# AMReX-Combustion/PeleAnalysis

Measured on AMD Instinct MI355X. Metric: Mcells/s for grad+curvature on 512^3-base 3-level AMR; % HBM roofline, higher is better.
Workload: dtype f64; 1 GPU; fused grad->curvature, 3-level AMR, base 512^3, ref_ratio 2, 128^3 boxes (64 per level) in the file, swept on the internal tiling pa_level_retile makes of them (4, 4, 4 boxes per level, largest 512x256x256), 1 comp(s), periodic x/y + wall z, 402653184 cells in the job; cells=402653184, cells_this_rank=402653184, ncomp=1, components_per_batch=1, fused=True, parallelism=single GPU

## Files before the change

include/peleanalysis_amd.h:

```cpp
#ifndef PELEANALYSIS_AMD_H
#define PELEANALYSIS_AMD_H
#include <stdint.h>

#ifdef __cplusplus
extern "C" {
#endif

typedef struct pa_ctx pa_ctx;
typedef struct pa_level pa_level;
typedef struct pa_mf pa_mf;

typedef struct { double* p; int32_t lo[3]; int32_t hi[3]; int32_t ncomp; int64_t nstride; } pa_fab;
typedef struct { int32_t lo[3]; int32_t hi[3]; } pa_box;

enum { PA_BC_PERIODIC = 0, PA_BC_NEUMANN = 1, PA_BC_REFLECT_ODD = 2 };

int         pa_version(void);
pa_ctx*     pa_ctx_create(int device, void* hip_stream );
void        pa_ctx_destroy(pa_ctx*);
const char* pa_last_error(const pa_ctx*);
int         pa_sync(pa_ctx*);
void*       pa_ctx_stream(pa_ctx*);
void        pa_options_reload(void);

void* pa_device_malloc(pa_ctx*, int64_t bytes);
void  pa_device_free(pa_ctx*, void* devptr);
int   pa_memcpy_h2d(pa_ctx*, void* devdst, const void* hostsrc, int64_t bytes);
int   pa_memcpy_d2h(pa_ctx*, void* hostdst, const void* devsrc, int64_t bytes);
int   pa_memcpy_d2d(pa_ctx*, void* devdst, const void* devsrc, int64_t bytes);
int   pa_device_count(void);

int pa_profile_enable(pa_ctx*, int on);
const char* pa_sweep_kernel_name(const pa_ctx*);
int pa_sweep_occupancy(pa_ctx*, int which);
int pa_last_slow_cells(pa_ctx*);
int64_t pa_level_irregular_cells(pa_ctx*, const pa_level*);
int pa_profile_read(pa_ctx*, int tag, int64_t* nlaunch, double* total_ms, int reset);

pa_level* pa_level_create(pa_ctx*, int nboxes, const int32_t* boxes6, const int32_t domlo[3],
                          const int32_t domhi[3], const int32_t is_per[3], const double prob_lo[3],
                          const double prob_hi[3]);
typedef struct { int32_t peer; double* sendbuf; int64_t nsend; double* recvbuf; int64_t nrecv; } pa_xfer;
typedef struct {
  void*   user;
  int32_t rank, nranks;
  int (*exchange)(void* user, void* hip_stream, int32_t n, const pa_xfer* x);
  int (*allreduce)(void* user, double* vals, int32_t n, int32_t op);
} pa_comm;
int pa_ctx_set_comm(pa_ctx*, const pa_comm*);
int pa_ctx_set_delay_comm(pa_ctx*, int nranks, int rank, double fixed_us, double link_GBs);
int pa_delay_comm_stats(const pa_ctx*, int64_t* calls, double* total_us);
int pa_rccl_unique_id(pa_ctx*, void* id128);
int pa_ctx_init_rccl(pa_ctx*, int nranks, int rank, const void* id128);
int pa_ctx_nranks(const pa_ctx*);
int pa_comm_selftest(pa_ctx*, int64_t n);
int pa_allreduce(pa_ctx*, double* vals, int n, int op);
int pa_distribution_map(int nboxes, const int32_t* boxes6, int nranks, int32_t* owner);
pa_level* pa_level_create_sharded(pa_ctx*, int nboxes, const int32_t* boxes6, const int32_t* owner, int rank, int nranks,
                                  const int32_t domlo[3], const int32_t domhi[3], const int32_t is_per[3],
                                  const double prob_lo[3], const double prob_hi[3]);
int pa_level_global_ids(const pa_level*, int32_t* gids );
int64_t pa_plan_fill_boundary(int nboxes, const int32_t* boxes6, const int32_t* owner, int rank, const int32_t domlo[3],
                              const int32_t domhi[3], const int32_t is_per[3], int ng, int32_t* rows9, int64_t cap);
int64_t pa_plan_coarse_source(int nfine, const int32_t* fboxes6, const int32_t* fowner, const int32_t fdomlo[3],
                              const int32_t fdomhi[3], int ncrse, const int32_t* cboxes6, const int32_t* cowner,
                              const int32_t cdomlo[3], const int32_t cdomhi[3], const int32_t is_per[3], int rank,
                              int mode, int ng, int halo, int32_t* rows9, int64_t cap);
int64_t pa_plan_restriction(int nfine, const int32_t* fboxes6, const int32_t* fowner, const int32_t fdomlo[3],
                            const int32_t fdomhi[3], int ncrse, const int32_t* cboxes6, const int32_t* cowner,
                            const int32_t cdomlo[3], const int32_t cdomhi[3], const int32_t is_per[3], int rank, int ratio,
                            int which, int32_t* rows9, int64_t cap);
int pa_level_retile(int nboxes, const int32_t* boxes6, const int32_t max_size[3], int min_thick, int32_t* out_boxes6, int cap);
int pa_hierarchy_retile_limits(int nlev, const int32_t* nboxes, const int32_t* const* boxes6, int min_thick, int32_t max_size[3]);
int pa_hierarchy_retile_limits_ranks(int nlev, const int32_t* nboxes, const int32_t* const* boxes6, int min_thick, int nranks, int32_t max_size[3]);
void      pa_level_destroy(pa_level*);
int       pa_level_nboxes(const pa_level*);

int64_t pa_mf_layout(int nboxes, const int32_t* boxes6, int ncomp, int ng, int64_t* off, int64_t* cstride);
pa_mf*  pa_mf_create(pa_ctx*, const pa_level*, int ncomp, int ng, double* devptr );
void    pa_mf_destroy(pa_mf*);
double* pa_mf_data(pa_mf*);
int64_t pa_mf_size(const pa_mf*);
int     pa_mf_upload(pa_ctx*, pa_mf*, const double* host);
int     pa_mf_download(pa_ctx*, const pa_mf*, double* host);
int     pa_mf_upload_comps(pa_ctx*, pa_mf*, const double* host, int comp, int ncomp);
int     pa_mf_download_comps(pa_ctx*, const pa_mf*, double* host, int comp, int ncomp);
int     pa_mf_setval(pa_ctx*, pa_mf*, int comp, int ncomp, double v);
int     pa_mf_copy(pa_ctx*, const pa_mf* src, int scomp, pa_mf* dst, int dcomp, int ncomp, int ng);

int pa_fill_boundary(pa_ctx*, pa_mf*, int comp, int ncomp, int ng);
int pa_apply_bc(pa_ctx*, pa_mf* fine, int comp, const pa_mf* crse, int ccomp, const int32_t bc[3],
                int ratio, int only_dir);
int pa_bc_errors(pa_ctx*);

int pa_grad_level(pa_ctx*, const pa_mf* phi, int comp, pa_mf* out, int ocomp);
int pa_minmax_level(pa_ctx*, const pa_mf* s, int comp, double* mn, double* mx);
int pa_progress_level(pa_ctx*, const pa_mf* s, int comp, double pmin, double pmax, pa_mf* c, int ccomp, int ng);
int pa_normal_level(pa_ctx*, const pa_mf* c, int comp, pa_mf* G, int gcomp, pa_mf* normgrad, int ngcomp,
                    pa_mf* n, int ncomp0);
int pa_div_level(pa_ctx*, pa_mf* n, int ncomp0, double scale, const pa_mf* c, int ccomp, double thr,
                 pa_mf* K, int kcomp);
int pa_progress_shell_level(pa_ctx*, const pa_mf* s, int comp, double pmin, double pmax, pa_mf* c, int ccomp, int ng,
                            int depth);
int pa_gradcurv_level(pa_ctx*, const pa_mf* phi, int pcomp, double prog_min, double prog_max, double thr,
                      pa_mf* out, int ocomp);
int pa_gradcurv_faces_level(pa_ctx*, const pa_mf* c, int ccomp, const pa_mf* crse_n ,
                            int cncomp0, const int32_t bc[3], int ratio, double thr, pa_mf* out, int ncomp0,
                            int kcomp);

int pa_grad_fab(pa_ctx*, pa_box valid, const pa_fab* phi, int comp, const double dxinv[3], pa_fab* out, int ocomp);
int pa_progress_fab(pa_ctx*, pa_box bx, const pa_fab* s, int comp, double pmin, double pmax, pa_fab* c, int ccomp);
int pa_normal_fab(pa_ctx*, pa_box valid, const pa_fab* c, int comp, const double dxinv[3], pa_fab* G, int gcomp,
                  pa_fab* normgrad, int ngcomp, pa_fab* n, int ncomp0);
int pa_div_fab(pa_ctx*, pa_box valid, const pa_fab* n, int ncomp0, const double dxinv[3], double scale,
               pa_fab* K, int kcomp);
int pa_gradcurv_fab(pa_ctx*, pa_box valid, const pa_fab* phi, int pcomp, double prog_min, double prog_max,
                    const double dxinv[3], double thr, pa_fab* out, int ocomp);
int pa_boxfilter_fab(pa_ctx*, pa_box valid, const pa_fab* in, pa_fab* out, int scomp, int ncomp, int ng,
                     const double* w );

int pa_box_filter_weights(int fgr, double* w);
int pa_filter_weights(int type, int fgr, double* w);
int pa_boxfilter_level(pa_ctx*, const pa_mf* in, pa_mf* out, int scomp, int ncomp, int ng, const double* w);
int pa_boxfilter_hierarchy(pa_ctx*, int nlev, const pa_mf* const* in, pa_mf* const* out, int scomp, int ncomp, const int32_t* ngs,
                           const double* const* ws);
int pa_boxfilter_level2d(pa_ctx*, const pa_mf* in, pa_mf* out, int scomp, int ncomp, int ng, const double* w);
int pa_foextrap(pa_ctx*, pa_mf*, int comp, int ncomp, int ng);
int pa_fillpatch_two_levels(pa_ctx*, pa_mf* fine, const pa_mf* crse, int comp, int ncomp, int ng, int ratio,
                            int interp_type);

int pa_fill_ghosts_hierarchy(pa_ctx*, int nlev, pa_mf* const* mfs, int comp, int ncomp, const int32_t* ngs, int ratio, int interp_type, int foextrap);

int pa_mc_count_fab(pa_ctx*, pa_box loop, const pa_fab* state, const pa_fab* mask, int isocomp, double isoval,
                    int64_t* nvert, int64_t* ntri);
int pa_mc_emit_fab(pa_ctx*, pa_box loop, const pa_fab* state, const pa_fab* mask, int isocomp, double isoval,
                   double* dev_verts , int32_t* dev_vkeys ,
                   int32_t* dev_tris , int64_t nvert, int64_t ntri);
int pa_iso_mask_level(pa_ctx*, pa_mf* mask, int comp, const pa_level* fine, int ratio);
int pa_iso_coords_level(pa_ctx*, pa_mf* state, int comp0);
int pa_mc_level(pa_ctx*, const pa_mf* state, const pa_mf* mask, int mcomp, const pa_box* loops ,
                int isocomp, double isoval, int64_t* nvert , int64_t* ntri ,
                double** dev_verts , int32_t** dev_vkeys ,
                int32_t** dev_tris );
int pa_msq_level(pa_ctx*, const pa_mf* state, const pa_mf* mask, int mcomp, const pa_box* loops ,
                 int isocomp, double isoval, int64_t* nvert , int64_t* nseg ,
                 double** dev_verts , int32_t** dev_vkeys ,
                 int32_t** dev_segs );
int pa_mc_level_fine(pa_ctx*, const pa_mf* state, const pa_level* fine, int ratio, const pa_box* loops, int isocomp,
                     double isoval, int64_t* nvert, int64_t* ntri, double** dev_verts, int32_t** dev_vkeys,
                     int32_t** dev_tris);
int pa_msq_level_fine(pa_ctx*, const pa_mf* state, const pa_level* fine, int ratio, const pa_box* loops, int isocomp,
                      double isoval, int64_t* nvert, int64_t* nseg, double** dev_verts, int32_t** dev_vkeys,
                      int32_t** dev_segs);
int pa_mc_hierarchy_fine(pa_ctx*, int nlev, const pa_mf* const* states, const int32_t* fine_mask, int ratio,
                         const pa_box* const* loops, int isocomp, double isoval, int64_t* const* nvert, int64_t* const* ntri,
                         double** dev_verts, int32_t** dev_vkeys, int32_t** dev_tris, void** block);
int pa_mc_hierarchy_xyz(pa_ctx*, int nlev, const pa_mf* const* fields, const int32_t* fine_mask, int ratio, const pa_box* const* loops,
                        int isocomp, double isoval, int64_t* const* nvert, int64_t* const* ntri, double** dev_verts, int32_t** dev_vkeys,
                        int32_t** dev_tris, void** block);
typedef struct { const double* verts; int64_t nvert; const int32_t* tris; int64_t ntri; } pa_iso_frag;
int pa_iso_merge(pa_ctx*, int nfrag, const pa_iso_frag* frags , int ncomp, int64_t* nnodes,
                 double** dev_nodes, int64_t* nelts, int32_t** dev_elts);
const uint16_t* pa_mc_edge_table(void);
const int8_t*   pa_mc_tri_table(void);

typedef struct {
  int64_t ntri;  const uint32_t* tri;
  int64_t nvert; const float* x;
  float origin[3]; float dx;
  int32_t n[3];
  float* phi;
} pa_sdf_grid;
int pa_sdf_level_set3(pa_ctx*, int ngrids, const pa_sdf_grid* grids , int exact_band );
int pa_sdf_signed_fab(pa_ctx*, pa_box vbox, const float* dev_phi, const pa_fab* state, int isocomp, double isoval,
                      double dmax, pa_fab* dist, int dcomp);

int pa_stream_trace(pa_ctx*, int nlev, pa_mf* const* vfield, int vcomp, int64_t nseed, const double* seeds, int nsteps,
                    double dt, double* dev_pos, int32_t* nredist );
int pa_stream_trace_ranks(pa_ctx*, int nlev, pa_mf* const* vfield, int vcomp, int64_t nseed, const double* seeds, int nsteps,
                          double dt, double* dev_pos, int32_t* nredist , int share_flags);

int pa_vtrace_fab(pa_ctx*, const pa_fab* T, int32_t nT, const double* loc, int64_t nloc, const int32_t* ids, int32_t n_ids,
                  pa_fab* g, int32_t computeVec, pa_fab* strm, int32_t ncs, const double dx[3], const double plo[3],
                  const double phi[3], double hRK, int32_t* errFlag);
int pa_streamgrad_prepare(pa_ctx*, int nlev, pa_mf* const* state);
int pa_streamgrad_trace(pa_ctx*, int nlev, pa_mf* const* state, int vcomp, int64_t nnodes, const double* nodes,
                        const int64_t* box_start, const int32_t* ids, int nRKsteps, double hRK, double* strm,
                        int32_t* box_flag);

// ... 97 lines not shown
```

peleanalysis_amd/capi.py:

```python
from __future__ import annotations

import ctypes as C
import os
from typing import List, Optional, Sequence

import numpy as np

from .hierarchy import Hierarchy, Level, MultiFab, mf_layout

_HERE = os.path.dirname(os.path.abspath(__file__))
LIB_PATH = os.path.join(_HERE, "libpeleanalysis_amd.so")

BC_PERIODIC, BC_NEUMANN, BC_REFLECT_ODD = 0, 1, 2


class PaFab(C.Structure):
    _fields_ = [("p", C.c_void_p), ("lo", C.c_int32 * 3), ("hi", C.c_int32 * 3), ("ncomp", C.c_int32), ("nstride", C.c_int64)]


class PaBox(C.Structure):
    _fields_ = [("lo", C.c_int32 * 3), ("hi", C.c_int32 * 3)]


class PaCurvParams(C.Structure):
    _fields_ = [("prog_min", C.c_double), ("prog_max", C.c_double), ("do_threshold", C.c_int32), ("threshold", C.c_double),
                ("fused", C.c_int32), ("do_gauss_curv", C.c_int32), ("do_strain", C.c_int32), ("get_strain_tensor", C.c_int32),
                ("do_velnormal", C.c_int32), ("vel_comp", C.c_int32), ("do_smooth", C.c_int32), ("smoothing_time", C.c_double),
                ("spacedim", C.c_int32)]


class PaXfer(C.Structure):
    _fields_ = [("peer", C.c_int32), ("sendbuf", C.c_void_p), ("nsend", C.c_int64), ("recvbuf", C.c_void_p), ("nrecv", C.c_int64)]


EXCHANGE_FN = C.CFUNCTYPE(C.c_int, C.c_void_p, C.c_void_p, C.c_int32, C.POINTER(PaXfer))
ALLREDUCE_FN = C.CFUNCTYPE(C.c_int, C.c_void_p, C.POINTER(C.c_double), C.c_int32, C.c_int32)


DONE_FN = C.CFUNCTYPE(C.c_int, C.c_void_p, C.c_int)
DONE2_FN = C.CFUNCTYPE(C.c_int, C.c_void_p, C.c_int, C.c_int)


class PaComm(C.Structure):
    _fields_ = [("user", C.c_void_p), ("rank", C.c_int32), ("nranks", C.c_int32), ("exchange", EXCHANGE_FN), ("allreduce", ALLREDUCE_FN)]


class PaIsoFrag(C.Structure):
    _fields_ = [("verts", C.c_void_p), ("nvert", C.c_int64), ("tris", C.c_void_p), ("ntri", C.c_int64)]


class PaJpdfParams(C.Structure):
    _fields_ = [("nload", C.c_int32), ("do_stoichiometry", C.c_int32), ("hlist", C.c_double * 8), ("olist", C.c_double * 8), ("vmin", C.c_double * 8),
                ("vmax", C.c_double * 8), ("do_conditioning", C.c_int32), ("cvar", C.c_int32), ("norm_cval", C.c_int32), ("cnorm_min", C.c_double),
                ("cnorm_max", C.c_double), ("cmin", C.c_double), ("cmax", C.c_double), ("uncombined", C.c_int32)]


class PaSdfGrid(C.Structure):
    _fields_ = [("ntri", C.c_int64), ("tri", C.c_void_p), ("nvert", C.c_int64), ("x", C.c_void_p), ("origin", C.c_float * 3), ("dx", C.c_float),
                ("n", C.c_int32 * 3), ("phi", C.c_void_p)]


_lib = None


def load_library() -> C.CDLL:
    global _lib
    if _lib is not None:
        return _lib
    if not os.path.exists(LIB_PATH):
        raise RuntimeError(f"{LIB_PATH} not found: run `python -c 'import __graft_entry__ as g; g.build()'` "
                           "(hipcc --offload-arch=gfx950).  There is no CPU fallback.")
    L = C.CDLL(LIB_PATH)
    vp, i32, i64, dbl = C.c_void_p, C.c_int32, C.c_int64, C.c_double
    pi32, pdbl = C.POINTER(C.c_int32), C.POINTER(C.c_double)
    sig = {
        "pa_version": (C.c_int, []),
        "pa_options_reload": (None, []),
        "pa_ctx_create": (vp, [C.c_int, vp]),
        "pa_ctx_destroy": (None, [vp]),
        "pa_last_error": (C.c_char_p, [vp]),
        "pa_sync": (C.c_int, [vp]),
        "pa_ctx_stream": (vp, [vp]),
        "pa_device_malloc": (vp, [vp, i64]),
        "pa_device_free": (None, [vp, vp]),
        "pa_memcpy_h2d": (C.c_int, [vp, vp, vp, i64]),
        "pa_memcpy_d2h": (C.c_int, [vp, vp, vp, i64]),
        "pa_memcpy_d2d": (C.c_int, [vp, vp, vp, i64]),
        "pa_device_count": (C.c_int, []),
        "pa_profile_enable": (C.c_int, [vp, C.c_int]),
        "pa_sweep_kernel_name": (C.c_char_p, [vp]),
        "pa_sweep_occupancy": (C.c_int, [vp, C.c_int]),
        "pa_profile_read": (C.c_int, [vp, C.c_int, C.POINTER(i64), pdbl, C.c_int]),
        "pa_level_create": (vp, [vp, C.c_int, pi32, pi32, pi32, pi32, pdbl, pdbl]),
        "pa_level_create_sharded": (vp, [vp, C.c_int, pi32, pi32, C.c_int, C.c_int, pi32, pi32, pi32, pdbl, pdbl]),
        "pa_level_global_ids": (C.c_int, [vp, pi32]),
        "pa_ctx_set_comm": (C.c_int, [vp, C.POINTER(PaComm)]),
        "pa_ctx_set_delay_comm": (C.c_int, [vp, C.c_int, C.c_int, dbl, dbl]),
        "pa_delay_comm_stats": (C.c_int, [vp, C.POINTER(i64), pdbl]),
        "pa_rccl_unique_id": (C.c_int, [vp, vp]),
        "pa_ctx_init_rccl": (C.c_int, [vp, C.c_int, C.c_int, vp]),
        "pa_ctx_nranks": (C.c_int, [vp]),
        "pa_comm_selftest": (C.c_int, [vp, i64]),
        "pa_allreduce": (C.c_int, [vp, pdbl, C.c_int, C.c_int]),
        "pa_distribution_map": (C.c_int, [C.c_int, pi32, C.c_int, pi32]),
        "pa_plan_fill_boundary": (i64, [C.c_int, pi32, pi32, C.c_int, pi32, pi32, pi32, C.c_int, pi32, i64]),
        "pa_plan_coarse_source": (i64, [C.c_int, pi32, pi32, pi32, pi32, C.c_int, pi32, pi32, pi32, pi32, pi32, C.c_int, C.c_int, C.c_int, C.c_int, pi32,
                                        i64]),
        "pa_plan_restriction": (i64, [C.c_int, pi32, pi32, pi32, pi32, C.c_int, pi32, pi32, pi32, pi32, pi32, C.c_int, C.c_int, C.c_int, pi32, i64]),
        "pa_level_retile": (C.c_int, [C.c_int, pi32, pi32, C.c_int, pi32, C.c_int]),
        "pa_hierarchy_retile_limits": (C.c_int, [C.c_int, pi32, C.POINTER(pi32), C.c_int, pi32]),
        "pa_hierarchy_retile_limits_ranks": (C.c_int, [C.c_int, pi32, C.POINTER(pi32), C.c_int, C.c_int, pi32]),
        "pa_level_destroy": (None, [vp]),
        "pa_level_nboxes": (C.c_int, [vp]),
        "pa_mf_layout": (i64, [C.c_int, pi32, C.c_int, C.c_int, C.POINTER(i64), C.POINTER(i64)]),
        "pa_mf_create": (vp, [vp, vp, C.c_int, C.c_int, vp]),
        "pa_mf_destroy": (None, [vp]),
        "pa_mf_data": (vp, [vp]),
        "pa_mf_size": (i64, [vp]),
        "pa_mf_upload": (C.c_int, [vp, vp, vp]),
        "pa_mf_download": (C.c_int, [vp, vp, vp]),
        "pa_mf_upload_comps": (C.c_int, [vp, vp, vp, C.c_int, C.c_int]),
        "pa_mf_download_comps": (C.c_int, [vp, vp, vp, C.c_int, C.c_int]),
        "pa_mf_setval": (C.c_int, [vp, vp, C.c_int, C.c_int, dbl]),
        "pa_mf_copy": (C.c_int, [vp, vp, C.c_int, vp, C.c_int, C.c_int, C.c_int]),
        "pa_fill_boundary": (C.c_int, [vp, vp, C.c_int, C.c_int, C.c_int]),
        "pa_apply_bc": (C.c_int, [vp, vp, C.c_int, vp, C.c_int, pi32, C.c_int, C.c_int]),
        "pa_bc_errors": (C.c_int, [vp]),
        "pa_grad_level": (C.c_int, [vp, vp, C.c_int, vp, C.c_int]),
        "pa_minmax_level": (C.c_int, [vp, vp, C.c_int, pdbl, pdbl]),
        "pa_progress_level": (C.c_int, [vp, vp, C.c_int, dbl, dbl, vp, C.c_int, C.c_int]),
        "pa_normal_level": (C.c_int, [vp, vp, C.c_int, vp, C.c_int, vp, C.c_int, vp, C.c_int]),
        "pa_div_level": (C.c_int, [vp, vp, C.c_int, dbl, vp, C.c_int, dbl, vp, C.c_int]),
        "pa_progress_shell_level": (C.c_int, [vp, vp, C.c_int, dbl, dbl, vp, C.c_int, C.c_int, C.c_int]),
        "pa_gradcurv_level": (C.c_int, [vp, vp, C.c_int, dbl, dbl, dbl, vp, C.c_int]),
        "pa_gradcurv_faces_level": (C.c_int, [vp, vp, C.c_int, vp, C.c_int, pi32, C.c_int, dbl, vp, C.c_int, C.c_int]),
        "pa_grad_fab": (C.c_int, [vp, PaBox, C.POINTER(PaFab), C.c_int, pdbl, C.POINTER(PaFab), C.c_int]),
        "pa_progress_fab": (C.c_int, [vp, PaBox, C.POINTER(PaFab), C.c_int, dbl, dbl, C.POINTER(PaFab), C.c_int]),
        "pa_normal_fab": (C.c_int, [vp, PaBox, C.POINTER(PaFab), C.c_int, pdbl, C.POINTER(PaFab), C.c_int, C.POINTER(PaFab), C.c_int,
                                    C.POINTER(PaFab), C.c_int]),
        "pa_div_fab": (C.c_int, [vp, PaBox, C.POINTER(PaFab), C.c_int, pdbl, dbl, C.POINTER(PaFab), C.c_int]),
        "pa_gradcurv_fab": (C.c_int, [vp, PaBox, C.POINTER(PaFab), C.c_int, dbl, dbl, pdbl, dbl, C.POINTER(PaFab), C.c_int]),
        "pa_boxfilter_fab": (C.c_int, [vp, PaBox, C.POINTER(PaFab), C.POINTER(PaFab), C.c_int, C.c_int, C.c_int, pdbl]),
        "pa_box_filter_weights": (C.c_int, [C.c_int, pdbl]),
        "pa_filter_weights": (C.c_int, [C.c_int, C.c_int, pdbl]),
        "pa_boxfilter_level": (C.c_int, [vp, vp, vp, C.c_int, C.c_int, C.c_int, pdbl]),
        "pa_boxfilter_hierarchy": (C.c_int, [vp, C.c_int, C.POINTER(vp), C.POINTER(vp), C.c_int, C.c_int, pi32, C.POINTER(pdbl)]),
        "pa_boxfilter_level2d": (C.c_int, [vp, vp, vp, C.c_int, C.c_int, C.c_int, pdbl]),
        "pa_foextrap": (C.c_int, [vp, vp, C.c_int, C.c_int, C.c_int]),
        "pa_fillpatch_two_levels": (C.c_int, [vp, vp, vp, C.c_int, C.c_int, C.c_int, C.c_int, C.c_int]),
        "pa_fill_ghosts_hierarchy": (C.c_int, [vp, C.c_int, C.POINTER(vp), C.c_int, C.c_int, pi32, C.c_int, C.c_int, C.c_int]),
        "pa_mc_count_fab": (C.c_int, [vp, PaBox, C.POINTER(PaFab), C.POINTER(PaFab), C.c_int, dbl, C.POINTER(i64), C.POINTER(i64)]),
        "pa_mc_emit_fab": (C.c_int, [vp, PaBox, C.POINTER(PaFab), C.POINTER(PaFab), C.c_int, dbl, vp, vp, vp, i64, i64]),
        "pa_iso_mask_level": (C.c_int, [vp, vp, C.c_int, vp, C.c_int]),
        "pa_iso_coords_level": (C.c_int, [vp, vp, C.c_int]),
        "pa_mc_level_fine": (C.c_int, [vp, vp, vp, C.c_int, C.POINTER(PaBox), C.c_int, dbl, C.POINTER(i64), C.POINTER(i64), C.POINTER(vp), C.POINTER(vp),
                                       C.POINTER(vp)]),
        "pa_msq_level_fine": (C.c_int, [vp, vp, vp, C.c_int, C.POINTER(PaBox), C.c_int, dbl, C.POINTER(i64), C.POINTER(i64), C.POINTER(vp), C.POINTER(vp),
                                        C.POINTER(vp)]),
        "pa_mc_hierarchy_fine": (C.c_int, [vp, C.c_int, C.POINTER(vp), pi32, C.c_int, C.POINTER(C.POINTER(PaBox)), C.c_int, dbl, C.POINTER(C.POINTER(i64)),
                                           C.POINTER(C.POINTER(i64)), C.POINTER(vp), C.POINTER(vp), C.POINTER(vp), C.POINTER(vp)]),
        "pa_mc_hierarchy_xyz": (C.c_int, [vp, C.c_int, C.POINTER(vp), pi32, C.c_int, C.POINTER(C.POINTER(PaBox)), C.c_int, dbl, C.POINTER(C.POINTER(i64)),
                                          C.POINTER(C.POINTER(i64)), C.POINTER(vp), C.POINTER(vp), C.POINTER(vp), C.POINTER(vp)]),
        "pa_msq_level": (C.c_int, [vp, vp, vp, C.c_int, C.POINTER(PaBox), C.c_int, dbl, C.POINTER(i64), C.POINTER(i64), C.POINTER(vp), C.POINTER(vp),
                                   C.POINTER(vp)]),
        "pa_mc_level": (C.c_int, [vp, vp, vp, C.c_int, C.POINTER(PaBox), C.c_int, dbl, C.POINTER(i64), C.POINTER(i64), C.POINTER(vp), C.POINTER(vp),
                                  C.POINTER(vp)]),
        "pa_iso_merge": (C.c_int, [vp, C.c_int, C.POINTER(PaIsoFrag), C.c_int, C.POINTER(i64), C.POINTER(vp), C.POINTER(i64), C.POINTER(vp)]),
        "pa_mc_edge_table": (C.POINTER(C.c_uint16), []),
        "pa_mc_tri_table": (C.POINTER(C.c_int8), []),
        "pa_sdf_level_set3": (C.c_int, [vp, C.c_int, C.POINTER(PaSdfGrid), C.c_int]),
        "pa_sdf_signed_fab": (C.c_int, [vp, PaBox, vp, C.POINTER(PaFab), C.c_int, dbl, dbl, C.POINTER(PaFab), C.c_int]),
        "pa_smooth_solve": (C.c_int, [vp, C.c_int, C.POINTER(vp), C.c_int, C.POINTER(vp), C.c_int, dbl, pi32, dbl, C.c_int, C.POINTER(C.c_int), pdbl]),
        "pa_stream_trace": (C.c_int, [vp, C.c_int, C.POINTER(vp), C.c_int, i64, pdbl, C.c_int, dbl, vp, pi32]),
        "pa_last_slow_cells": (C.c_int, [vp]),
        "pa_level_irregular_cells": (i64, [vp, vp]),
        "pa_stream_trace_ranks": (C.c_int, [vp, C.c_int, C.POINTER(vp), C.c_int, i64, pdbl, C.c_int, dbl, vp, pi32, C.c_int]),
        "pa_vtrace_fab": (C.c_int, [vp, C.POINTER(PaFab), i32, vp, i64, vp, i32, C.POINTER(PaFab), i32, C.POINTER(PaFab), i32, pdbl, pdbl, pdbl, dbl,
                                    pi32]),
        "pa_streamgrad_prepare": (C.c_int, [vp, C.c_int, C.POINTER(vp)]),
        "pa_streamgrad_trace": (C.c_int, [vp, C.c_int, C.POINTER(vp), C.c_int, i64, vp, C.POINTER(i64), vp, C.c_int, dbl, vp, pi32]),
        "pa_interpstream_fab": (C.c_int, [vp, C.POINTER(PaFab), i32, C.POINTER(PaFab), i32, C.POINTER(PaFab), pdbl, pdbl, pi32]),
        "pa_set_distance_fab": (C.c_int, [vp, C.POINTER(PaFab), C.POINTER(PaFab)]),
        "pa_streamsample_run": (C.c_int, [vp, C.c_int, C.POINTER(vp), i32, pdbl, pdbl, pi32, pi32, pi32, pi32, pi32, vp, vp, i32, i32, i32, pi32]),
        "pa_device_mem_info": (C.c_int, [vp, C.POINTER(i64), C.POINTER(i64)]),
        "pa_minmax_comps_level": (C.c_int, [vp, vp, C.c_int, pi32, pdbl, pdbl]),
        "pa_jpdf_create": (vp, [vp, C.c_int, C.c_int]),
        "pa_jpdf_begin": (C.c_int, [vp, vp, dbl, pdbl]),
        "pa_jpdf_add_level": (C.c_int, [vp, vp, vp, vp, C.c_int, dbl, C.POINTER(PaJpdfParams), C.POINTER(i64), C.POINTER(i64)]),
        "pa_jpdf_read": (C.c_int, [vp, vp, pdbl, pdbl, pdbl]),
        "pa_condmean_create": (vp, [vp, C.c_int, C.c_int, C.c_int]),
        "pa_condmean_begin": (C.c_int, [vp, vp, i64, pdbl]),
        "pa_condmean_add_level": (C.c_int, [vp, vp, vp, vp, C.c_int, C.POINTER(PaBox), i64, dbl, dbl, C.c_int]),
        "pa_condmean_read": (C.c_int, [vp, vp, C.POINTER(i64), pdbl, pdbl, pdbl, pdbl]),
        "pa_hist_destroy": (None, [vp]),
        "pa_integral_create": (vp, [vp, C.c_int, C.c_int, C.c_int, C.POINTER(PaBox), C.c_int]),
        "pa_integral_begin": (C.c_int, [vp, vp, dbl, pdbl]),
        "pa_integral_add_level": (C.c_int, [vp, vp, vp, vp, C.c_int, C.c_int, dbl, C.c_int, dbl, dbl, C.c_int]),
        "pa_integral_slots": (i64, [vp]),
        "pa_integral_read": (C.c_int, [vp, vp, pdbl]),
        "pa_integral_destroy": (None, [vp]),
        "pa_tube_create": (vp, [vp, i32, C.POINTER(i64), i64, pi32, i64, pi32]),
        "pa_tube_destroy": (None, [vp]),
        "pa_tube_wedges": (C.c_int, [vp, vp, vp, vp, i32, i32, i32, i32, vp, vp, vp, vp, vp]),
        "pa_tube_lines": (C.c_int, [vp, vp, vp, vp, i32, i32, i32, vp]),
        "pa_tube_peaks": (C.c_int, [vp, vp, vp, i32, i32, i32, pi32, vp, vp]),
        "pa_tube_node_means": (C.c_int, [vp, vp, i32, vp, vp]),
        "pa_tube_node_all": (C.c_int, [vp, vp, vp, vp]),
        "pa_tube_node_avg": (C.c_int, [vp, vp, vp, i32, i32, vp]),
        "pa_tube_smooth": (C.c_int, [vp, vp, vp, vp, i32, vp]),
        "pa_tube_neighbors": (C.c_int, [vp, vp, C.POINTER(i64), C.POINTER(i64), pi32]),
        "pa_smooth_last": (C.c_int, [vp, C.POINTER(C.c_int), pdbl]),
        "pa_curvature_last_path": (C.c_int, [vp]),
        "pa_level_free_scratch": (i64, [vp]),
        "pa_grad_run": (C.c_int, [vp, C.c_int, C.POINTER(vp), C.c_int, pi32, C.POINTER(vp), C.c_int]),
        "pa_curvature_run": (C.c_int, [vp, C.c_int, C.POINTER(vp), C.c_int, pi32, C.POINTER(PaCurvParams), C.POINTER(vp), C.c_int]),
        "pa_gradcurv_run": (C.c_int, [vp, C.c_int, C.POINTER(vp), C.c_int, pi32, C.POINTER(PaCurvParams), C.POINTER(vp), C.POINTER(vp),
                                      C.c_int]),
        "pa_gradcurv_run_comps": (C.c_int, [vp, C.c_int, C.POINTER(vp), C.c_int, C.c_int, pi32, C.POINTER(PaCurvParams), C.POINTER(vp), C.POINTER(vp),
                                            C.c_int, DONE_FN, vp]),
        "pa_gradcurv_run_comps2": (C.c_int, [vp, C.c_int, C.POINTER(vp), C.c_int, C.c_int, pi32, C.POINTER(PaCurvParams), C.POINTER(vp), C.POINTER(vp),
                                             C.c_int, C.c_int, DONE2_FN, vp]),
    }
    missing = []
    for name, (res, args) in sig.items():
        try:
            fn = getattr(L, name)
        except AttributeError:
            missing.append(name)
            continue
        fn.restype = res
        fn.argtypes = args
    L._pa_signatures = sig
    L._pa_missing = missing
    _lib = L
    return L


def declared_symbols(header: Optional[str] = None) -> List[str]:
    import re
    header = header or os.path.join(os.path.dirname(_HERE), "include", "peleanalysis_amd.h")
    txt = re.sub(r"/\*.*?\*/", "", open(header).read(), flags=re.S)
    return sorted(set(re.findall(r"\b(pa_[a-z0-9_]+)\s*\(", txt)))


def reload_options() -> None:
    load_library().pa_options_reload()


class PaError(RuntimeError):
    pass


def _i3(v):
    return (C.c_int32 * 3)(*[int(x) for x in v])


def _d3(v):
    return (C.c_double * 3)(*[float(x) for x in v])


class Context:
    def __init__(self, device: int = 0, stream: Optional[int] = None):
        self.lib = load_library()
        self.h = self.lib.pa_ctx_create(int(device), C.c_void_p(stream) if stream else None)
        if not self.h:
            raise PaError("pa_ctx_create failed: no MI355X/HIP device visible (no CPU fallback)")

    def check(self, rc: int):
        if rc != 0:
            raise PaError(self.lib.pa_last_error(self.h).decode())

    def sync(self):
        self.check(self.lib.pa_sync(self.h))

    def profile_enable(self, on=True):
        self.check(self.lib.pa_profile_enable(self.h, int(on)))

    def profile_read(self, tag: int, reset: bool = False):
        n, ms = C.c_int64(0), C.c_double(0.0)
        self.check(self.lib.pa_profile_read(self.h, tag, C.byref(n), C.byref(ms), int(reset)))
        return n.value, ms.value

    def bc_errors(self) -> int:
        return int(self.lib.pa_bc_errors(self.h))

    def set_comm(self, comm: "PaComm"):
        self._comm = comm
        self.check(self.lib.pa_ctx_set_comm(self.h, C.byref(comm) if comm is not None else None))

    def rccl_unique_id(self) -> bytes:
        buf = C.create_string_buffer(128)
        self.check(self.lib.pa_rccl_unique_id(self.h, buf))
        return buf.raw

    def init_rccl(self, nranks: int, rank: int, unique_id: bytes):
        assert len(unique_id) == 128
        self.check(self.lib.pa_ctx_init_rccl(self.h, int(nranks), int(rank), C.create_string_buffer(unique_id, 128)))

    def comm_selftest(self, n: int = 4096):
        self.check(self.lib.pa_comm_selftest(self.h, int(n)))

    def allreduce(self, vals, op: int):
        a = np.ascontiguousarray(vals, dtype=np.float64).copy()
        self.check(self.lib.pa_allreduce(self.h, a.ctypes.data_as(C.POINTER(C.c_double)), a.size, int(op)))
        return a

    def close(self):
        if self.h:
            self.lib.pa_ctx_destroy(self.h)
            self.h = None

    def __enter__(self):
        return self

    def __exit__(self, *exc):
        self.close()


class DevBuf:

    def __init__(self, ctx: Context, nbytes: int):
        self.ctx, self.nbytes = ctx, int(nbytes)
        self.ptr = ctx.lib.pa_device_malloc(ctx.h, self.nbytes)
        if not self.ptr:
            raise PaError(ctx.lib.pa_last_error(ctx.h).decode())

    @classmethod
    def from_numpy(cls, ctx: Context, a: np.ndarray) -> "DevBuf":
# ... 689 lines not shown
```

peleanalysis_amd/csrc/pa_core.hip:

```cpp
#include "pa_internal.h"
#include "pa_dist.h"
#include <algorithm>
#include <atomic>
#include <cstring>
#include <numeric>

int pa_fail(pa_ctx* ctx, const std::string& msg) {
  if (ctx) ctx->err = msg;
  return 1;
}

extern "C" int pa_version(void) { return 100; }

static int host_owner(const pa_level* L, int i, int j, int k);
const WgTab* pa_sweep_wgtab(const pa_level* L, int cls, int tw, int mty, int kseg, bool force, int part) {
  if (part) force = true;
  const long long key = ((long long)cls << 56) | ((long long)part << 54) | ((long long)(force ? 1 : 0) << 52) | ((long long)tw << 40) | ((long long)mty << 24) | (long long)kseg;
  auto it = L->wgtabs.find(key);
  if (it != L->wgtabs.end()) return (it->second->d || part) ? it->second.get() : nullptr;
  std::unique_ptr<WgTab> T(new WgTab());
  struct Chunk { int n, box, t0; };
  std::vector<std::pair<int, int>> bt;
  std::vector<std::vector<int>> sel;
  long long real = 0;
// ... 536 lines not shown
        cpoff[e] = L->cp_total;
        L->cp_total += ((long long)pw * ph + 7) / 8 * 8;
      }
    }
    sfindex[f] = (int)e;
    sfoff[e] = ncode;
    ncode += (long long)(B.hi[t0] - B.lo[t0] + 1) * (B.hi[t1] - B.lo[t1] + 1);
    L->cgoff[e] = L->cg_total;
    L->cg_total += ((long long)(B.hi[t0] - B.lo[t0] + 3) * (B.hi[t1] - B.lo[t1] + 5) + 7) / 8 * 8;
  }
  {
    std::vector<int> wide, narrow;
    for (int b = 0; b < nboxes; ++b) {
      const DBox& B = L->boxes[b];
      const bool nar = B.hi[0] - B.lo[0] + 1 <= 32;
      (nar ? narrow : wide).push_back(b);
      for (int d = 0; d < 3; ++d) {
        int& m = nar ? L->nmax[d] : L->wmax[d];
        m = std::max(m, B.hi[d] - B.lo[d] + 1);
      }
    }
    L->nwide = (int)wide.size();
    L->nnarrow = (int)narrow.size();
    if (L->nwide && L->nnarrow) {
      wide.insert(wide.end(), narrow.begin(), narrow.end());
      if (hipMalloc(&L->d_blist, sizeof(int) * wide.size()) != hipSuccess ||
          hipMemcpy(L->d_blist, wide.data(), sizeof(int) * wide.size(), hipMemcpyHostToDevice) != hipSuccess) {
        pa_fail(ctx, "pa_level_create: device allocation failed");
        delete L;
        return nullptr;
      }
    }
  }
  {
    std::vector<int> wg, pwg;
    for (size_t e = 0; e < L->sfaces.size(); ++e) {
      const int f = L->sfaces[e];
      const DBox& B = L->boxes[f / 6];
      const int d = (f % 6) >> 1, t0 = (d == 0) ? 1 : 0, t1 = (d == 2) ? 1 : 2;
      const long long nc = (long long)(B.hi[t0] - B.lo[t0] + 1) * (B.hi[t1] - B.lo[t1] + 1);
      for (int c = 0; c < (int)((nc + 255) / 256); ++c) { wg.push_back((int)e); wg.push_back(c); }
      const long long n0 = B.hi[t0] - B.lo[t0] + 1, n1 = B.hi[t1] - B.lo[t1] + 1, P = n1 >= 2 ? 2 * n0 + 2 * (n1 - 2) : n0;
      for (int c = 0; c < (int)((P + 255) / 256); ++c) { pwg.push_back((int)e); pwg.push_back(c); }
    }
    L->npfwg = (int)(pwg.size() / 2);
    if (L->npfwg > 0 && (hipMalloc(&L->d_pfwg, sizeof(int) * pwg.size()) != hipSuccess ||
                         hipMemcpy(L->d_pfwg, pwg.data(), sizeof(int) * pwg.size(), hipMemcpyHostToDevice) != hipSuccess)) {
      pa_fail(ctx, "pa_level_create: device allocation failed");
      delete L;
      return nullptr;
    }
    std::vector<int> sfb;
    for (int f : L->sfaces)
      if (sfb.empty() || sfb.back() != f / 6) sfb.push_back(f / 6);
    L->nsfboxes = (int)sfb.size();
    if (L->nsfboxes > 0 && (hipMalloc(&L->d_sfboxes, sizeof(int) * sfb.size()) != hipSuccess ||
                            hipMemcpy(L->d_sfboxes, sfb.data(), sizeof(int) * sfb.size(), hipMemcpyHostToDevice) != hipSuccess)) {
      pa_fail(ctx, "pa_level_create: device allocation failed");
      delete L;
      return nullptr;
    }
    {
      std::vector<SfChunk> ck;
      for (size_t e = 0; e < L->sfaces.size(); ++e) {
        const int f = L->sfaces[e];
        const DBox& B = L->boxes[f / 6];
        const int d = (f % 6) >> 1, t0 = (d == 0) ? 1 : 0, t1 = (d == 2) ? 1 : 2;
        const int n0 = B.hi[t0] - B.lo[t0] + 1, n1 = B.hi[t1] - B.lo[t1] + 1;
        int cw = 32;
        while (cw < 512 && cw < n0) cw *= 2;
        const int ch = 1024 / cw;
        for (int v0 = -(B.lo[t1] & 1); v0 < n1; v0 += ch)
          for (int u0 = -(B.lo[t0] & 1); u0 < n0; u0 += cw) {
            SfChunk D;
            D.face = (int)e; D.box = f / 6; D.dir_side = f % 6; D.flags = 0;
            for (int q = 0; q < 3; ++q) { D.lo[q] = B.lo[q]; D.hi[q] = B.hi[q]; }
            D.u0 = u0; D.v0 = v0; D.cw = cw; D.ch = ch;
            D.sfoff = sfoff[e]; D.cgoff = L->cgoff[e]; D.cpoff = cpoff[e];
            ck.push_back(D);
          }
      }
      L->nsfchunk = (int)ck.size();
      if (L->nsfchunk > 0 && (hipMalloc(&L->d_sfchunk, sizeof(SfChunk) * ck.size()) != hipSuccess ||
                              hipMemcpy(L->d_sfchunk, ck.data(), sizeof(SfChunk) * ck.size(), hipMemcpyHostToDevice) != hipSuccess)) {
        pa_fail(ctx, "pa_level_create: device allocation failed");
        delete L;
        return nullptr;
      }
    }
    L->nsfwg = (int)(wg.size() / 2);
    if (L->nsfwg > 0 && (hipMalloc(&L->d_sfwg, sizeof(int) * wg.size()) != hipSuccess ||
                         hipMemcpy(L->d_sfwg, wg.data(), sizeof(int) * wg.size(), hipMemcpyHostToDevice) != hipSuccess)) {
      pa_fail(ctx, "pa_level_create: device allocation failed");
      delete L;
      return nullptr;
    }
  }
  if (hipMalloc(&L->d_boxes, sizeof(DBox) * std::max(nboxes, 1)) != hipSuccess ||
      hipMalloc(&L->d_sfaces, sizeof(int) * nsf_alloc) != hipSuccess ||
      (!L->sfaces.empty() && hipMemcpy(L->d_sfaces, L->sfaces.data(), sizeof(int) * L->sfaces.size(), hipMemcpyHostToDevice) != hipSuccess) ||
      hipMalloc(&L->d_sfindex, sizeof(int) * std::max<size_t>(sfindex.size(), 1)) != hipSuccess ||
      (!sfindex.empty() && hipMemcpy(L->d_sfindex, sfindex.data(), sizeof(int) * sfindex.size(), hipMemcpyHostToDevice) != hipSuccess) ||
      hipMalloc(&L->d_cpoff, sizeof(long long) * nsf_alloc) != hipSuccess ||
      hipMemcpy(L->d_cpoff, cpoff.data(), sizeof(long long) * nsf_alloc, hipMemcpyHostToDevice) != hipSuccess ||
      hipMalloc(&L->d_cgoff, sizeof(long long) * nsf_alloc) != hipSuccess ||
      hipMemcpy(L->d_cgoff, L->cgoff.data(), sizeof(long long) * nsf_alloc, hipMemcpyHostToDevice) != hipSuccess ||
      hipMalloc(&L->d_sfoff, sizeof(long long) * nsf_alloc) != hipSuccess ||
      hipMemcpy(L->d_sfoff, sfoff.data(), sizeof(long long) * nsf_alloc, hipMemcpyHostToDevice) != hipSuccess ||
      hipMalloc(&L->d_sfcode, sizeof(unsigned short) * std::max<long long>(ncode, 1)) != hipSuccess ||
      hipMalloc(&L->d_owner, sizeof(int) * msz) != hipSuccess ||
      (nboxes > 0 && hipMemcpy(L->d_boxes, L->boxes.data(), sizeof(DBox) * nboxes, hipMemcpyHostToDevice) != hipSuccess) ||
      hipMemcpy(L->d_owner, L->owner.data(), sizeof(int) * msz, hipMemcpyHostToDevice) != hipSuccess) {
    pa_fail(ctx, "pa_level_create: device allocation failed");
    if (L->d_boxes) (void)hipFree(L->d_boxes);
    if (L->d_owner) (void)hipFree(L->d_owner);
    if (L->d_sfaces) (void)hipFree(L->d_sfaces);
    if (L->d_sfindex) (void)hipFree(L->d_sfindex);
    if (L->d_sfoff) (void)hipFree(L->d_sfoff);
    if (L->d_cgoff) (void)hipFree(L->d_cgoff);
    if (L->d_cpoff) (void)hipFree(L->d_cpoff);
    if (L->d_sfcode) (void)hipFree(L->d_sfcode);
    delete L;
    return nullptr;
  }
  DLevelView& V = L->view;
  V.cgoff = L->d_cgoff;
  V.cg = nullptr;
  V.cpoff = L->d_cpoff;
  V.cp = nullptr;
  V.sfindex = L->d_sfindex;
  V.sfoff = L->d_sfoff;
  V.sfcode = L->d_sfcode;
  V.gshift = (g & (g - 1)) == 0 ? __builtin_ctz((unsigned)g) : -1;
  V.nsf = (int)L->sfaces.size();
  V.sfaces = L->d_sfaces;
  V.nboxes = nboxes;
  V.boxes = L->d_boxes;
  V.owner = L->d_owner;
  V.g = g;
  for (int d = 0; d < 3; ++d) {
    V.domlo[d] = L->domlo[d]; V.domhi[d] = L->domhi[d]; V.is_per[d] = L->is_per[d];
    V.mlo[d] = L->mlo[d]; V.mn[d] = L->mn[d]; V.dxinv[d] = L->dxinv[d];
  }
  if (!L->sfaces.empty()) {
    const long long n0 = L->maxn[0], n1 = L->maxn[1], n2 = L->maxn[2];
    const long long nt = std::max(n1 * n2, std::max(n0 * n2, n0 * n1));
    hipLaunchKernelGGL(k_build_sfcode, dim3((unsigned)((nt + 255) / 256), (unsigned)L->sfaces.size()), dim3(256), 0, ctx->stream, V, L->d_sfcode);
    if (L->nsfchunk > 0) hipLaunchKernelGGL(k_sfchunk_flags, dim3((unsigned)L->nsfchunk), dim3(256), 0, ctx->stream, V, L->d_sfchunk);
    if (hipGetLastError() != hipSuccess || hipStreamSynchronize(ctx->stream) != hipSuccess) {
      pa_fail(ctx, "pa_level_create: building the boundary masks failed");
      pa_level_destroy(L);
      return nullptr;
    }
  }
  return L;
}

extern "C" void pa_level_destroy(pa_level* L) {
  if (!L) return;
  if (L->d_sfaces) (void)hipFree(L->d_sfaces);
  if (L->d_sfindex) (void)hipFree(L->d_sfindex);
  if (L->d_sfoff) (void)hipFree(L->d_sfoff);
  if (L->d_cgoff) (void)hipFree(L->d_cgoff);
  if (L->d_cg) (void)hipFree(L->d_cg);
  if (L->d_ncg) (void)hipFree(L->d_ncg);
  if (L->d_cpoff) (void)hipFree(L->d_cpoff);
  if (L->d_cp) (void)hipFree(L->d_cp);
  if (L->d_sfcode) (void)hipFree(L->d_sfcode);
  if (L->d_boxes) (void)hipFree(L->d_boxes);
  if (L->d_owner) (void)hipFree(L->d_owner);
  if (L->d_irr) (void)hipFree(L->d_irr);
  if (L->d_sfwg) (void)hipFree(L->d_sfwg);
  if (L->d_pfwg) (void)hipFree(L->d_pfwg);
  if (L->d_sfchunk) (void)hipFree(L->d_sfchunk);
  if (L->d_ring) (void)hipFree(L->d_ring);
  if (L->d_blist) (void)hipFree(L->d_blist);
  if (L->d_sfboxes) (void)hipFree(L->d_sfboxes);
  delete L;
}
extern "C" int pa_level_nboxes(const pa_level* L) { return L ? (int)L->boxes.size() : 0; }

extern "C" int64_t pa_mf_layout(int nboxes, const int32_t* b6, int ncomp, int ng, int64_t* off, int64_t* cstride) {
  int64_t t = 0;
  for (int b = 0; b < nboxes; ++b) {
    if (off) off[b] = t;
    int64_t n = 1;
    for (int d = 0; d < 3; ++d) n *= (int64_t)(b6[6 * b + 3 + d] - b6[6 * b + d] + 1 + 2 * ng);
    const int64_t cs = pa_cstride(n, ncomp);
    if (cstride) cstride[b] = cs;
    t += cs * ncomp;
  }
  return t;
}

extern "C" pa_mf* pa_mf_create(pa_ctx* ctx, const pa_level* L, int ncomp, int ng, double* devptr) {
  PaBind bind_(ctx);
  if (!ctx || !L) return nullptr;
  if (ncomp <= 0 || ng < 0) { pa_fail(ctx, "pa_mf_create: bad ncomp/ng"); return nullptr; }
  pa_mf* M = new pa_mf();
  M->lev = L; M->ncomp = ncomp; M->ng = ng;
  const int nb = (int)L->boxes.size();
  std::vector<int32_t> b6(6 * (size_t)nb);
  for (int b = 0; b < nb; ++b)
    for (int d = 0; d < 3; ++d) { b6[6 * b + d] = L->boxes[b].lo[d]; b6[6 * b + 3 + d] = L->boxes[b].hi[d]; }
  std::vector<int64_t> off(nb);
  M->total = pa_mf_layout(nb, b6.data(), ncomp, ng, off.data(), nullptr);
  M->off.assign(off.begin(), off.end());
  if (hipMalloc(&M->d_off, sizeof(long long) * std::max(nb, 1)) != hipSuccess ||
      (nb > 0 && hipMemcpy(M->d_off, M->off.data(), sizeof(long long) * nb, hipMemcpyHostToDevice) != hipSuccess)) {
    pa_fail(ctx, "pa_mf_create: device allocation failed");
    delete M;
    return nullptr;
  }
  if (devptr) {
    M->data = devptr;
  } else {
    if (hipMalloc(&M->data, sizeof(double) * (size_t)std::max<long long>(M->total, 1)) != hipSuccess ||
        hipMemsetAsync(M->data, 0, sizeof(double) * (size_t)M->total, ctx->stream) != hipSuccess) {
      pa_fail(ctx, "pa_mf_create: out of device memory (" + std::to_string(M->total * 8) + " bytes)");
      (void)hipFree(M->d_off);
      delete M;
      return nullptr;
    }
    M->owned = true;
  }
  M->view.data = M->data; M->view.off = M->d_off; M->view.ncomp = ncomp; M->view.ng = ng; M->view.xform = 0; M->view.xa = 0; M->view.xb = 1;
  return M;
}

extern "C" void pa_mf_destroy(pa_mf* M) {
  if (!M) return;
  if (M->owned && M->data) (void)hipFree(M->data);
  if (M->d_off) (void)hipFree(M->d_off);
  delete M;
}
extern "C" double* pa_mf_data(pa_mf* M) { return M ? M->data : nullptr; }
extern "C" int64_t pa_mf_size(const pa_mf* M) { return M ? M->total : 0; }

extern "C" int pa_mf_upload(pa_ctx* ctx, pa_mf* M, const double* host) {
  PaBind bind_(ctx);
  if (ctx && M && M->total == 0) return 0;
  if (!ctx || !M || !host) return pa_fail(ctx, "pa_mf_upload: null argument");
  PA_HIP(hipMemcpyAsync(M->data, host, sizeof(double) * (size_t)M->total, hipMemcpyHostToDevice, ctx->stream));
  PA_HIP(hipStreamSynchronize(ctx->stream));
  return 0;
}
extern "C" int pa_mf_download(pa_ctx* ctx, const pa_mf* M, double* host) {
  PaBind bind_(ctx);
  if (ctx && M && M->total == 0) return 0;
  if (!ctx || !M || !host) return pa_fail(ctx, "pa_mf_download: null argument");
  PA_HIP(hipMemcpyAsync(host, M->data, sizeof(double) * (size_t)M->total, hipMemcpyDeviceToHost, ctx->stream));
  PA_HIP(hipStreamSynchronize(ctx->stream));
  return 0;
}

static int mf_copy_comps(pa_ctx* ctx, const pa_mf* M, double* host, int comp, int ncomp, bool up, const char* who) {
  if (ctx && M && M->total == 0) return 0;
  if (!ctx || !M || !host) return pa_fail(ctx, std::string(who) + ": null argument");
  if (comp < 0 || ncomp < 1 || comp + ncomp > M->ncomp) return pa_fail(ctx, std::string(who) + ": component range");
  const pa_level* L = M->lev;
  for (size_t b = 0; b < L->boxes.size(); ++b) {
    const DBox& B = L->boxes[b];
    const long long cs = pa_cstride((long long)(B.hi[0] - B.lo[0] + 1 + 2 * M->ng) * (B.hi[1] - B.lo[1] + 1 + 2 * M->ng) * (B.hi[2] - B.lo[2] + 1 + 2 * M->ng), M->ncomp);
    const long long o = M->off[b] + (long long)comp * cs;
    if (up) PA_HIP(hipMemcpyAsync(M->data + o, host + o, sizeof(double) * (size_t)(cs * ncomp), hipMemcpyHostToDevice, ctx->stream));
    else PA_HIP(hipMemcpyAsync(host + o, M->data + o, sizeof(double) * (size_t)(cs * ncomp), hipMemcpyDeviceToHost, ctx->stream));
  }
  PA_HIP(hipStreamSynchronize(ctx->stream));
  return 0;
}
extern "C" int pa_mf_upload_comps(pa_ctx* ctx, pa_mf* M, const double* host, int comp, int ncomp) {
  PaBind bind_(ctx);
  return mf_copy_comps(ctx, M, const_cast<double*>(host), comp, ncomp, true, "pa_mf_upload_comps");
}
extern "C" int pa_mf_download_comps(pa_ctx* ctx, const pa_mf* M, double* host, int comp, int ncomp) {
  PaBind bind_(ctx);
  return mf_copy_comps(ctx, M, host, comp, ncomp, false, "pa_mf_download_comps");
}

__global__ void k_setval(double* p, long long n, double v) {
  for (long long i = blockIdx.x * (long long)blockDim.x + threadIdx.x; i < n; i += (long long)gridDim.x * blockDim.x) p[i] = v;
}

__global__ void k_setval_comp(DLevelView L, DMFView M, int comp, int ncomp, double v) {
  const int b = blockIdx.y;
  const DBox B = L.boxes[b];
  const long long per = pa_cstride((long long)(B.hi[0] - B.lo[0] + 1 + 2 * M.ng) * (B.hi[1] - B.lo[1] + 1 + 2 * M.ng) *
                                       (B.hi[2] - B.lo[2] + 1 + 2 * M.ng), M.ncomp);
  double* p = M.data + M.off[b] + per * comp;
  const long long n = per * ncomp;
  for (long long i = blockIdx.x * (long long)blockDim.x + threadIdx.x; i < n; i += (long long)gridDim.x * blockDim.x) p[i] = v;
}

extern "C" int pa_mf_setval(pa_ctx* ctx, pa_mf* M, int comp, int ncomp, double v) {
  PaBind bind_(ctx);
  if (!ctx || !M) return pa_fail(ctx, "pa_mf_setval: null argument");
  if (comp < 0 || comp + ncomp > M->ncomp) return pa_fail(ctx, "pa_mf_setval: component range");
  if (M->lev->boxes.empty()) return 0;
  dim3 grid(64, (unsigned)M->lev->boxes.size());
  hipLaunchKernelGGL(k_setval_comp, grid, dim3(256), 0, ctx->stream, M->lev->view, M->view, comp, ncomp, v);
  PA_HIP(hipGetLastError());
  return 0;
}

__global__ void k_copy(DLevelView L, DMFView S, int scomp, DMFView D, int dcomp, int ncomp, int ng) {
  const int b = blockIdx.y;
  const DBox B = L.boxes[b];
  const int nx = B.hi[0] - B.lo[0] + 1 + 2 * ng, ny = B.hi[1] - B.lo[1] + 1 + 2 * ng, nz = B.hi[2] - B.lo[2] + 1 + 2 * ng;
  const long long n = (long long)nx * ny * nz * ncomp;
  for (long long t = blockIdx.x * (long long)blockDim.x + threadIdx.x; t < n; t += (long long)gridDim.x * blockDim.x) {
    const int i = (int)(t % nx);
    const int j = (int)((t / nx) % ny);
    const int k = (int)((t / ((long long)nx * ny)) % nz);
    const int c = (int)(t / ((long long)nx * ny * nz));
    const int I = B.lo[0] - ng + i, J = B.lo[1] - ng + j, K = B.lo[2] - ng + k;
    D.data[D.off[b] + fab_index(B, D.ng, D.ncomp, dcomp + c, I, J, K)] = S.data[S.off[b] + fab_index(B, S.ng, S.ncomp, scomp + c, I, J, K)];
  }
}

extern "C" int pa_mf_copy(pa_ctx* ctx, const pa_mf* S, int scomp, pa_mf* D, int dcomp, int ncomp, int ng) {
  PaBind bind_(ctx);
  if (!ctx || !S || !D) return pa_fail(ctx, "pa_mf_copy: null argument");
  if (S->lev != D->lev) return pa_fail(ctx, "pa_mf_copy: different levels");
  if (ng > S->ng || ng > D->ng || scomp + ncomp > S->ncomp || dcomp + ncomp > D->ncomp)
    return pa_fail(ctx, "pa_mf_copy: ng/component range");
  if (S->lev->boxes.empty()) return 0;
  dim3 grid(128, (unsigned)S->lev->boxes.size());
  hipLaunchKernelGGL(k_copy, grid, dim3(256), 0, ctx->stream, S->lev->view, S->view, scomp, D->view, dcomp, ncomp, ng);
  PA_HIP(hipGetLastError());
  return 0;
}

__device__ __forceinline__ bool shell_cell(const DBox& B, int ng, long long tt, int& i, int& j, int& k) {
// ... 469 lines not shown
```

peleanalysis_amd/csrc/pa_fused.hip:

```cpp
#include "pa_internal.h"
#include "pa_dist.h"
#include "pa_fabview.h"
#include "pa_fused_march.h"
#include "pa_fused_march3.h"
#include "pa_fused_march3n.h"
#include <algorithm>
#include <cstdlib>

#ifndef PA_FC_WAVES
#define PA_FC_WAVES 3
#endif
struct Vec3 { double x, y, z; };

struct ShellAcc {
  FabView C;
  int cc;
  __device__ __forceinline__ double operator()(int i, int j, int k) const { return C(i, j, k, cc); }
};
struct CgAcc {
  const DLevelView* L;
  FabView P;
  DBox B;
  int b, pcomp;
  double pmin, invd;
  const double* cg;
  __device__ __forceinline__ double operator()(int i, int j, int k) const {
    const int p[3] = {i, j, k};
    int nout = 0, fd[2] = {0, 0}, fs[2] = {0, 0};
    bool near = true;
#pragma unroll
    for (int d = 0; d < 3; ++d) {
      const int o = p[d] < B.lo[d] ? B.lo[d] - p[d] : (p[d] > B.hi[d] ? p[d] - B.hi[d] : 0);
      if (o) {
        if (nout < 2) { fd[nout] = d; fs[nout] = p[d] > B.hi[d]; }
        ++nout;
        near = near && o == 1;
      }
    }
    int e = -1, d = 0;
    if (near && nout == 1) { d = fd[0]; e = L->sfindex[b * 6 + d * 2 + fs[0]]; }
    if (near && nout == 2) {
      const int ea = L->sfindex[b * 6 + fd[0] * 2 + fs[0]], ec = L->sfindex[b * 6 + fd[1] * 2 + fs[1]];
      if (ea >= 0 && ec >= 0) return 0.0;
      if (ea >= 0) { e = ea; d = fd[0]; }
      if (ec >= 0) { e = ec; d = fd[1]; }
    }
    if (e < 0) return (P(i, j, k, pcomp) - pmin) * invd;
    const int t0 = (d == 0) ? 1 : 0, t1 = (d == 2) ? 1 : 2;
    return cg[L->cgoff[e] + (long long)(p[t1] - B.lo[t1] + 1) * (B.hi[t0] - B.lo[t0] + 3) + (p[t0] - B.lo[t0] + 1)];
  }
};

template <typename Acc>
__device__ __forceinline__ Vec3 normal_at(const Acc& C, int i, int j, int k, const double dxinv[3]) {
  Vec3 n;
  normal_from(C(i - 1, j, k), C(i + 1, j, k), C(i, j - 1, k), C(i, j + 1, k), C(i, j, k - 1), C(i, j, k), C(i, j, k + 1), dxinv, n.x, n.y, n.z);
  return n;
}

struct FaceArgs {
  int bc[3];
  int ratio;
  int has_crse;
  int layers;
  double thr;
  int perim_only;
  double pmin, invd;
};

struct FixArgs {
  DLevelView L;
  DMFView MC_;
  int ccomp;
  DLevelView LCr;
  DMFView MN;
  int cncomp0;
  DMFView MO;
  int ncomp0, kcomp;
  FaceArgs A;
  int use_cp = 0;
  long long cg_stride = 0, cp_stride = 0;
  const int2* wg = nullptr; int nwg = 0;
  const int2* pwg = nullptr; int npwg = 0;
  const double* ncg = nullptr; long long ncgs = 0; int ncg_minw = 0;
};
typedef double pa_fix_d2 __attribute__((ext_vector_type(2)));
__device__ __forceinline__ bool ncg_face_ok(const DBox& B, int side, int minw) {
  const int nx = B.hi[0] - B.lo[0] + 1;
  return nx >= minw && (side ? ((nx - 1) & 63) + 1 : min(nx, 64)) >= 3;
}
template <typename BT>
__device__ __forceinline__ bool wg_decode(const BT& Bt, int& blev, unsigned& fy, long long& t, unsigned w = blockIdx.x) {
  blev = 0;
  while (blev + 1 < Bt.n && w >= (unsigned)Bt.a[blev].nwg) { w -= (unsigned)Bt.a[blev].nwg; ++blev; }
  if (w >= (unsigned)Bt.a[blev].nwg) return false;
  const int2 c = Bt.a[blev].wg[w];
  fy = (unsigned)c.x;
  t = (long long)c.y * 256 + threadIdx.x;
  return true;
}
struct SlotK { const double* prog = nullptr; int cn_z = 8; };

__device__ __forceinline__ double comp_of(const Vec3& v, int d) { return d == 0 ? v.x : (d == 1 ? v.y : v.z); }

__device__ __forceinline__ bool in_box(const DBox& B, const int q[3]) {
  return q[0] >= B.lo[0] && q[0] <= B.hi[0] && q[1] >= B.lo[1] && q[1] <= B.hi[1] && q[2] >= B.lo[2] && q[2] <= B.hi[2];
}

__global__ __launch_bounds__(256) void k_faces_normal(DLevelView L, DMFView MC_, int ccomp, DMFView MO, int ncomp0, FaceArgs A) {
  int b, dir, side, layer, q[3];
  DBox B;
  const long long t = blockIdx.x * (long long)blockDim.x + threadIdx.x;
  if (!sface_decode(L, blockIdx.y, t, 1, b, B, dir, side, q, layer)) return;
  if ((L.sfcode[L.sfoff[blockIdx.y] + t] & 3u) == 0) return;
  int X[3] = {q[0], q[1], q[2]};
  X[dir] += side ? -1 : 1;
  const ShellAcc C = {mf_view(MC_, B, b), ccomp};
  const double dxinv[3] = {L.dxinv[0], L.dxinv[1], L.dxinv[2]};
  Vec3 no = normal_at(C, X[0], X[1], X[2], dxinv);
  if (A.thr >= 0.0) {
    const double c0 = C(X[0], X[1], X[2]);
    if (c0 < A.thr || c0 > 1.0 - A.thr) { no.x = 0.0; no.y = 0.0; no.z = 0.0; }
  }
  double* o = MO.data + MO.off[b];
  o[fab_index(B, MO.ng, MO.ncomp, ncomp0, X[0], X[1], X[2])] = no.x;
  o[fab_index(B, MO.ng, MO.ncomp, ncomp0 + 1, X[0], X[1], X[2])] = no.y;
  o[fab_index(B, MO.ng, MO.ncomp, ncomp0 + 2, X[0], X[1], X[2])] = no.z;
}

struct SlowList {
  int* count; int2* items; int cap;
  int* gcount = nullptr; int4* gitems = nullptr; int gcap = 0; unsigned glev = 0;
};
template <bool CG, bool PATCH, bool CGCLIP = false>
__device__ __forceinline__ void faces_curv_cell(const LevBatch<FixArgs>& Bt, unsigned y, long long t, int perim_only, int* nbad, const SlotK& sk, int z) {
  unsigned fy;
  const FixArgs& Fx = Bt.a[Bt.find(y, fy)];
  const DLevelView& L = Fx.L;
  const DMFView& MC_ = Fx.MC_;
  const DLevelView& LCr = Fx.LCr;
  const DMFView& MN = Fx.MN;
  const DMFView& MO = Fx.MO;
  FaceArgs A = Fx.A;
  if (sk.prog) { A.pmin = sk.prog[2 * z]; A.invd = sk.prog[2 * z + 1]; }
  const int ccomp = Fx.ccomp + z, cncomp0 = Fx.cncomp0 + sk.cn_z * z, ncomp0 = Fx.ncomp0 + 8 * z, kcomp = Fx.kcomp + 8 * z;
  const double* cgz = L.cg + z * Fx.cg_stride;
  const double* cpz = L.cp ? L.cp + z * Fx.cp_stride : nullptr;
  int b, fdir, side, layer, q0[3];
  DBox B;
  if (perim_only) {
    const int e = L.sfaces[fy];
    b = e / 6; fdir = (e % 6) >> 1; side = e & 1;
    B = L.boxes[b];
    const int t0 = (fdir == 0) ? 1 : 0, t1 = (fdir == 2) ? 1 : 2;
    const unsigned n0 = B.hi[t0] - B.lo[t0] + 1, n1 = B.hi[t1] - B.lo[t1] + 1;
    const unsigned P = (n1 >= 2) ? 2 * n0 + 2 * (n1 - 2) : n0;
    if (t >= (long long)P * A.layers) return;
    unsigned r = (unsigned)t;
    layer = 0;
    while (r >= P) { r -= P; ++layer; }
    unsigned a0, a1;
    if (r < n0) { a0 = r; a1 = 0; }
    else if (r < 2 * n0) { a0 = r - n0; a1 = n1 - 1; }
    else { r -= 2 * n0; a0 = (r & 1u) ? n0 - 1 : 0; a1 = 1 + (r >> 1); }
    if (n0 == 1 && (r & 1u) && t >= 2 * (long long)n0) return;
    q0[fdir] = side ? B.hi[fdir] + 1 : B.lo[fdir] - 1;
    q0[t0] = B.lo[t0] + (int)a0;
    q0[t1] = B.lo[t1] + (int)a1;
    if (layer >= B.hi[fdir] - B.lo[fdir] + 1) return;
    if ((L.sfcode[L.sfoff[fy] + a0 + (long long)n0 * a1] & 3u) == 0) return;
  } else {
    if (!sface_decode(L, fy, t, A.layers, b, B, fdir, side, q0, layer)) return;
    const int t0 = (fdir == 0) ? 1 : 0, t1 = (fdir == 2) ? 1 : 2;
    if (layer >= B.hi[fdir] - B.lo[fdir] + 1) return;
    if ((L.sfcode[L.sfoff[fy] + (t - (long long)layer * (B.hi[t0] - B.lo[t0] + 1) * (B.hi[t1] - B.lo[t1] + 1))] & 3u) == 0) return;
  }
  const int n[3] = {B.hi[0] - B.lo[0] + 1, B.hi[1] - B.lo[1] + 1, B.hi[2] - B.lo[2] + 1};
  int X[3] = {q0[0], q0[1], q0[2]};
  X[fdir] += side ? -(1 + layer) : (1 + layer);
  const ShellAcc Cs = {mf_view(MC_, B, b), ccomp};
  const CgAcc Cg = {&L, mf_view(MC_, B, b), B, b, ccomp, A.pmin, A.invd, cgz};
  const double dxinv[3] = {L.dxinv[0], L.dxinv[1], L.dxinv[2]};
  const double* o = MO.data + MO.off[b];
  auto C = [&](int i, int j, int k) -> double { return CG ? Cg(i, j, k) : Cs(i, j, k); };
  auto nrm = [&](const int p[3], int d) -> double {
    if ((!CG || CGCLIP) && A.thr >= 0.0) {
      const double cp = C(p[0], p[1], p[2]);
      if (cp < A.thr || cp > 1.0 - A.thr) return comp_of(normal_at(C, p[0], p[1], p[2], dxinv), d);
    }
    return o[fab_index(B, MO.ng, MO.ncomp, ncomp0 + d, p[0], p[1], p[2])];
  };
  double curv = 0.0;
  bool ok = true;
  for (int d = 0; d < 3; ++d) {
    const double n0d = nrm(X, d);
    double nb[2];
    for (int s2 = 0; s2 < 2; ++s2) {
      const int sg = s2 ? 1 : -1;
      int q[3] = {X[0], X[1], X[2]};
      q[d] += sg;
      if (in_box(B, q)) { nb[s2] = nrm(q, d); continue; }
      unsigned code = 0;
      const int e2 = L.sfindex[b * 6 + d * 2 + s2];
      {
        const int u0 = (d == 0) ? 1 : 0, u1 = (d == 2) ? 1 : 2;
        if (e2 >= 0) code = L.sfcode[L.sfoff[e2] + (q[u0] - B.lo[u0]) + (long long)n[u0] * (q[u1] - B.lo[u1])];
      }
      const int cls = (int)(code & 3u);
      if (cls == 0) {
        nb[s2] = comp_of(normal_at(C, q[0], q[1], q[2], dxinv), d);
      } else if (cls == 2) {
        nb[s2] = (A.bc[d] == PA_BC_REFLECT_ODD) ? -n0d : n0d;
      } else {
        if (!A.has_crse) { ok = false; nb[s2] = 0.0; continue; }
        double coef[4];
        const int NX = cf_normal_coef(n[d], A.ratio, coef);
        const int xf[1] = {0};
        double bv1[1];
        const long long cpo = (Fx.use_cp && L.cp) ? L.cpoff[e2] : -1;
        if (PATCH || cpo >= 0) cf_interp_patch<1>(code, cpz + cpo, B, s2, MN, q, d, xf, ok, bv1);
        else cf_interp<1>(code, LCr, MN, cncomp0 + d, q, d, A.ratio, xf, ok, bv1);
        const double bv = bv1[0];
        double tmp = 0.0;
        for (int m = 1; m < NX; ++m) {
          int pc[3] = {q[0], q[1], q[2]};
          pc[d] -= sg * m;
          const double v = (m == 1) ? n0d : nrm(pc, d);
          tmp += v * coef[m];
        }
        double g = tmp;
        g += bv * coef[0];
        nb[s2] = g;
      }
    }
    curv += cdiff(dxinv[d], nb[0], n0d, nb[1]);
  }
  curv = curv * 0.5;
  if ((!CG || CGCLIP) && A.thr >= 0.0) {
    const double c0 = C(X[0], X[1], X[2]);
    if (c0 < A.thr || c0 > 1.0 - A.thr) curv = 0.0;
  }
  if (!ok) atomicAdd(nbad, 1);
  MO.data[MO.off[b] + fab_index(B, MO.ng, MO.ncomp, kcomp, X[0], X[1], X[2])] = curv;
}
template <bool CG, bool PATCH = false, bool CGCLIP = false>
__global__ __launch_bounds__(256, PA_FC_WAVES) void k_faces_curv(LevBatch<FixArgs> Bt, int* nbad, SlotK sk = SlotK()) {
  unsigned fy;
  const int perim = Bt.a[Bt.find(blockIdx.y, fy)].A.perim_only;
  faces_curv_cell<CG, PATCH, CGCLIP>(Bt, blockIdx.y, blockIdx.x * (long long)blockDim.x + threadIdx.x, perim, nbad, sk, (int)blockIdx.z);
}
template <bool CG, bool PATCH, bool CGCLIP>
__device__ __forceinline__ void faces_tab_wg(const LevBatch<FixArgs>& Bt, int* nbad, const SlotK& sk, unsigned w) {
  int blev = 0;
  while (blev + 1 < Bt.n && w >= (unsigned)Bt.a[blev].npwg) { w -= (unsigned)Bt.a[blev].npwg; ++blev; }
  if (w >= (unsigned)Bt.a[blev].npwg) return;
  const int2 it = Bt.a[blev].pwg[w];
  faces_curv_cell<CG, PATCH, CGCLIP>(Bt, (unsigned)Bt.ycum[blev] + (unsigned)it.x, (long long)it.y * 256 + threadIdx.x, 1, nbad, sk, (int)blockIdx.z);
}
template <bool CG, bool PATCH = false, bool CGCLIP = false>
__global__ __launch_bounds__(256, PA_FC_WAVES) void k_faces_curv_tab(LevBatch<FixArgs> Bt, int* nbad, SlotK sk = SlotK()) {
  faces_tab_wg<CG, PATCH, CGCLIP>(Bt, nbad, sk, blockIdx.x);
}
template <bool PATCH>
__global__ __launch_bounds__(256, PA_FC_WAVES) void k_faces_curv_list(LevBatch<FixArgs> Bt, int* nbad, SlowList sl, SlotK sk = SlotK()) {
  const int n = min(*sl.count, sl.cap);
  for (int i = blockIdx.x * 256 + threadIdx.x; i < n; i += gridDim.x * 256) {
    const int2 it = sl.items[i];
    faces_curv_cell<true, PATCH, true>(Bt, (unsigned)it.x & 0xffffffu, it.y, 0, nbad, sk, (int)((unsigned)it.x >> 24));
  }
}

template <int FD, int NL, bool PATCH, bool CLIP = false>
__device__ __forceinline__ void faces_curv_fast_body(const DLevelView& L, const DLevelView& LCr, const DMFView& MN, int cncomp0, const DMFView& MO,
                                                     int ncomp0, int kcomp, const FaceArgs& A, int* nbad, int b, const DBox& B, int side,
                                                     const int q0[3], unsigned code, const double* patch, const DMFView& MP = DMFView(), int pcomp = 0, SlowList sl = SlowList(),
                                                     unsigned row = 0, long long tcell = 0, const double* ncgp = nullptr, long long ncgs = 0) {
  constexpr int T0 = (FD == 0) ? 1 : 0, T1 = (FD == 2) ? 1 : 2;
  const int cls = (int)(code & 3u);
  int sbn = -1, qw[3] = {0, 0, 0};
  if (cls == 0) {
    if (NL > 1) return;
    if (classify(L, q0[0], q0[1], q0[2], sbn, qw) != 0 || sbn < 0) return;
  }
  const int n[3] = {B.hi[0] - B.lo[0] + 1, B.hi[1] - B.lo[1] + 1, B.hi[2] - B.lo[2] + 1};
  const int sg = side ? 1 : -1;
  int X1[3] = {q0[0], q0[1], q0[2]};
  X1[FD] -= sg;
  const long long nxo = n[0] + 2 * MO.ng, nyo = n[1] + 2 * MO.ng, nzo = n[2] + 2 * MO.ng;
  const long long cso = pa_cstride(nxo * nyo * nzo, MO.ncomp);
  const long long st[3] = {1, nxo, nxo * nyo};
  const long long idx1 = ((long long)(X1[2] - B.lo[2] + MO.ng) * nyo + (X1[1] - B.lo[1] + MO.ng)) * nxo + (X1[0] - B.lo[0] + MO.ng);
  const long long in = -sg * st[FD];
  double* o = MO.data + MO.off[b];
  const double* nf = o + (long long)(ncomp0 + FD) * cso + idx1;
  const double* n0p = o + (long long)(ncomp0 + T0) * cso + idx1;
  const double* n1p = o + (long long)(ncomp0 + T1) * cso + idx1;
  const bool pre = FD == 0 && NL == 1 && !CLIP && ncgp != nullptr;
  double nfd1, nfd2, nfd3, a0m = 0, a0c = 0, a0p = 0, a1m = 0, a1c = 0, a1p = 0, t01n = 0, t11n = 0;
  if (pre) {
    const pa_fix_d2* np = (const pa_fix_d2*)ncgp;
    const pa_fix_d2 v0 = np[0], v1 = np[ncgs], v2 = np[2 * ncgs];
    nfd1 = v0.x; nfd2 = v0.y; nfd3 = v1.x; t01n = v1.y; t11n = v2.x;
  } else {
    nfd1 = nf[0]; nfd2 = nf[in]; nfd3 = nf[2 * in];
    a0m = n0p[-st[T0]]; a0c = n0p[0]; a0p = n0p[st[T0]];
    a1m = n1p[-st[T1]]; a1c = n1p[0]; a1p = n1p[st[T1]];
  }
  if (CLIP) {
    static_assert(!CLIP || NL == 1, "the clip-aware fast path fixes one layer");
    const FabView P = mf_view(MP, B, b);
    auto clipped = [&](int i, int j, int k) {
      const double c = (P(i, j, k, pcomp) - A.pmin) * A.invd;
      return c < A.thr || c > 1.0 - A.thr;
    };
    if (clipped(X1[0], X1[1], X1[2])) return;
    const int iv = -sg;
    bool slow = false;
    if (cls == 0) {
      const double gn = MO.data[MO.off[sbn] + fab_index(L.boxes[sbn], MO.ng, MO.ncomp, ncomp0 + FD, qw[0], qw[1], qw[2])];
      slow = gn == 0.0 && clipped(q0[0], q0[1], q0[2]);
    }
// ... 201 lines not shown
  DBox B;
#pragma unroll
  for (int d = 0; d < 3; ++d) { B.lo[d] = D.lo[d]; B.hi[d] = D.hi[d]; }
  const bool wall = (D.flags & PA_SFC_WALL) != 0;
  const bool pre = FD == 0 && Fx.ncg && z == 0 && ncg_face_ok(B, side, Fx.ncg_minw);
  double nfd[2][2][3], A0[2][4], A1[2][4], t01n[2][2], t11n[2][2];
  long long k0[4], k1o[4];
#pragma unroll
  for (int k = 0; k < 4; ++k) {
    k0[k] = (long long)(min(max(u + k - 1, 0), n0 - 1) - u) * s0;
    k1o[k] = (long long)(min(max(v + k - 1, 0), n1 - 1) - v) * s1;
  }
  if (pre) {
    const pa_fix_d2* np = (const pa_fix_d2*)(Fx.ncg + 2 * (D.cgoff + (long long)(v + 1) * (n0 + 2) + (u + 1)));
#pragma unroll
    for (int dv = 0; dv < 2; ++dv)
#pragma unroll
      for (int du = 0; du < 2; ++du) {
        const pa_fix_d2 v0 = np[dv * (n0 + 2) + du], v1 = np[Fx.ncgs + dv * (n0 + 2) + du], v2 = np[2 * Fx.ncgs + dv * (n0 + 2) + du];
        nfd[dv][du][0] = v0.x; nfd[dv][du][1] = v0.y; nfd[dv][du][2] = v1.x; t01n[dv][du] = v1.y; t11n[dv][du] = v2.x;
      }
  } else {
#pragma unroll
    for (int dv = 0; dv < 2; ++dv)
#pragma unroll
      for (int du = 0; du < 2; ++du)
#pragma unroll
        for (int m = 0; m < 3; ++m) nfd[dv][du][m] = nf[dv * s1 + du * s0 + m * in];
#pragma unroll
    for (int dv = 0; dv < 2; ++dv)
#pragma unroll
      for (int k = 0; k < 4; ++k) A0[dv][k] = n0p[dv * s1 + k0[k]];
#pragma unroll
    for (int du = 0; du < 2; ++du)
#pragma unroll
      for (int k = 0; k < 4; ++k) A1[du][k] = n1p[du * s0 + k1o[k]];
  }
  double r[3][3];
  if (!wall) {
    int plane, pu0, pv0, pw, ph;
    cpatch_geom(B, FD, side, plane, pu0, pv0, pw, ph);
    const double* const cb = L.cp + z * Fx.cp_stride + D.cpoff + (long long)((X1[T1] >> 1) - pv0) * pw + ((X1[T0] >> 1) - pu0);
    bool ok = true;
#pragma unroll
    for (int a1 = 0; a1 < 3; ++a1)
#pragma unroll
      for (int a0 = 0; a0 < 3; ++a0) r[a1][a0] = cb[(a1 - 1) * pw + (a0 - 1)];
#pragma unroll
    for (int a1 = 0; a1 < 3; ++a1)
#pragma unroll
      for (int a0 = 0; a0 < 3; ++a0)
        if (__double_as_longlong(r[a1][a0]) == PA_CP_MISSING) { ok = false; r[a1][a0] = 0.0; }
    if (!ok) atomicAdd(nbad, ((int)(u > 0) + (int)(u + 1 < n0 - 1)) * ((int)(v > 0) + (int)(v + 1 < n1 - 1)));
  }
  const bool odd = Fx.A.bc[FD] == PA_BC_REFLECT_ODD;
  constexpr double nc0 = k_cf_coef.nrm[4][0], nc1 = k_cf_coef.nrm[4][1], nc2 = k_cf_coef.nrm[4][2], nc3 = k_cf_coef.nrm[4][3];
#pragma unroll
  for (int dv = 0; dv < 2; ++dv)
#pragma unroll
    for (int du = 0; du < 2; ++du) {
      const double nfd1 = nfd[dv][du][0], nfd2 = nfd[dv][du][1], nfd3 = nfd[dv][du][2];
      double g;
      if (wall) {
        g = odd ? -nfd1 : nfd1;
      } else {
        const double c00 = du ? k_cf_coef.tan[1][1][1][0] : k_cf_coef.tan[0][1][1][0], c01 = du ? k_cf_coef.tan[1][1][1][1] : k_cf_coef.tan[0][1][1][1],
                     c02 = du ? k_cf_coef.tan[1][1][1][2] : k_cf_coef.tan[0][1][1][2];
        const double c10 = dv ? k_cf_coef.tan[1][1][1][0] : k_cf_coef.tan[0][1][1][0], c11 = dv ? k_cf_coef.tan[1][1][1][1] : k_cf_coef.tan[0][1][1][1],
                     c12 = dv ? k_cf_coef.tan[1][1][1][2] : k_cf_coef.tan[0][1][1][2];
        const double xi0 = du ? 0.25 : -0.25, xi1 = dv ? 0.25 : -0.25;
        double b0 = 0.0;
        b0 += c00 * r[1][0];
        b0 += c01 * r[1][1];
        b0 += c02 * r[1][2];
        b0 += c10 * r[0][1];
        b0 += c11 * r[1][1];
        b0 += c12 * r[2][1];
        b0 -= r[1][1];
        b0 += ((xi0 * xi1) * 0.25) * (((r[2][2] - r[2][0]) + r[0][0]) - r[0][2]);
        double tmp = 0.0;
        tmp += nfd1 * nc1;
        tmp += nfd2 * nc2;
        tmp += nfd3 * nc3;
        g = tmp;
        g += b0 * nc0;
      }
      const double f1 = side ? cdiff(L.dxinv[FD], nfd2, nfd1, g) : cdiff(L.dxinv[FD], g, nfd1, nfd2);
      const double t01 = pre ? t01n[dv][du] : cdiff(L.dxinv[T0], A0[dv][du], A0[dv][du + 1], A0[dv][du + 2]);
      const double t11 = pre ? t11n[dv][du] : cdiff(L.dxinv[T1], A1[du][dv], A1[du][dv + 1], A1[du][dv + 2]);
      double k1 = 0.0;
      k1 += (FD == 0) ? f1 : t01;
      k1 += (FD == 1) ? f1 : (FD == 0 ? t01 : t11);
      k1 += (FD == 2) ? f1 : t11;
      k1 = k1 * 0.5;
      const int uu = u + du, vv = v + dv;
      if (uu > 0 && uu < n0 - 1 && vv > 0 && vv < n1 - 1) ko[dv * s1 + du * s0] = k1;
    }
}


template <int FD>
__device__ __forceinline__ void fix_chunk_mixed(const FixArgs& Fx, const SfChunk& D, int z, int* nbad, const double* tabs) {
  constexpr int T0 = (FD == 0) ? 1 : 0, T1 = (FD == 2) ? 1 : 2;
  const int side = D.dir_side & 1;
  const DMFView& MO = Fx.MO;
  const DLevelView& L = Fx.L;
  const int n[3] = {D.hi[0] - D.lo[0] + 1, D.hi[1] - D.lo[1] + 1, D.hi[2] - D.lo[2] + 1};
  const int n0 = n[T0], n1 = n[T1];
  const int hw = D.cw >> 1, sh = 31 - __builtin_clz((unsigned)hw);
  const int u = D.u0 + 2 * ((int)threadIdx.x & (hw - 1)), v = D.v0 + 2 * ((int)threadIdx.x >> sh);
  if (u >= n0 || v >= n1) return;
  const int ng = MO.ng, ncomp0 = Fx.ncomp0 + 8 * z, kcomp = Fx.kcomp + 8 * z;
  const long long nxo = n[0] + 2 * ng, nyo = n[1] + 2 * ng, nzo = n[2] + 2 * ng;
  const long long cso = pa_cstride(nxo * nyo * nzo, MO.ncomp);
  const long long st[3] = {1, nxo, nxo * nyo};
  int X1[3];
  X1[FD] = side ? D.hi[FD] : D.lo[FD];
  X1[T0] = D.lo[T0] + u;
  X1[T1] = D.lo[T1] + v;
  const long long idx1 = ((long long)(X1[2] - D.lo[2] + ng) * nyo + (X1[1] - D.lo[1] + ng)) * nxo + (X1[0] - D.lo[0] + ng);
  const long long in = side ? -st[FD] : st[FD], s0 = st[T0], s1 = st[T1];
  double* const o = MO.data + MO.off[D.box];
  const double* const nf = o + (long long)(ncomp0 + FD) * cso + idx1;
  const double* const n0p = o + (long long)(ncomp0 + T0) * cso + idx1;
  const double* const n1p = o + (long long)(ncomp0 + T1) * cso + idx1;
  double* const ko = o + (long long)kcomp * cso + idx1;
  DBox B;
#pragma unroll
  for (int d = 0; d < 3; ++d) { B.lo[d] = D.lo[d]; B.hi[d] = D.hi[d]; }
  const bool pre = FD == 0 && Fx.ncg && z == 0 && ncg_face_ok(B, side, Fx.ncg_minw);
  bool live[2][2];
  long long off[2][2], cgo[2][2];
  unsigned code[2][2];
  const int ulo = min(1, n0 - 1), uhi = max(n0 - 2, 0), vlo = min(1, n1 - 1), vhi = max(n1 - 2, 0);
#pragma unroll
  for (int dv = 0; dv < 2; ++dv)
#pragma unroll
    for (int du = 0; du < 2; ++du) {
      const int uu = u + du, vv = v + dv;
      live[dv][du] = uu > 0 && uu < n0 - 1 && vv > 0 && vv < n1 - 1;
      const int uc = min(max(uu, ulo), uhi), vc = min(max(vv, vlo), vhi);
      off[dv][du] = (long long)(vc - v) * s1 + (long long)(uc - u) * s0;
      cgo[dv][du] = (long long)(vc + 1) * (n0 + 2) + (uc + 1);
      code[dv][du] = L.sfcode[D.sfoff + (long long)vc * n0 + uc];
    }
  if (n0 < 3 || n1 < 3) return;
  const bool cf_here = (D.flags & PA_SFC_HAS_CF) != 0;
  CfBlock K;
  if (cf_here) {
    int plane, pu0, pv0, pw, ph;
    cpatch_geom(B, FD, side, plane, pu0, pv0, pw, ph);
    cf_block_load(L.cp + z * Fx.cp_stride + D.cpoff + (long long)((X1[T1] >> 1) - pv0) * pw + ((X1[T0] >> 1) - pu0), pw, K);
  }
  double nfd[2][2][3], a0[2][2][3], a1[2][2][3], t01n[2][2], t11n[2][2];
  if (pre) {
    const pa_fix_d2* np = (const pa_fix_d2*)(Fx.ncg + 2 * D.cgoff);
#pragma unroll
    for (int dv = 0; dv < 2; ++dv)
#pragma unroll
      for (int du = 0; du < 2; ++du) {
        const pa_fix_d2 v0 = np[cgo[dv][du]], v1 = np[Fx.ncgs + cgo[dv][du]], v2 = np[2 * Fx.ncgs + cgo[dv][du]];
        nfd[dv][du][0] = v0.x; nfd[dv][du][1] = v0.y; nfd[dv][du][2] = v1.x; t01n[dv][du] = v1.y; t11n[dv][du] = v2.x;
      }
  } else {
#pragma unroll
    for (int dv = 0; dv < 2; ++dv)
#pragma unroll
      for (int du = 0; du < 2; ++du) {
#pragma unroll
        for (int m = 0; m < 3; ++m) nfd[dv][du][m] = nf[off[dv][du] + m * in];
#pragma unroll
        for (int k = 0; k < 3; ++k) {
          a0[dv][du][k] = n0p[off[dv][du] + (k - 1) * s0];
          a1[dv][du][k] = n1p[off[dv][du] + (k - 1) * s1];
        }
      }
  }
  if (cf_here) cf_block_finish(K);
  const bool odd = Fx.A.bc[FD] == PA_BC_REFLECT_ODD;
  constexpr double nc0 = k_cf_coef.nrm[4][0], nc1 = k_cf_coef.nrm[4][1], nc2 = k_cf_coef.nrm[4][2], nc3 = k_cf_coef.nrm[4][3];
  int nbad_here = 0;
#pragma unroll
  for (int dv = 0; dv < 2; ++dv)
#pragma unroll
    for (int du = 0; du < 2; ++du) {
      const unsigned cd = live[dv][du] ? code[dv][du] : 2u;
      const int cls = (int)(cd & 3u);
      const double nfd1 = nfd[dv][du][0], nfd2 = nfd[dv][du][1], nfd3 = nfd[dv][du][2];
      double g = odd ? -nfd1 : nfd1;
      bool write = live[dv][du];
      if (cf_here) {
        double b[1];
        const bool bad = cf_block_interp<1>(K, cd, du, dv, tabs, 0.0, 1.0, b);
        double tmp = 0.0;
        tmp += nfd1 * nc1;
        tmp += nfd2 * nc2;
        tmp += nfd3 * nc3;
        double h = tmp;
        h += b[0] * nc0;
        g = cls == 1 ? h : g;
        nbad_here += (cls == 1 && bad) ? 1 : 0;
      }
      if (cls == 0) {
        int q0[3] = {X1[0], X1[1], X1[2]};
        q0[FD] += side ? 1 : -1;
        q0[T0] += du;
        q0[T1] += dv;
        int sbn = -1, qw[3];
        if (classify(L, q0[0], q0[1], q0[2], sbn, qw) == 0 && sbn >= 0) g = MO.data[MO.off[sbn] + fab_index(L.boxes[sbn], MO.ng, MO.ncomp, ncomp0 + FD, qw[0], qw[1], qw[2])];
        else write = false;
      }
      const double f1 = side ? cdiff(L.dxinv[FD], nfd2, nfd1, g) : cdiff(L.dxinv[FD], g, nfd1, nfd2);
      const double t01 = pre ? t01n[dv][du] : cdiff(L.dxinv[T0], a0[dv][du][0], a0[dv][du][1], a0[dv][du][2]);
      const double t11 = pre ? t11n[dv][du] : cdiff(L.dxinv[T1], a1[dv][du][0], a1[dv][du][1], a1[dv][du][2]);
      double k1 = 0.0;
      k1 += (FD == 0) ? f1 : t01;
      k1 += (FD == 1) ? f1 : (FD == 0 ? t01 : t11);
      k1 += (FD == 2) ? f1 : t11;
      k1 = k1 * 0.5;
      if (write) ko[off[dv][du]] = k1;
    }
  if (nbad_here) atomicAdd(nbad, nbad_here);
}

struct LevChunks { const SfChunk* ck[PA_MAXB]; unsigned w0[PA_MAXB + 1]; };
template <bool PATCH>
__global__ __launch_bounds__(256) void k_faces_fix_chunks(LevBatch<FixArgs> Bt, LevChunks Ck, int* nbad, SlotK sk, unsigned nperim) {
  if (blockIdx.x < nperim) { faces_tab_wg<true, PATCH, false>(Bt, nbad, sk, blockIdx.x); return; }
  const unsigned wx = blockIdx.x - nperim;
  int blev = 0;
  while (blev + 1 < Bt.n && wx >= Ck.w0[blev + 1]) ++blev;
  const FixArgs& Fx = Bt.a[blev];
  const SfChunk D = Ck.ck[blev][wx - Ck.w0[blev]];
  const int dir = D.dir_side >> 1;
  const int e0 = D.hi[0] - D.lo[0] + 1, e1 = D.hi[1] - D.lo[1] + 1, e2 = D.hi[2] - D.lo[2] + 1;
  const int blen = dir == 0 ? e0 : (dir == 1 ? e1 : e2), n0 = dir == 0 ? e1 : e0, n1 = dir == 2 ? e1 : e2;
  const bool cfok = Fx.A.has_crse && Fx.A.ratio == 2 && Fx.use_cp && Fx.L.cp && D.cpoff >= 0;
  const bool straight = blen >= 3 && ((D.flags & PA_SFC_WALL) != 0 || ((D.flags & PA_SFC_FULL) != 0 && cfok));
  const bool mixed = !straight && blen >= 3 && (cfok || !(D.flags & PA_SFC_HAS_CF));
  if (straight) {
    switch (dir) {
      case 0: fix_chunk_uniform<0>(Fx, D, (int)blockIdx.z, nbad); break;
      case 1: fix_chunk_uniform<1>(Fx, D, (int)blockIdx.z, nbad); break;
      default: fix_chunk_uniform<2>(Fx, D, (int)blockIdx.z, nbad); break;
    }
    return;
  }
  if (mixed) {
    __shared__ double tabs[54];
    cf_tab_to_lds(tabs);
    switch (dir) {
      case 0: fix_chunk_mixed<0>(Fx, D, (int)blockIdx.z, nbad, tabs); break;
      case 1: fix_chunk_mixed<1>(Fx, D, (int)blockIdx.z, nbad, tabs); break;
      default: fix_chunk_mixed<2>(Fx, D, (int)blockIdx.z, nbad, tabs); break;
    }
    return;
  }
  const int hw = D.cw >> 1, sh = 31 - __builtin_clz((unsigned)hw);
  const int u = D.u0 + 2 * ((int)threadIdx.x & (hw - 1)), v = D.v0 + 2 * ((int)threadIdx.x >> sh);
  for (int dv = 0; dv < 2; ++dv)
    for (int du = 0; du < 2; ++du)
      if (u + du >= 0 && v + dv >= 0 && u + du < n0 && v + dv < n1) faces_fast_cell<1, PATCH, false>(Bt, nbad, SlowList(), sk, blev, (unsigned)D.face, (long long)(v + dv) * n0 + (u + du));
}

template <int NL, bool PATCH = false, bool CLIP = false>
__global__ __launch_bounds__(256) void k_faces_curv_fast(LevBatch<FixArgs> Bt, int* nbad, SlowList sl = SlowList(), SlotK sk = SlotK()) {
  faces_fast_wg<NL, PATCH, CLIP>(Bt, nbad, sl, sk, blockIdx.x);
}
static int fused_kseg() { return 64; }
static dim3 march_grid(int nx, int ny, int nz, int kseg, int mty, unsigned nboxes) {
  const unsigned tx = (nx + 63) / 64, ty = (ny + mty - 1) / mty, tz = (nz + kseg - 1) / kseg;
  return dim3(tx * ty * tz, nboxes);
}
static int fused_order() { return 2; }
template <typename BP>
static void march_launch(hipStream_t st, const BP& bp, int nx, int ny, int nz, unsigned nboxes, const MarchArgs& A0, bool  = false, std::string* kname = nullptr) {
  MarchArgs A = A0;
  {
    const long long per_seg = (long long)((nx + 63) / 64) * ((ny + 12) / 13) * nboxes;
    if (per_seg * ((nz + A.kseg - 1) / A.kseg) < 2048) {
      long long best = -1;
      int best_k = A.kseg;
      for (int tz = 1; tz <= std::max(1, nz / 8); ++tz) {
        const int k = (nz + tz - 1) / tz;
        const long long rounds = (per_seg * ((nz + k - 1) / k) + 255) / 256, cost = rounds * (k + 4);
        if (best < 0 || cost < best) { best = cost; best_k = k; }
      }
      A.kseg = std::max(best_k, 4);
    }
  }
  A.order = fused_order();
  A.nboxes = (int)nboxes;
  const bool clip = A.thr >= 0.0;
  if (nx <= 32) {
    constexpr int NRW = 8;
    const unsigned tiles = (unsigned)(((nx + 31) / 32) * ((ny + 2 * NRW - 1) / (2 * NRW)) * ((nz + A.kseg - 1) / A.kseg));
    A.tiles_max = (int)tiles;
    const dim3 g(tiles * 8u * ((nboxes + 7u) / 8u), 1);
    if (A.cg && clip) hipLaunchKernelGGL((k_gradcurv_march3n<BP, NRW, true, true>), g, dim3(64 * (NRW + 2)), 0, st, bp, A);
    else if (A.cg) hipLaunchKernelGGL((k_gradcurv_march3n<BP, NRW, false, true>), g, dim3(64 * (NRW + 2)), 0, st, bp, A);
    else if (clip) hipLaunchKernelGGL((k_gradcurv_march3n<BP, NRW, true>), g, dim3(64 * (NRW + 2)), 0, st, bp, A);
    else hipLaunchKernelGGL((k_gradcurv_march3n<BP, NRW, false>), g, dim3(64 * (NRW + 2)), 0, st, bp, A);
    if (kname) *kname = std::string("k_gradcurv_march3n<NRW=8,CLIP=") + (clip ? "1" : "0") + ",CG=" + (A.cg ? "1>" : "0>");
    return;
  }
  auto go = [&](auto mc) {
    constexpr int M = decltype(mc)::value;
    dim3 g = march_grid(nx, ny, nz, A.kseg, M, nboxes);
    A.txy_max = ((nx + 63) / 64) * ((ny + M - 1) / M);
    A.tiles_max = (int)g.x;
    g = dim3(g.x * 8u * ((nboxes + 7u) / 8u), 1);
    if (kname) *kname = "k_gradcurv_march3<MTY=" + std::to_string(M) + ",CLIP=" + std::to_string((int)clip) + ",PAIR=0,CG=" + std::to_string((int)(A.cg != 0)) + ">";
    if (A.cg && !clip) hipLaunchKernelGGL((k_gradcurv_march3<BP, M, false, false, 0, true>), g, dim3(64 * (M + 3)), 0, st, bp, A);
    else if (A.cg) hipLaunchKernelGGL((k_gradcurv_march3<BP, M, true, false, 0, true>), g, dim3(64 * (M + 3)), 0, st, bp, A);
    else if (clip) hipLaunchKernelGGL((k_gradcurv_march3<BP, M, true>), g, dim3(64 * (M + 3)), 0, st, bp, A);
    else hipLaunchKernelGGL((k_gradcurv_march3<BP, M, false>), g, dim3(64 * (M + 3)), 0, st, bp, A);
  };
  if (ny >= 52) go(std::integral_constant<int, 13>{});
  else if (ny >= 16) go(std::integral_constant<int, 8>{});
  else go(std::integral_constant<int, 4>{});
}

extern "C" int pa_sweep_occupancy(pa_ctx* ctx, int which) {
  PaBind bind_(ctx);
  if (!ctx) return -1;
  int nb = -1;
  hipError_t e = which == 0 ? hipOccupancyMaxActiveBlocksPerMultiprocessor(&nb, k_gradcurv_march3_levels<13, false>, 64 * 16, 0)
                            : hipOccupancyMaxActiveBlocksPerMultiprocessor(&nb, k_gradcurv_march3n_levels<8, false>, 64 * 10, 0);
  if (e != hipSuccess) { (void)hipGetLastError(); return -1; }
  return nb;
}

extern "C" int pa_gradcurv_level(pa_ctx* ctx, const pa_mf* phi, int pcomp, double pmin, double pmax, double thr, pa_mf* out, int ocomp) {
  PaBind bind_(ctx);
  if (!ctx || !phi || !out) return pa_fail(ctx, "pa_gradcurv_level: null argument");
  if (phi->lev != out->lev) return pa_fail(ctx, "pa_gradcurv_level: different levels");
  if (phi->ng < 2) return pa_fail(ctx, "pa_gradcurv_level: phi needs >= 2 ghost layers");
  if (pcomp < 0 || pcomp >= phi->ncomp || ocomp < 0 || ocomp + 8 > out->ncomp) return pa_fail(ctx, "pa_gradcurv_level: component range");
  if (!(pmax > pmin)) return pa_fail(ctx, "pa_gradcurv_level: progress variable has no range");
  const pa_level* L = phi->lev;
  if (phi->lev->boxes.empty()) return 0;
  LevelBP2 bp{L->view, phi->view, out->view};
  MarchArgs A{pcomp, ocomp, fused_kseg(), pmin, 1.0 / (pmax - pmin), thr, 0, 1, 1, 1};
  ProfScope prof(ctx, PA_TAG_GRADCURV);
  march_launch(ctx->stream, bp, L->maxn[0], L->maxn[1], L->maxn[2], (unsigned)L->boxes.size(), A, false, &ctx->sweep_kernel);
  PA_HIP(hipGetLastError());
  return 0;
}

int pa_gradcurv_faces_phase(pa_ctx* ctx, const pa_mf* c, int ccomp, const pa_mf* crse_n, int cncomp0, const int32_t bc[3], int ratio, double thr,
                            pa_mf* out, int ncomp0, int kcomp, int phase);
extern "C" int pa_gradcurv_faces_level(pa_ctx* ctx, const pa_mf* c, int ccomp, const pa_mf* crse_n, int cncomp0, const int32_t bc[3],
                                       int ratio, double thr, pa_mf* out, int ncomp0, int kcomp) {
  PaBind bind_(ctx);
  return pa_gradcurv_faces_phase(ctx, c, ccomp, crse_n, cncomp0, bc, ratio, thr, out, ncomp0, kcomp, 3);
}
int pa_gradcurv_faces_phase(pa_ctx* ctx, const pa_mf* c, int ccomp, const pa_mf* crse_n, int cncomp0, const int32_t bc[3], int ratio, double thr,
                            pa_mf* out, int ncomp0, int kcomp, int phase) {
  if (!ctx || !c || !out) return pa_fail(ctx, "pa_gradcurv_faces_level: null argument");
  if (c->lev != out->lev) return pa_fail(ctx, "pa_gradcurv_faces_level: different levels");
  if (c->ng < 2) return pa_fail(ctx, "pa_gradcurv_faces_level: c needs >= 2 ghost layers");
  if (ccomp >= c->ncomp || kcomp >= out->ncomp || ncomp0 + 3 > out->ncomp || (crse_n && cncomp0 + 3 > crse_n->ncomp))
    return pa_fail(ctx, "pa_gradcurv_faces_level: component range");
  if (crse_n && ratio != 2) return pa_fail(ctx, "pa_gradcurv_faces_level: only refinement ratio 2 is supported");
  const pa_level* L = c->lev;
  for (const DBox& B : L->boxes)
    for (int d = 0; d < 3; ++d)
      if (crse_n && B.hi[d] - B.lo[d] + 1 < 3) return pa_fail(ctx, "pa_gradcurv_faces_level: boxes thinner than 3 cells need the pass-by-pass path");
  if (crse_n && (phase & 2) && pa_coarse_source(ctx, L, crse_n, cncomp0, 3, 0, 0, 0, &crse_n, &cncomp0)) return 1;
  FaceArgs A;
  for (int d = 0; d < 3; ++d) A.bc[d] = bc[d];
  A.ratio = ratio; A.has_crse = crse_n ? 1 : 0; A.thr = thr; A.layers = 2; A.perim_only = 0; A.pmin = 0.0; A.invd = 1.0;
  bool fast = !(thr >= 0.0);
  for (const DBox& B : c->lev->boxes)
    for (int d = 0; d < 3; ++d) fast = fast && (B.hi[d] - B.lo[d] + 1 >= 3);
  constexpr int fast_env = 1;
  fast = fast && fast_env;
  if (L->sfaces.empty()) return 0;
  const long long n0 = L->maxn[0], n1 = L->maxn[1], n2 = L->maxn[2];
  const long long nf = std::max(n1 * n2, std::max(n0 * n2, n0 * n1));
  const unsigned nsf = (unsigned)L->sfaces.size();
  ProfScope prof(ctx, PA_TAG_GRADCURV_FACES);
  if (phase & 1) hipLaunchKernelGGL(k_faces_normal, dim3((unsigned)((nf + 255) / 256), nsf), dim3(256), 0, ctx->stream, L->view, c->view, ccomp, out->view, ncomp0, A);
  if (!(phase & 2)) {
    PA_HIP(hipGetLastError());
    return 0;
  }
  LevBatch<FixArgs> Bt;
  Bt.n = 1;
  Bt.ycum[1] = (int)nsf;
  Bt.a[0] = FixArgs{L->view, c->view, ccomp, crse_n ? crse_n->lev->view : L->view, crse_n ? crse_n->view : c->view, cncomp0, out->view, ncomp0, kcomp, A};
  Bt.a[0].wg = (const int2*)L->d_sfwg;
  Bt.a[0].nwg = L->nsfwg;
  if (fast) {
    hipLaunchKernelGGL(k_faces_curv_fast<2>, dim3((unsigned)L->nsfwg), dim3(256), 0, ctx->stream, Bt, ctx->d_flags);
    Bt.a[0].A.perim_only = 1;
  }
  const long long ncell = fast ? 2 * (std::max(n0, std::max(n1, n2)) + std::max(n0, std::max(n1, n2))) : nf;
  hipLaunchKernelGGL(k_faces_curv<false>, dim3((unsigned)((ncell * A.layers + 255) / 256), nsf), dim3(256), 0, ctx->stream, Bt, ctx->d_flags);
  PA_HIP(hipGetLastError());
  return 0;
}

extern "C" int pa_gradcurv_fab(pa_ctx* ctx, pa_box valid, const pa_fab* phi, int pcomp, double pmin, double pmax, const double dxinv[3],
                               double thr, pa_fab* out, int ocomp) {
  PaBind bind_(ctx);
  if (!ctx || !phi || !out || !dxinv) return pa_fail(ctx, "pa_gradcurv_fab: null argument");
  std::string why;
  if (!fab_covers(*phi, valid, 2, pcomp, 1, why) || !fab_covers(*out, valid, 0, ocomp, 8, why)) return pa_fail(ctx, "pa_gradcurv_fab: " + why);
  if (!(pmax > pmin)) return pa_fail(ctx, "pa_gradcurv_fab: progress variable has no range");
  FabBP2 bp{fab_view(*phi), fab_view(*out), to_dbox(valid), {dxinv[0], dxinv[1], dxinv[2]}};
  MarchArgs A{pcomp, ocomp, fused_kseg(), pmin, 1.0 / (pmax - pmin), thr, 0, 1, 1, 1};
  march_launch(ctx->stream, bp, valid.hi[0] - valid.lo[0] + 1, valid.hi[1] - valid.lo[1] + 1, valid.hi[2] - valid.lo[2] + 1, 1, A);
  PA_HIP(hipGetLastError());
  return 0;
// ... 244 lines not shown
        double b[2];
        const bool bad = cf_block_interp<2>(K, cd, du, dv, tabs, xa, xb, b);
        double tp = 0.0, tc = 0.0;
        tp += f[dv][du][0] * nc1;  tc += ((f[dv][du][0] - A.pmin) * A.invd) * nc1;
        tp += f[dv][du][1] * nc2;  tc += ((f[dv][du][1] - A.pmin) * A.invd) * nc2;
        tp += f[dv][du][2] * nc3;  tc += ((f[dv][du][2] - A.pmin) * A.invd) * nc3;
        double hp = tp, hc = tc;
        hp += b[0] * nc0;
        hc += b[1] * nc0;
        gp = cls == 1 ? hp : gp;
        gc = cls == 1 ? hc : gc;
        nbad_here += (cls == 1 && bad) ? 1 : 0;
      }
      if (in[dv][du] && cls != 0) {
        p[iq + off[dv][du]] = gp;
        if (!PHIONLY) cgp[dv * (n0 + 2) + du] = gc;
      }
    }
  if (nbad_here) atomicAdd(nbad, nbad_here);
  if (!PHIONLY && any_valid) {
#pragma unroll
    for (int dv = 0; dv < 2; ++dv)
#pragma unroll
      for (int du = 0; du < 2; ++du) {
        if (!(in[dv][du] && (code[dv][du] & 3u) == 0u)) continue;
        int qq[3] = {q[0], q[1], q[2]};
        qq[t0] += du;
        qq[t1] += dv;
        int sb, xw[3];
        double x;
        if (classify(L, qq[0], qq[1], qq[2], sb, xw) == 0 && sb >= 0) x = M.data[M.off[sb] + fab_index(L.boxes[sb], M.ng, M.ncomp, comp, xw[0], xw[1], xw[2])];
        else x = p[iq + off[dv][du]];
        cgp[dv * (n0 + 2) + du] = (x - A.pmin) * A.invd;
      }
  }
}

struct RingItem { int b, q[3], w , ef, code, pad; };
__global__ __launch_bounds__(256) void k_find_ring(DLevelView L, const int* sfboxes, int nsfboxes, RingItem* items, int* count, int cap) {
  const int b = sfboxes[blockIdx.y];
  const DBox B = L.boxes[b];
  const int n[3] = {B.hi[0] - B.lo[0] + 1, B.hi[1] - B.lo[1] + 1, B.hi[2] - B.lo[2] + 1};
  long long t = blockIdx.x * (long long)blockDim.x + threadIdx.x;
  int e = -1, which = 0, pos = 0;
  for (int d = 0; d < 3; ++d) {
    if (t < 4LL * n[d]) { e = d; which = (int)((unsigned)t / (unsigned)n[d]); pos = (int)((unsigned)t % (unsigned)n[d]); break; }
    t -= 4LL * n[d];
  }
  if (e < 0) return;
  const int a = (e == 0) ? 1 : 0, c = (e == 2) ? 1 : 2;
  const int sa = which & 1, sc = which >> 1;
  int q[3];
  q[e] = B.lo[e] + pos;
  q[a] = sa ? B.hi[a] + 1 : B.lo[a] - 1;
  q[c] = sc ? B.hi[c] + 1 : B.lo[c] - 1;
  const int cls = classify(L, q[0], q[1], q[2]);
  if (cls == 0) return;
  int qa[3] = {q[0], q[1], q[2]}, qc[3] = {q[0], q[1], q[2]};
  qa[a] += sa ? -1 : 1;
  qc[c] += sc ? -1 : 1;
  const bool va = classify(L, qa[0], qa[1], qa[2]) == 0;
  const bool vc = classify(L, qc[0], qc[1], qc[2]) == 0;
  if (va == vc) return;
  const int dir = va ? a : c, sd = va ? sa : sc;
  if (cls == 2 && !((q[dir] < L.domlo[dir] || q[dir] > L.domhi[dir]) && !L.is_per[dir])) return;
  const int ef = L.sfindex[b * 6 + dir * 2 + sd];
  if (ef < 0) return;
  const int i = atomicAdd(count, 1);
  if (items && i < cap) {
    RingItem R;
    R.b = b; R.q[0] = q[0]; R.q[1] = q[1]; R.q[2] = q[2]; R.w = dir | (sd << 2) | (cls << 3); R.ef = ef;
    R.code = cls == 1 ? (int)(cf_masks(L, q, dir, 2) | 1u) : 0;
    R.pad = 0;
    items[i] = R;
  }
}

template <bool PATCH, bool DIRECT>
__device__ __forceinline__ void prep_ring_item(const PrepLev& Pl, const RingItem& R, int* nbad, const SlotK& sk) {
  const DLevelView& L = Pl.L;
  const DMFView& M = Pl.M;
  const DLevelView& LC = Pl.LC;
  const int z = (int)blockIdx.z;
  DMFView MC = Pl.MC;
  PrepArgs A = Pl.A;
  if (sk.prog) { A.pmin = MC.xa = sk.prog[2 * z]; A.invd = MC.xb = sk.prog[2 * z + 1]; }
  const int comp = Pl.comp + z, ccomp = Pl.ccomp + z;
  double* const cgz = L.cg + z * Pl.cg_stride;
  const double* const cpz = L.cp ? L.cp + z * Pl.cp_stride : nullptr;
  const int b = R.b, dir = R.w & 3, sd = (R.w >> 2) & 1, cls = R.w >> 3, ef = R.ef;
  const int q[3] = {R.q[0], R.q[1], R.q[2]};
  const DBox B = L.boxes[b];
  const int n[3] = {B.hi[0] - B.lo[0] + 1, B.hi[1] - B.lo[1] + 1, B.hi[2] - B.lo[2] + 1};
  const int s = sd ? -1 : 1;
  if (cls == 1 && !A.has_crse) { atomicAdd(nbad, 1); return; }
  const double* p = M.data + M.off[b];
  auto phi_at = [&](const int x[3]) -> double {
    if (DIRECT) {
      int sb, xw[3];
      if (classify(L, x[0], x[1], x[2], sb, xw) == 0 && sb >= 0) return M.data[M.off[sb] + fab_index(L.boxes[sb], M.ng, M.ncomp, comp, xw[0], xw[1], xw[2])];
    }
    return p[fab_index(B, M.ng, M.ncomp, comp, x[0], x[1], x[2])];
  };
  double g;
  if (cls == 2) {
    int in[3] = {q[0], q[1], q[2]};
    in[dir] += s;
    const double v = (phi_at(in) - A.pmin) * A.invd;
    g = (A.bc[dir] == PA_BC_REFLECT_ODD) ? -v : v;
  } else {
    bool ok = true;
    double coef[4];
    const int NX = cf_normal_coef(n[dir], A.ratio, coef);
    double bv;
    const long long cpo = (Pl.use_cp && L.cp) ? L.cpoff[ef] : -1;
    if (PATCH || cpo >= 0) {
      const int xf[1] = {MC.xform};
      double b1[1];
      cf_interp_patch<1>((unsigned)R.code, cpz + cpo, B, sd, MC, q, dir, xf, ok, b1);
      bv = b1[0];
    } else {
      const int xf[1] = {MC.xform};
      double b1[1];
      cf_interp<1>((unsigned)R.code, LC, MC, ccomp, q, dir, A.ratio, xf, ok, b1);
      bv = b1[0];
    }
    if (!ok) atomicAdd(nbad, 1);
    double tmp = 0.0;
    for (int m = 1; m < NX; ++m) {
      int pc[3] = {q[0], q[1], q[2]};
      pc[dir] += s * m;
      tmp += ((phi_at(pc) - A.pmin) * A.invd) * coef[m];
    }
    g = tmp;
    g += bv * coef[0];
  }
  const int t0 = (dir == 0) ? 1 : 0, t1 = (dir == 2) ? 1 : 2;
  cgz[L.cgoff[ef] + (long long)(q[t1] - B.lo[t1] + 1) * (B.hi[t0] - B.lo[t0] + 3) + (q[t0] - B.lo[t0] + 1)] = g;
}
struct LevRings { const RingItem* it[PA_MAXB]; unsigned n[PA_MAXB]; unsigned w0[PA_MAXB + 1]; };
template <bool PATCH, bool DIRECT>
__device__ __forceinline__ void prep_ring_wg(const LevBatch<PrepLev>& Bt, const LevRings& Rg, int* nbad, const SlotK& sk, unsigned w) {
  int blev = 0;
  while (blev + 1 < Bt.n && w >= Rg.w0[blev + 1]) ++blev;
  const unsigned i = (w - Rg.w0[blev]) * 256u + threadIdx.x;
  if (i >= Rg.n[blev]) return;
  prep_ring_item<PATCH, DIRECT>(Bt.a[blev], Rg.it[blev][i], nbad, sk);
}
template <bool PATCH, bool DIRECT = false>
__global__ __launch_bounds__(256) void k_prep_ring(LevBatch<PrepLev> Bt, LevRings Rg, int* nbad, SlotK sk = SlotK()) {
  prep_ring_wg<PATCH, DIRECT>(Bt, Rg, nbad, sk, blockIdx.x);
}

template <bool PATCH, bool PHIONLY = false>
__global__ __launch_bounds__(256) void k_prep_faces_chunks(LevBatch<PrepLev> Bt, LevChunks Ck, LevRings Rg, int* nbad, SlotK sk = SlotK()) {
  const unsigned nrw = Rg.w0[Bt.n];
  if (blockIdx.x < nrw) { if (!PHIONLY) prep_ring_wg<PATCH, true>(Bt, Rg, nbad, sk, blockIdx.x); return; }
  const unsigned wx = blockIdx.x - nrw;
  int blev = 0;
  while (blev + 1 < Bt.n && wx >= Ck.w0[blev + 1]) ++blev;
  const PrepLev& Pl = Bt.a[blev];
  const SfChunk D = Ck.ck[blev][wx - Ck.w0[blev]];
  const int dir = D.dir_side >> 1;
  const int e0 = D.hi[0] - D.lo[0] + 1, e1 = D.hi[1] - D.lo[1] + 1, e2 = D.hi[2] - D.lo[2] + 1;
  const int blen = dir == 0 ? e0 : (dir == 1 ? e1 : e2), n0 = dir == 0 ? e1 : e0, n1 = dir == 2 ? e1 : e2;
  const bool cfok = Pl.A.has_crse && Pl.A.ratio == 2 && Pl.use_cp && Pl.L.cp && D.cpoff >= 0 && blen >= 3;
  const bool straight = (D.flags & PA_SFC_WALL) != 0 || ((D.flags & PA_SFC_FULL) != 0 && cfok);
  const bool mixed = !straight && blen >= 3 && (cfok || !(D.flags & PA_SFC_HAS_CF));
  if (straight || mixed) {
    __shared__ double tabs[54];
    if (mixed) cf_tab_to_lds(tabs);
    const int z = (int)blockIdx.z;
    PrepArgs A = Pl.A;
    double xa = Pl.MC.xa, xb = Pl.MC.xb;
    if (sk.prog) { A.pmin = xa = sk.prog[2 * z]; A.invd = xb = sk.prog[2 * z + 1]; }
    double* const cgz = PHIONLY ? nullptr : Pl.L.cg + z * Pl.cg_stride;
    const double* const cpz = Pl.L.cp ? Pl.L.cp + z * Pl.cp_stride : nullptr;
    if (straight) {
      switch (dir) {
        case 0: prep_chunk_uniform<0, PHIONLY>(Pl, D, A, xa, xb, Pl.comp + z, cgz, cpz, nbad); break;
        case 1: prep_chunk_uniform<1, PHIONLY>(Pl, D, A, xa, xb, Pl.comp + z, cgz, cpz, nbad); break;
        default: prep_chunk_uniform<2, PHIONLY>(Pl, D, A, xa, xb, Pl.comp + z, cgz, cpz, nbad); break;
      }
    } else {
      switch (dir) {
        case 0: prep_chunk_mixed<0, PHIONLY>(Pl, D, A, xa, xb, Pl.comp + z, cgz, cpz, nbad, tabs); break;
        case 1: prep_chunk_mixed<1, PHIONLY>(Pl, D, A, xa, xb, Pl.comp + z, cgz, cpz, nbad, tabs); break;
        default: prep_chunk_mixed<2, PHIONLY>(Pl, D, A, xa, xb, Pl.comp + z, cgz, cpz, nbad, tabs); break;
      }
    }
    return;
  }
  const int hw = D.cw >> 1, sh = 31 - __builtin_clz((unsigned)hw);
  const int u = D.u0 + 2 * ((int)threadIdx.x & (hw - 1)), v = D.v0 + 2 * ((int)threadIdx.x >> sh);
  for (int dv = 0; dv < 2; ++dv)
    for (int du = 0; du < 2; ++du)
      if (u + du >= 0 && v + dv >= 0 && u + du < n0 && v + dv < n1) prep_faces_cell<PATCH, PHIONLY>(Pl, nbad, sk, (unsigned)D.face, (long long)(v + dv) * n0 + (u + du));
}

static int level_cg(pa_ctx* ctx, const pa_level* Lc, int nsets = 1) {
  pa_level* L = const_cast<pa_level*>(Lc);
  if (L->d_cg && L->cg_sets >= nsets) return 0;
  if (L->d_cg) {
    PA_HIP(hipStreamSynchronize(ctx->stream));
    if (ctx->stream2) PA_HIP(hipStreamSynchronize(ctx->stream2));
    (void)hipFree(L->d_cg);
    L->d_cg = nullptr;
  }
  const size_t n = (size_t)std::max<long long>(L->cg_total, 8) * (size_t)nsets;
  PA_HIP(hipMalloc(&L->d_cg, sizeof(double) * n));
  PA_HIP(hipMemsetAsync(L->d_cg, 0, sizeof(double) * n, ctx->stream));
  L->cg_sets = nsets;
  L->view.cg = L->d_cg;
  return 0;
}
static long long cg_stride(const pa_level* L) { return std::max<long long>(L->cg_total, 8); }
static int level_ncg(pa_ctx* ctx, const pa_level* Lc) {
  pa_level* L = const_cast<pa_level*>(Lc);
  if (L->d_ncg) return 0;
  const size_t n = 6 * (size_t)std::max<long long>(L->cg_total, 8);
  if (hipMalloc(&L->d_ncg, sizeof(double) * n) != hipSuccess) { L->d_ncg = nullptr; return pa_fail(ctx, "compact first-layer arrays: device allocation failed"); }
  PA_HIP(hipMemsetAsync(L->d_ncg, 0, sizeof(double) * n, ctx->stream));
  return 0;
}
static long long cp_stride(const pa_level* L) { return std::max<long long>(L->cp_total, 8); }
static int level_ring(pa_ctx* ctx, const pa_level* Lc) {
  pa_level* L = const_cast<pa_level*>(Lc);
  if (L->nring >= 0) return 0;
  if (L->nsfboxes == 0 || L->sfaces.empty()) { L->nring = 0; return 0; }
  int* d_count = nullptr;
  auto fail = [&](const char* what) {
    if (d_count) (void)hipFree(d_count);
    if (L->d_ring) { (void)hipFree(L->d_ring); L->d_ring = nullptr; }
    (void)hipGetLastError();
    return pa_fail(ctx, std::string("ring list: ") + what);
  };
  if (hipMalloc(&d_count, sizeof(int)) != hipSuccess) return fail("device allocation failed");
  const long long nt = 4LL * (L->maxn[0] + L->maxn[1] + L->maxn[2]);
  int n = 0;
  for (int pass = 0; pass < 2; ++pass) {
    if (pass == 1) {
      if (n == 0) break;
      if (hipMalloc(&L->d_ring, sizeof(RingItem) * (size_t)n) != hipSuccess) { L->d_ring = nullptr; return fail("device allocation failed"); }
    }
    if (hipMemsetAsync(d_count, 0, sizeof(int), ctx->stream) != hipSuccess) return fail("memset failed");
    for (int y0 = 0; y0 < L->nsfboxes; y0 += 65535)
      hipLaunchKernelGGL(k_find_ring, dim3((unsigned)((nt + 255) / 256), (unsigned)std::min(65535, L->nsfboxes - y0)), dim3(256), 0, ctx->stream, L->view, L->d_sfboxes + y0,
                         L->nsfboxes - y0, pass ? (RingItem*)L->d_ring : nullptr, d_count, n);
    int m = 0;
    if (hipMemcpyAsync(&m, d_count, sizeof(int), hipMemcpyDeviceToHost, ctx->stream) != hipSuccess || hipStreamSynchronize(ctx->stream) != hipSuccess) return fail("reading the count failed");
    if (pass == 1 && m != n) return fail("the two passes disagree");
    n = m;
  }
  (void)hipFree(d_count);
  d_count = nullptr;
  if (n > 1) {
    std::vector<RingItem> h((size_t)n);
    if (hipMemcpy(h.data(), L->d_ring, sizeof(RingItem) * (size_t)n, hipMemcpyDeviceToHost) != hipSuccess) return fail("download failed");
    std::sort(h.begin(), h.end(), [](const RingItem& a, const RingItem& b) {
      if (a.ef != b.ef) return a.ef < b.ef;
      if (a.q[2] != b.q[2]) return a.q[2] < b.q[2];
      if (a.q[1] != b.q[1]) return a.q[1] < b.q[1];
      return a.q[0] < b.q[0];
    });
    if (hipMemcpy(L->d_ring, h.data(), sizeof(RingItem) * (size_t)n, hipMemcpyHostToDevice) != hipSuccess) return fail("upload failed");
  }
  L->nring = n;
  return 0;
}


struct CpLev { DLevelView L; DLevelView LC; DMFView MC; int ccomp, by_dir; long long cp_stride = 0; int zstride = 1; };
__global__ __launch_bounds__(256) void k_cpatch(LevBatch<CpLev> Bt) {
  unsigned fy;
  const CpLev& P = Bt.a[Bt.find(blockIdx.y, fy)];
  const DLevelView& L = P.L;
  const long long off = L.cpoff[fy];
  if (off < 0) return;
  const int e = L.sfaces[fy], dir = (e % 6) >> 1, side = e & 1;
  const DBox B = L.boxes[e / 6];
  int plane, u0, v0, pw, ph;
  cpatch_geom(B, dir, side, plane, u0, v0, pw, ph);
  const unsigned t = blockIdx.x * 256u + threadIdx.x;
  if (t >= (unsigned)(pw * ph)) return;
  const int t0 = dir == 0 ? 1 : 0, t1 = dir == 2 ? 1 : 2;
  const unsigned r = t / (unsigned)pw;
  int p[3];
  p[dir] = plane; p[t0] = u0 + (int)(t - r * (unsigned)pw); p[t1] = v0 + (int)r;
  double v = __longlong_as_double(PA_CP_MISSING);
  const int z = (int)blockIdx.z;
  if (wrap_cell(P.LC, p)) {
    const int cb = owner_of(P.LC, p);
    if (cb >= 0) v = P.MC.data[P.MC.off[cb] + fab_index(P.LC.boxes[cb], P.MC.ng, P.MC.ncomp, P.ccomp + P.zstride * z + (P.by_dir ? dir : 0), p[0], p[1], p[2])];
  }
  L.cp[z * P.cp_stride + off + t] = v;
}
struct CprLev { DLevelView L; DLevelView LC; DMFView MC; const int* regs; const int* wgs; int nwg, ccomp, by_dir; long long cp_stride = 0; int zstride = 1; };
__global__ __launch_bounds__(256) void k_cpatch_regions(LevBatch<CprLev> Bt) {
  const CprLev& P = Bt.a[blockIdx.y];
  if ((int)blockIdx.x >= P.nwg) return;
  const int* R = P.regs + 12 * P.wgs[2 * blockIdx.x];
  const unsigned t = (unsigned)P.wgs[2 * blockIdx.x + 1] * 256u + threadIdx.x, nu = (unsigned)R[7];
  if (t >= nu * (unsigned)R[8]) return;
  const unsigned b = nu == 1 ? t : __umulhi(t, (unsigned)R[10]), a = t - b * nu;
  const int dir = R[9], t0 = dir == 0 ? 1 : 0, t1 = dir == 2 ? 1 : 2;
  const DLevelView& L = P.L;
  const int e = L.sfaces[R[0]], side = e & 1;
  int plane, u0, v0, pw, ph;
  cpatch_geom(L.boxes[e / 6], dir, side, plane, u0, v0, pw, ph);
  int p[3] = {R[4], R[5], R[6]};
  p[t0] += (int)a; p[t1] += (int)b;
  const int z = (int)blockIdx.z;
  L.cp[z * P.cp_stride + L.cpoff[R[0]] + (long long)(R[3] + (int)b) * pw + (R[2] + (int)a)] =
      P.MC.data[P.MC.off[R[1]] + fab_index(P.LC.boxes[R[1]], P.MC.ng, P.MC.ncomp, P.ccomp + P.zstride * z + (P.by_dir ? dir : 0), p[0], p[1], p[2])];
}
__global__ __launch_bounds__(256) void k_cpatch_clear(double* cp, long long n) {
  const long long t = blockIdx.x * 256LL + threadIdx.x;
  if (t < n) cp[t] = __longlong_as_double(PA_CP_MISSING);
}
static int level_cp(pa_ctx* ctx, const pa_level* Lc, int nsets = 1) {
  pa_level* L = const_cast<pa_level*>(Lc);
  if (L->d_cp && L->cp_sets >= nsets) return 0;
  if (L->d_cp) {
    PA_HIP(hipStreamSynchronize(ctx->stream));
    if (ctx->stream2) PA_HIP(hipStreamSynchronize(ctx->stream2));
    (void)hipFree(L->d_cp);
    L->d_cp = nullptr;
  }
  const long long n = cp_stride(L) * nsets;
  PA_HIP(hipMalloc(&L->d_cp, sizeof(double) * (size_t)n));
  hipLaunchKernelGGL(k_cpatch_clear, dim3((unsigned)((n + 255) / 256)), dim3(256), 0, ctx->stream, L->d_cp, n);
  L->cp_sets = nsets;
  L->view.cp = L->d_cp;
  return 0;
}
static bool cpatch_on() { return true; }
static int cpatch_launch(pa_ctx* ctx, int l0, int l1, pa_mf* const* fine, const pa_mf* const* crse, int ccomp, int by_dir, int nslots = 1, int zstride = 1) {
  {
    LevBatch<CprLev> Br;
    bool regions = true;
    int mw = 0;
    for (int l = l0; l < l1 && regions; ++l) {
      const pa_level* L = fine[l]->lev;
      if (!crse[l] || L->boxes.empty() || L->sfaces.empty() || L->cp_total == 0) continue;
      if (level_cp(ctx, L, nslots)) return 1;
      const CpPlan* P = pa_cp_plan(ctx, L, crse[l]->lev);
      regions = P && P->ok;
      if (!regions || P->nwg == 0) continue;
      Br.a[Br.n] = CprLev{L->view, crse[l]->lev->view, crse[l]->view, P->d_regs, P->d_wgs, P->nwg, ccomp, by_dir, cp_stride(L), zstride};
      ++Br.n;
// ... 296 lines not shown
          double gv = tmp;
          gv += bv * coef[0];
          nb[s2] = gv;
        }
      }
      curv += cdiff(dxinv[d], nb[0], n0d, nb[1]);
    }
    curv = curv * 0.5;
    if (!ok) atomicAdd(nbad, 1);
    *kout = curv;
  }
}
template <bool CLIP, bool GEN = true, bool PATCH = false>
__global__ __launch_bounds__(256) void k_curv_general(GenLev G, int* nbad, SlotK sk) {
  curv_general_body<CLIP, GEN, PATCH>(G, nbad, sk, blockIdx.x * 256LL + threadIdx.x, gridDim.x * 256LL);
}
struct GenBatch { int n; unsigned wg0[PA_MAXB + 1]; GenLev a[PA_MAXB]; };
static_assert(sizeof(GenBatch) + sizeof(SlotK) + 16 <= 4000, "kernel arguments of k_curv_general_levels");
template <bool CLIP, bool GEN, bool PATCH>
__global__ __launch_bounds__(256) void k_curv_general_levels(GenBatch Bt, int* nbad, SlotK sk) {
  int l = 0;
  while (l + 1 < Bt.n && blockIdx.x >= Bt.wg0[l + 1]) ++l;
  const GenLev G = Bt.a[l];
  curv_general_body<CLIP, GEN, PATCH>(G, nbad, sk, (long long)(blockIdx.x - Bt.wg0[l]) * 256 + threadIdx.x, 1LL << 40);
}

bool pa_fused2_level_ok(const pa_level* L) {
  const std::vector<DBox>& all = L->gboxes.empty() ? L->boxes : L->gboxes;
  for (const DBox& B : all)
    for (int d = 0; d < 3; ++d)
      if (B.hi[d] - B.lo[d] + 1 < 3) return false;
  return true;
}

struct GaussFixLev { DLevelView L; DMFView G, O; int pc, kgc; double thr; const SfChunk* ck; unsigned nck; const int4* irr; unsigned nirr; unsigned w0; };
__device__ __forceinline__ void gauss_cell(const GaussFixLev& A, int b, int i, int j, int k) {
  const DBox V = A.L.boxes[b];
  const FabView G = mf_view(A.G, V, b), O = mf_view(A.O, V, b);
  double H[3][3], g[3];
#pragma unroll
  for (int d = 0; d < 3; ++d) {
    const double c0 = G(i, j, k, d);
    g[d] = c0;
    H[d][0] = cdiff(A.L.dxinv[0], G(i - 1, j, k, d), c0, G(i + 1, j, k, d));
    H[d][1] = cdiff(A.L.dxinv[1], G(i, j - 1, k, d), c0, G(i, j + 1, k, d));
    H[d][2] = cdiff(A.L.dxinv[2], G(i, j, k - 1, d), c0, G(i, j, k + 1, d));
  }
  const double ax0 = H[1][1] * H[2][2] - H[2][1] * H[1][2];
  const double ay0 = H[1][2] * H[2][0] - H[2][2] * H[1][0];
  const double az0 = H[1][0] * H[2][1] - H[2][0] * H[1][1];
  const double ax1 = H[0][2] * H[2][1] - H[2][2] * H[0][1];
  const double ay1 = H[0][0] * H[2][2] - H[2][0] * H[0][2];
  const double az1 = H[0][1] * H[2][0] - H[2][1] * H[0][0];
  const double ax2 = H[0][1] * H[1][2] - H[1][1] * H[0][2];
  const double ay2 = H[0][2] * H[1][0] - H[1][2] * H[0][0];
  const double az2 = H[0][0] * H[1][1] - H[1][0] * H[0][1];
  const double cx = g[0], cy = g[1], cz = g[2];
  const double sn = sqrt(cx * cx + cy * cy + cz * cz);
  const double gn = (1e-14 < sn) ? sn : 1e-14;
  double kg = (cx * (ax0 * cx + ax1 * cy + ax2 * cz) + cy * (ay0 * cx + ay1 * cy + ay2 * cz) + cz * (az0 * cx + az1 * cy + az2 * cz)) / ((gn * gn) * (gn * gn));
  if (A.thr >= 0.0) {
    const double p = O(i, j, k, A.pc);
    if (p < A.thr || p > 1.0 - A.thr) kg = 0.0;
  }
  O(i, j, k, A.kgc) = kg;
}
__global__ __launch_bounds__(256) void k_gauss_cells(LevBatch<GaussFixLev> Bt) {
  int l = 0;
  while (l + 1 < Bt.n && blockIdx.x >= Bt.a[l + 1].w0) ++l;
  const GaussFixLev& A = Bt.a[l];
  const unsigned w = blockIdx.x - A.w0;
  if (w < A.nck) {
    const SfChunk D = A.ck[w];
    const int dir = D.dir_side >> 1, side = D.dir_side & 1;
    const int e0 = D.hi[0] - D.lo[0] + 1, e1 = D.hi[1] - D.lo[1] + 1, e2 = D.hi[2] - D.lo[2] + 1;
    const int n0 = dir == 0 ? e1 : e0, n1 = dir == 2 ? e1 : e2;
    const int sh = 31 - __builtin_clz((unsigned)D.cw);
#pragma unroll 2
    for (int r = 0; r < 4; ++r) {
      const int c = (int)threadIdx.x + 256 * r;
      const int uu = D.u0 + (c & (D.cw - 1)), vv = D.v0 + (c >> sh);
      if (uu < 0 || vv < 0 || uu >= n0 || vv >= n1) continue;
      int i, j, k;
      if (dir == 0) { i = side ? D.hi[0] : D.lo[0]; j = D.lo[1] + uu; k = D.lo[2] + vv; }
      else if (dir == 1) { i = D.lo[0] + uu; j = side ? D.hi[1] : D.lo[1]; k = D.lo[2] + vv; }
      else { i = D.lo[0] + uu; j = D.lo[1] + vv; k = side ? D.hi[2] : D.lo[2]; }
      gauss_cell(A, D.box, i, j, k);
    }
    return;
  }
  const unsigned q = (w - A.nck) * 256u + threadIdx.x;
  if (q < A.nirr) {
    const int4 it = A.irr[q];
    gauss_cell(A, it.x, it.y, it.z, it.w);
  }
}
int pa_gauss_cells_levels(pa_ctx* ctx, int nlev, pa_mf* const* G, pa_mf* const* out, int pc, int kgc, double thr) {
  for (int l0 = 0; l0 < nlev; l0 += PA_MAXB) {
    LevBatch<GaussFixLev> Bt;
    unsigned w = 0;
    for (int l = l0; l < nlev && l < l0 + PA_MAXB; ++l) {
      const pa_level* L = out[l]->lev;
      if (L->boxes.empty()) continue;
      if (G[l]->lev != L || G[l]->ng < 1 || G[l]->ncomp < 3) return pa_fail(ctx, "pa_gauss_cells_levels: G needs 3 components and a ghost layer on the level of out");
      if (L->nirr < 0 && level_irregular(ctx, L)) return 1;
      GaussFixLev A{L->view, G[l]->view, out[l]->view, pc, kgc, thr, L->d_sfchunk, (unsigned)L->nsfchunk, (const int4*)L->d_irr, (unsigned)std::max(L->nirr, 0), w};
      w += A.nck + (A.nirr + 255u) / 256u;
      Bt.a[Bt.n++] = A;
    }
    if (!Bt.n || w == 0) continue;
    hipLaunchKernelGGL(k_gauss_cells, dim3(w), dim3(256), 0, ctx->stream, Bt);
  }
  PA_HIP(hipGetLastError());
  return 0;
}

int pa_gradcurv_prep_levels(pa_ctx* ctx, int nlev, pa_mf* const* phi, int comp, const pa_mf* const* crse, int ccomp, const int32_t bc[3], double pmin, double pmax, int phase,
                            int nslots, const double* prog) {
  bool direct = (phase & 4) != 0;
  for (int l = 0; l < nlev; ++l) direct = direct && phi[l]->lev->nranks == 1;
  SlotK sk;
  sk.prog = prog;
  const bool use_cp = cpatch_on();
  for (int l0 = 0; l0 < nlev; l0 += PA_MAXB) {
    if (use_cp && (phase & 1) && cpatch_launch(ctx, l0, std::min(nlev, l0 + PA_MAXB), phi, crse, ccomp, 0, nslots, 1)) return 1;
    LevBatch<PrepLev> Bf;
    const pa_level* batch_lev[PA_MAXB] = {};
    long long ntf = 0;
    for (int l = l0; l < nlev && l < l0 + PA_MAXB; ++l) {
      const pa_level* L = phi[l]->lev;
      if (L->boxes.empty()) continue;
      if (!(phase & 8) && level_cg(ctx, L, nslots)) return 1;
      if (L->sfaces.empty()) continue;
      PrepLev P;
      P.cg_stride = cg_stride(L); P.cp_stride = cp_stride(L);
      for (int d = 0; d < 3; ++d) P.A.bc[d] = bc[d];
      P.A.ratio = 2; P.A.has_crse = crse[l] ? 1 : 0; P.A.pmin = pmin; P.A.invd = 1.0 / (pmax - pmin);
      P.L = L->view; P.M = phi[l]->view; P.comp = comp;
      P.LC = crse[l] ? crse[l]->lev->view : L->view;
      P.MC = crse[l] ? crse[l]->view : phi[l]->view;
      P.MC.xform = 1; P.MC.xa = pmin; P.MC.xb = P.A.invd;
      P.ccomp = ccomp;
      P.use_cp = (use_cp && crse[l] && L->cp_total > 0) ? 1 : 0;
      P.wg = (const int2*)L->d_sfwg; P.nwg = L->nsfwg; P.sfboxes = L->d_sfboxes;
      const long long n0 = L->maxn[0], n1 = L->maxn[1], n2 = L->maxn[2];
      ntf = std::max(ntf, std::max(n1 * n2, std::max(n0 * n2, n0 * n1)));
      batch_lev[Bf.n] = L;
      Bf.a[Bf.n] = P; Bf.ycum[Bf.n + 1] = Bf.ycum[Bf.n] + (int)L->sfaces.size(); ++Bf.n;
    }
    if (!Bf.n) continue;
    ProfScope prof(ctx, PA_TAG_BC);
    bool all_patch = true;
    for (int q = 0; q < Bf.n; ++q) all_patch = all_patch && (Bf.a[q].use_cp || !Bf.a[q].A.has_crse);
    LevChunks Ck;
    Ck.w0[0] = 0;
    for (int q = 0; q < Bf.n; ++q) {
      const pa_level* Lq = batch_lev[q];
      if (!Lq->d_sfchunk || Lq->nsfchunk <= 0) return pa_fail(ctx, "pa_gradcurv_prep_levels: a level without chunk records");
      Ck.ck[q] = Lq->d_sfchunk;
      Ck.w0[q + 1] = Ck.w0[q] + (unsigned)Lq->nsfchunk;
    }
    LevRings Rg, Rnone;
    Rg.w0[0] = 0;
    for (int q = 0; q <= PA_MAXB; ++q) Rnone.w0[q] = 0;
    for (int q = 0; q < PA_MAXB; ++q) { Rnone.it[q] = nullptr; Rnone.n[q] = 0; }
    if (phase & 2)
      for (int q = 0; q < Bf.n; ++q) {
        const pa_level* Lq = batch_lev[q];
        if (level_ring(ctx, Lq)) return 1;
        Rg.it[q] = (const RingItem*)Lq->d_ring;
        Rg.n[q] = (unsigned)Lq->nring;
        Rg.w0[q + 1] = Rg.w0[q] + (unsigned)((Lq->nring + 255) / 256);
      }
    const bool ring_with_faces = (phase & 1) && (phase & 2) && !(phase & 8) && direct && Rg.w0[Bf.n] * 8u <= Ck.w0[Bf.n];
    if (phase & 1) {
      const LevRings& Rk = ring_with_faces ? Rg : Rnone;
      const dim3 gc(Rk.w0[Bf.n] + Ck.w0[Bf.n], 1, (unsigned)nslots);
      if (phase & 8) {
        if (all_patch) hipLaunchKernelGGL((k_prep_faces_chunks<true, true>), gc, dim3(256), 0, ctx->stream, Bf, Ck, Rk, ctx->d_flags, sk);
        else hipLaunchKernelGGL((k_prep_faces_chunks<false, true>), gc, dim3(256), 0, ctx->stream, Bf, Ck, Rk, ctx->d_flags, sk);
      } else {
        if (all_patch) hipLaunchKernelGGL((k_prep_faces_chunks<true, false>), gc, dim3(256), 0, ctx->stream, Bf, Ck, Rk, ctx->d_flags, sk);
        else hipLaunchKernelGGL((k_prep_faces_chunks<false, false>), gc, dim3(256), 0, ctx->stream, Bf, Ck, Rk, ctx->d_flags, sk);
      }
    }
    if ((phase & 2) && !ring_with_faces && Rg.w0[Bf.n] > 0) {
      const dim3 gr(Rg.w0[Bf.n], 1, (unsigned)nslots);
      if (all_patch && direct) hipLaunchKernelGGL((k_prep_ring<true, true>), gr, dim3(256), 0, ctx->stream, Bf, Rg, ctx->d_flags, sk);
      else if (direct) hipLaunchKernelGGL((k_prep_ring<false, true>), gr, dim3(256), 0, ctx->stream, Bf, Rg, ctx->d_flags, sk);
      else if (all_patch) hipLaunchKernelGGL(k_prep_ring<true>, gr, dim3(256), 0, ctx->stream, Bf, Rg, ctx->d_flags, sk);
      else hipLaunchKernelGGL(k_prep_ring<false>, gr, dim3(256), 0, ctx->stream, Bf, Rg, ctx->d_flags, sk);
    }
  }
  PA_HIP(hipGetLastError());
  return 0;
}

struct SweepGroup { int lev; const int* list; int n; int dims[3]; };
static void sweep_groups(int l, const pa_level* L, std::vector<SweepGroup>& out) {
  if (L->boxes.empty()) return;
  if (!L->d_blist) { out.push_back({l, nullptr, (int)L->boxes.size(), {L->maxn[0], L->maxn[1], L->maxn[2]}}); return; }
  out.push_back({l, L->d_blist, L->nwide, {L->wmax[0], L->wmax[1], L->wmax[2]}});
  out.push_back({l, L->d_blist + L->nwide, L->nnarrow, {L->nmax[0], L->nmax[1], L->nmax[2]}});
}

static const WgTab* sweep_wgtab(const pa_level* L, const SweepGroup& g, int tw, int mty, int kseg, int part = 0, bool force = false) {
  if (!part && g.n <= 0) return nullptr;
  return pa_sweep_wgtab(L, !g.list ? 2 : (g.list == L->d_blist ? 0 : 1), tw, mty, kseg, force, part);
}

static int sweep_group_cg(pa_ctx* ctx, const SweepGroup& g, const pa_mf* phi, int pcomp, double pmin, double pmax, pa_mf* out, int ocomp, double thr, int slot) {
  const pa_level* L = phi->lev;
  if (level_cg(ctx, L, slot + 1)) return 1;
  LevelBP2 bp{L->view, phi->view, out->view};
  bp.L.cg += slot * cg_stride(L);
  MarchArgs A{pcomp, ocomp, fused_kseg(), pmin, 1.0 / (pmax - pmin), thr >= 0.0 ? thr : -1.0, 0, 1, 1, 1};
  A.cg = 1;
  A.boxlist = g.list;
  ProfScope prof(ctx, PA_TAG_GRADCURV);
  march_launch(ctx->stream, bp, g.dims[0], g.dims[1], g.dims[2], (unsigned)g.n, A, false, &ctx->sweep_kernel);
  PA_HIP(hipGetLastError());
  return 0;
}
int pa_gradcurv_level_cg(pa_ctx* ctx, const pa_mf* phi, int pcomp, double pmin, double pmax, pa_mf* out, int ocomp, double thr, int slot) {
  std::vector<SweepGroup> gs;
  sweep_groups(0, phi->lev, gs);
  for (const SweepGroup& g : gs)
    if (sweep_group_cg(ctx, g, phi, pcomp, pmin, pmax, out, ocomp, thr, slot)) return 1;
  return 0;
}

bool pa_gradcurv_gout_ok(int nlev, pa_mf* const* phi);
bool pa_gradcurv_parts_ok(int nlev, pa_mf* const* phi) { return pa_gradcurv_gout_ok(nlev, phi); }
bool pa_gradcurv_kg_ok(int nlev, pa_mf* const* phi) {
  if (!pa_gradcurv_gout_ok(nlev, phi)) return false;
  for (int l = 0; l < nlev; ++l) {
    const pa_level* L = phi[l]->lev;
    if (L->boxes.empty()) continue;
    if (L->nnarrow > 0 || L->maxn[1] < 16) return false;
    for (const DBox& B : L->boxes)
      if (B.hi[0] - B.lo[0] + 1 <= 32) return false;
  }
  return true;
}
bool pa_gradcurv_gout_ok(int nlev, pa_mf* const* phi) {
  if (pa_opt().force_fallbacks) return false;
  std::vector<SweepGroup> all;
  for (int l = 0; l < nlev; ++l) sweep_groups(l, phi[l]->lev, all);
  return all.size() <= 8 * PA_MAXB;
}

int pa_gradcurv_levels_cg(pa_ctx* ctx, int nlev, pa_mf* const* phi, int pcomp, double pmin, double pmax, pa_mf* const* out, int ocomp, double thr, int slot,
                          int nslots, const double* prog, const double* pmins, const double* pmaxs, pa_mf* const* gout, int part, int kg) {
  const bool clip = thr >= 0.0;
  if (kg && (!gout || !pa_gradcurv_kg_ok(nlev, phi))) return pa_fail(ctx, "pa_gradcurv_levels_cg: the Gaussian curvature inside the sweep needs the G-output sweeps of wide boxes");
  if (part && !pa_gradcurv_parts_ok(nlev, phi)) return pa_fail(ctx, "pa_gradcurv_levels_cg: this hierarchy's sweeps cannot be split into early and late tiles");
  if (nslots > 1 && (slot != 0 || !prog || !pmins || !pmaxs)) return pa_fail(ctx, "pa_gradcurv_levels_cg: component slots need slot 0 and the progress ranges");
  if (gout && (nslots != 1 || slot != 0 || !pa_gradcurv_gout_ok(nlev, phi))) return pa_fail(ctx, "pa_gradcurv_levels_cg: the G-output sweeps take one component of a hierarchy pa_gradcurv_gout_ok accepts");
  std::vector<SweepGroup> all, lv, rest;
  for (int l = 0; l < nlev; ++l) sweep_groups(l, phi[l]->lev, all);
  for (int l = 0; l < nlev; ++l) const_cast<pa_level*>(phi[l]->lev)->ncg_live = false;
  bool any_ncg = false;
  int mty = 0;
  bool same = true;
  for (const SweepGroup& g : all) {
    if (g.dims[0] <= 32) { rest.push_back(g); continue; }
    const int m = g.dims[1] >= 52 ? 13 : (g.dims[1] >= 16 ? 8 : 4);
    same = same && (mty == 0 || m == mty);
    mty = m;
    lv.push_back(g);
  }
  (void)same;
  const bool ok = !lv.empty() && lv.size() <= 8u * PA_MAXB && !pa_opt().force_fallbacks;
  if (!ok) {
    rest.insert(rest.begin(), lv.begin(), lv.end());
    lv.clear();
  }
  const std::vector<SweepGroup> lv_all = lv;
  bool nar_side = false;
  for (const SweepGroup& g : rest) nar_side = nar_side || g.dims[0] <= 32;
  nar_side = nar_side && !lv_all.empty() && part == 0 && !pa_opt().force_fallbacks && phi[0]->lev->nranks == 1;
  if (nar_side) {
    if (!ctx->stream2) PA_HIP(hipStreamCreateWithFlags(&ctx->stream2, hipStreamNonBlocking));
    while (ctx->sync_evs.size() < 5) {
      hipEvent_t e;
      PA_HIP(hipEventCreateWithFlags(&e, hipEventDisableTiming));
      ctx->sync_evs.push_back(e);
    }
    PA_HIP(hipEventRecord(ctx->sync_evs[3], ctx->stream));
    PA_HIP(hipStreamWaitEvent(ctx->stream2, ctx->sync_evs[3], 0));
  }
  for (int pass_i = 0; pass_i < 3 * 8; ++pass_i) {
    const int mty_pass = pass_i / 8 == 0 ? 13 : (pass_i / 8 == 1 ? 8 : 4), chunk = pass_i % 8;
    std::vector<SweepGroup> lvm, lv;
    for (const SweepGroup& g : lv_all)
      if ((g.dims[1] >= 52 ? 13 : (g.dims[1] >= 16 ? 8 : 4)) == mty_pass) lvm.push_back(g);
    for (size_t q = (size_t)chunk * PA_MAXB; q < lvm.size() && q < (size_t)(chunk + 1) * PA_MAXB; ++q) lv.push_back(lvm[q]);
    if (lv.empty()) continue;
    const int mty = mty_pass;
    SweepBatch S;
    S.n = (int)lv.size();
    S.wg0[0] = 0;
    std::vector<long long> per_seg(lv.size());
    long long wgs = 0;
    const int kdef = fused_kseg();
    for (size_t q = 0; q < lv.size(); ++q) {
      per_seg[q] = (long long)((lv[q].dims[0] + 63) / 64) * ((lv[q].dims[1] + mty - 1) / mty) * (long long)lv[q].n;
      wgs += per_seg[q] * ((lv[q].dims[2] + kdef - 1) / kdef);
    }
    int tz_best = 0;
    if (wgs < 2048) {
      long long best = -1;
      int nzmax = 0;
      for (const SweepGroup& g : lv) nzmax = std::max(nzmax, g.dims[2]);
      for (int tz = 1; tz <= std::max(1, nzmax / 8); ++tz) {
        long long w = 0;
        int kmax = 0;
        for (size_t q = 0; q < lv.size(); ++q) {
          const int nz = lv[q].dims[2], k = std::max(4, (nz + tz - 1) / tz);
          w += per_seg[q] * ((nz + k - 1) / k);
          kmax = std::max(kmax, k);
        }
        const long long cost = ((w + 255) / 256) * (kmax + 4);
        if (best < 0 || cost < best) { best = cost; tz_best = tz; }
      }
    }
    for (size_t q = 0; q < lv.size(); ++q) {
      const int l = lv[q].lev;
      const pa_level* L = phi[l]->lev;
      if (level_cg(ctx, L, slot + nslots)) return 1;
      S.bp[q] = LevelBP2{L->view, phi[l]->view, out[l]->view};
      S.bp[q].L.cg += slot * cg_stride(L);
      S.cgs[q] = cg_stride(L);
      MarchArgs A{pcomp, ocomp, kdef, pmin, 1.0 / (pmax - pmin), clip ? thr : -1.0, 2, 1, 1, 1};
      A.cg = 1;
      {
        if (pa_opt().ncg && !clip && nslots == 1 && slot == 0 && !L->sfaces.empty()) {
// ... 29 lines not shown
    S.prog = nslots > 1 ? prog : nullptr;
    const dim3 grid(S.wg0[S.n], (unsigned)nslots);
    if (gout && kg) {
      if (clip) {
        if (mty == 13) hipLaunchKernelGGL((k_gradcurv_march3_levels<13, true, 2>), grid, dim3(64 * 16), 0, ctx->stream, S);
        else hipLaunchKernelGGL((k_gradcurv_march3_levels<8, true, 2>), grid, dim3(64 * 11), 0, ctx->stream, S);
      } else {
        if (mty == 13) hipLaunchKernelGGL((k_gradcurv_march3_levels<13, false, 2>), grid, dim3(64 * 16), 0, ctx->stream, S);
        else hipLaunchKernelGGL((k_gradcurv_march3_levels<8, false, 2>), grid, dim3(64 * 11), 0, ctx->stream, S);
      }
    } else if (gout) {
      if (clip) {
        if (mty == 13) hipLaunchKernelGGL((k_gradcurv_march3_levels<13, true, true>), grid, dim3(64 * 16), 0, ctx->stream, S);
        else if (mty == 8) hipLaunchKernelGGL((k_gradcurv_march3_levels<8, true, true>), grid, dim3(64 * 11), 0, ctx->stream, S);
        else hipLaunchKernelGGL((k_gradcurv_march3_levels<4, true, true>), grid, dim3(64 * 7), 0, ctx->stream, S);
      } else {
        if (mty == 13) hipLaunchKernelGGL((k_gradcurv_march3_levels<13, false, true>), grid, dim3(64 * 16), 0, ctx->stream, S);
        else if (mty == 8) hipLaunchKernelGGL((k_gradcurv_march3_levels<8, false, true>), grid, dim3(64 * 11), 0, ctx->stream, S);
        else hipLaunchKernelGGL((k_gradcurv_march3_levels<4, false, true>), grid, dim3(64 * 7), 0, ctx->stream, S);
      }
    } else if (clip) {
      if (mty == 13) hipLaunchKernelGGL((k_gradcurv_march3_levels<13, true>), grid, dim3(64 * 16), 0, ctx->stream, S);
      else if (mty == 8) hipLaunchKernelGGL((k_gradcurv_march3_levels<8, true>), grid, dim3(64 * 11), 0, ctx->stream, S);
      else hipLaunchKernelGGL((k_gradcurv_march3_levels<4, true>), grid, dim3(64 * 7), 0, ctx->stream, S);
    } else {
      if (mty == 13) hipLaunchKernelGGL(k_gradcurv_march3_levels<13>, grid, dim3(64 * 16), 0, ctx->stream, S);
      else if (mty == 8) hipLaunchKernelGGL(k_gradcurv_march3_levels<8>, grid, dim3(64 * 11), 0, ctx->stream, S);
      else hipLaunchKernelGGL(k_gradcurv_march3_levels<4>, grid, dim3(64 * 7), 0, ctx->stream, S);
    }
    PA_HIP(hipGetLastError());
  }
  if (part == 1) return 0;
  std::vector<SweepGroup> nar;
  {
    std::vector<SweepGroup> keep;
    for (const SweepGroup& g : rest) (g.dims[0] <= 32 ? nar : keep).push_back(g);
    if (!nar.empty() && !pa_opt().force_fallbacks) rest.swap(keep);
    else nar.clear();
  }
  const std::vector<SweepGroup> nar_all = nar;
  for (size_t n0 = 0; n0 < nar_all.size(); n0 += PA_MAXB) {
    const std::vector<SweepGroup> nar(nar_all.begin() + (long)n0, nar_all.begin() + (long)std::min(nar_all.size(), n0 + PA_MAXB));
    constexpr int NRW = 8;
    SweepBatch S;
    S.n = (int)nar.size();
    S.wg0[0] = 0;
    for (size_t q = 0; q < nar.size(); ++q) {
      const int l = nar[q].lev;
      const pa_level* L = phi[l]->lev;
      if (level_cg(ctx, L, slot + nslots)) return 1;
      S.bp[q] = LevelBP2{L->view, phi[l]->view, out[l]->view};
      S.bp[q].L.cg += slot * cg_stride(L);
      S.cgs[q] = cg_stride(L);
      MarchArgs A{pcomp, ocomp, fused_kseg(), pmin, 1.0 / (pmax - pmin), clip ? thr : -1.0, 2, 1, 1, 1};
      A.cg = 1;
      A.boxlist = nar[q].list;
      A.nboxes = nar[q].n;
      const int nx = nar[q].dims[0], ny = nar[q].dims[1], nz = nar[q].dims[2];
      {
        const long long per_seg = (long long)((nx + 63) / 64) * ((ny + 12) / 13) * nar[q].n;
        if (per_seg * ((nz + A.kseg - 1) / A.kseg) < 2048) {
          long long best = -1;
          int best_k = A.kseg;
          for (int tz = 1; tz <= std::max(1, nz / 8); ++tz) {
            const int k = (nz + tz - 1) / tz;
            const long long rounds = (per_seg * ((nz + k - 1) / k) + 255) / 256, cost = rounds * (k + 4);
            if (best < 0 || cost < best) { best = cost; best_k = k; }
          }
          A.kseg = std::max(best_k, 4);
        }
      }
      const unsigned tiles = (unsigned)(((nx + 31) / 32) * ((ny + 2 * NRW - 1) / (2 * NRW)) * ((nz + A.kseg - 1) / A.kseg));
      A.tiles_max = (int)tiles;
      const WgTab* wt = sweep_wgtab(L, nar[q], 32, 2 * NRW, A.kseg);
      if (wt) A.wgtab = wt->d;
      if (gout) { A.gdata = gout[l]->data; A.goff = gout[l]->d_off; A.gng = gout[l]->ng; }
      S.A[q] = A;
      S.wg0[q + 1] = S.wg0[q] + (wt ? wt->n : tiles * 8u * (((unsigned)nar[q].n + 7u) / 8u));
    }
    ProfScope prof(ctx, PA_TAG_GRADCURV);
    S.prog = nslots > 1 ? prog : nullptr;
    hipStream_t ns = nar_side ? ctx->stream2 : ctx->stream;
    if (gout && clip) hipLaunchKernelGGL((k_gradcurv_march3n_levels<NRW, true, true>), dim3(S.wg0[S.n], 1u), dim3(64 * (NRW + 2)), 0, ns, S);
    else if (gout) hipLaunchKernelGGL((k_gradcurv_march3n_levels<NRW, false, true>), dim3(S.wg0[S.n], 1u), dim3(64 * (NRW + 2)), 0, ns, S);
    else if (clip) hipLaunchKernelGGL((k_gradcurv_march3n_levels<NRW, true>), dim3(S.wg0[S.n], (unsigned)nslots), dim3(64 * (NRW + 2)), 0, ns, S);
    else hipLaunchKernelGGL((k_gradcurv_march3n_levels<NRW, false>), dim3(S.wg0[S.n], (unsigned)nslots), dim3(64 * (NRW + 2)), 0, ns, S);
    PA_HIP(hipGetLastError());
    if (lv.empty()) ctx->sweep_kernel = "k_gradcurv_march3n_levels<NRW=8" + std::string(clip ? ",CLIP" : "") + ">[" + std::to_string(S.n) + " levels per launch]";
  }
  if (nar_side) {
    PA_HIP(hipEventRecord(ctx->sync_evs[4], ctx->stream2));
    PA_HIP(hipStreamWaitEvent(ctx->stream, ctx->sync_evs[4], 0));
  }
  if (gout && !rest.empty()) return pa_fail(ctx, "pa_gradcurv_levels_cg: a sweep group outside the all-levels launches (G-output variant)");
  for (const SweepGroup& g : rest)
    for (int z = 0; z < nslots; ++z)
      if (sweep_group_cg(ctx, g, phi[g.lev], pcomp + z, nslots > 1 ? pmins[z] : pmin, nslots > 1 ? pmaxs[z] : pmax, out[g.lev], ocomp + 8 * z, thr, slot + z)) return 1;
  if (!lv.empty())
    ctx->sweep_kernel = "k_gradcurv_march3_levels<MTY=" + std::to_string(mty) + (clip ? ",CLIP" : "") + ">[" + std::to_string(lv.size()) + " levels per launch" + (any_ncg ? "; x faces mirrored" : "") + "]" +
                        ((rest.empty() && nar.empty()) ? "" : " + narrow-box launch(es)");
  return 0;
}

int pa_gradcurv_fix_levels(pa_ctx* ctx, int nlev, pa_mf* const* phi, int pcomp, const pa_mf* const* crse_n, int cncomp0, const int32_t bc[3], double pmin, double pmax,
                           pa_mf* const* out, int ncomp0, int kcomp, double thr, int nslots, const double* prog, int cn_z, const pa_mf* const* crse_phi, int cpcomp) {
  SlotK sk;
  sk.prog = prog;
  sk.cn_z = cn_z;
  const bool use_cp = cpatch_on();
  const bool clip = thr >= 0.0;
  auto gen_lev = [&](int l) {
    const pa_level* L = phi[l]->lev;
    GenLev G;
    G.L = L->view; G.MP = phi[l]->view; G.pcomp = pcomp;
    const pa_mf* cp = crse_phi ? crse_phi[l] : nullptr;
    G.LCp = cp ? cp->lev->view : L->view; G.MCp = cp ? cp->view : phi[l]->view; G.cpcomp = cpcomp;
    G.LCn = crse_n[l] ? crse_n[l]->lev->view : L->view; G.MCn = crse_n[l] ? crse_n[l]->view : phi[l]->view; G.cncomp0 = cncomp0;
    G.MO = out[l]->view; G.ncomp0 = ncomp0; G.kcomp = kcomp;
    for (int d = 0; d < 3; ++d) G.A.bc[d] = bc[d];
    G.A.ratio = 2; G.A.has_crse = (crse_n[l] && cp) ? 1 : 0; G.A.thr = clip ? thr : -1.0; G.A.layers = 1; G.A.perim_only = 0; G.A.pmin = pmin; G.A.invd = 1.0 / (pmax - pmin);
    G.items = nullptr; G.n = 0;
    G.use_cp = (use_cp && crse_n[l] && L->cp_total > 0) ? 1 : 0;
    G.cp_stride = cp_stride(L);
    return G;
  };
  for (int l0 = 0; l0 < nlev; l0 += PA_MAXB) {
    if (use_cp && cpatch_launch(ctx, l0, std::min(nlev, l0 + PA_MAXB), phi, crse_n, cncomp0, 1, nslots, cn_z)) return 1;
    LevBatch<FixArgs> Bt;
    int blev[PA_MAXB];
    for (int l = l0; l < nlev && l < l0 + PA_MAXB; ++l) {
      const pa_level* L = phi[l]->lev;
      if (L->boxes.empty() || L->sfaces.empty()) continue;
      blev[Bt.n] = l;
      FaceArgs A;
      for (int d = 0; d < 3; ++d) A.bc[d] = bc[d];
      A.ratio = 2; A.has_crse = crse_n[l] ? 1 : 0; A.thr = clip ? thr : -1.0; A.layers = 1; A.perim_only = 1; A.pmin = pmin; A.invd = 1.0 / (pmax - pmin);
      Bt.a[Bt.n] = FixArgs{L->view, phi[l]->view, pcomp, crse_n[l] ? crse_n[l]->lev->view : L->view, crse_n[l] ? crse_n[l]->view : phi[l]->view, cncomp0,
                           out[l]->view, ncomp0, kcomp, A, (use_cp && crse_n[l] && L->cp_total > 0) ? 1 : 0, cg_stride(L), cp_stride(L), (const int2*)L->d_sfwg, L->nsfwg, (const int2*)L->d_pfwg, L->npfwg};
      if (L->ncg_live) {
        if (!clip && nslots == 1) { Bt.a[Bt.n].ncg = L->d_ncg; Bt.a[Bt.n].ncgs = cg_stride(L); Bt.a[Bt.n].ncg_minw = L->ncg_minw; }
        const_cast<pa_level*>(L)->ncg_live = false;
      }
      Bt.ycum[Bt.n + 1] = Bt.ycum[Bt.n] + (int)L->sfaces.size();
      ++Bt.n;
    }
    if (!Bt.n) continue;
    ProfScope prof(ctx, PA_TAG_GRADCURV_FACES);
    bool all_patch = true;
    for (int q = 0; q < Bt.n; ++q) all_patch = all_patch && (Bt.a[q].use_cp || !Bt.a[q].A.has_crse);
    if (Bt.ycum[Bt.n] >= (1 << 24)) return pa_fail(ctx, "pa_gradcurv_fix_levels: too many special faces in one batch");
    unsigned nwgf = 0;
    for (int q = 0; q < Bt.n; ++q) nwgf += (unsigned)Bt.a[q].nwg;
    const dim3 gfast(nwgf, 1, (unsigned)nslots);
    LevChunks Ck;
    Ck.w0[0] = 0;
    unsigned npt = 0;
    for (int q = 0; q < Bt.n; ++q) {
      const pa_level* Lq = phi[blev[q]]->lev;
      if (!Lq->d_sfchunk || Lq->nsfchunk <= 0 || !Bt.a[q].pwg || Bt.a[q].npwg <= 0) return pa_fail(ctx, "pa_gradcurv_fix_levels: a level without chunk records / perimeter tables");
      Ck.ck[q] = Lq->d_sfchunk;
      Ck.w0[q + 1] = Ck.w0[q] + (unsigned)Lq->nsfchunk;
      npt += (unsigned)Bt.a[q].npwg;
    }
    const dim3 gtab(npt, 1, (unsigned)nslots);
    if (clip) {
      SlowList sl;
      if (pa_slow_list(ctx, &sl)) return 1;
      PA_HIP(hipMemsetAsync(sl.count, 0, 2 * sizeof(int), ctx->stream));
      if (all_patch) hipLaunchKernelGGL((k_faces_curv_fast<1, true, true>), gfast, dim3(256), 0, ctx->stream, Bt, ctx->d_flags, sl, sk);
      else hipLaunchKernelGGL((k_faces_curv_fast<1, false, true>), gfast, dim3(256), 0, ctx->stream, Bt, ctx->d_flags, sl, sk);
      hipStream_t pst = ctx->stream;
      if (ctx->stream2 != ctx->stream) {
        if (!ctx->stream2) PA_HIP(hipStreamCreateWithFlags(&ctx->stream2, hipStreamNonBlocking));
        for (int e = 0; e < 2; ++e)
          if (!ctx->fix_evs[e]) PA_HIP(hipEventCreateWithFlags(&ctx->fix_evs[e], hipEventDisableTiming));
        pst = ctx->stream2;
        PA_HIP(hipEventRecord(ctx->fix_evs[0], ctx->stream));
        PA_HIP(hipStreamWaitEvent(pst, ctx->fix_evs[0], 0));
      }
      if (all_patch) hipLaunchKernelGGL((k_faces_curv_list<true>), dim3(1024), dim3(256), 0, ctx->stream, Bt, ctx->d_flags, sl, sk);
      else hipLaunchKernelGGL((k_faces_curv_list<false>), dim3(1024), dim3(256), 0, ctx->stream, Bt, ctx->d_flags, sl, sk);
      for (int q = 0; q < Bt.n; ++q) {
        if (phi[blev[q]]->lev->pure_faces) continue;
        GenLev G = gen_lev(blev[q]);
        G.items = sl.gitems; G.n = sl.gcap; G.ncount = sl.gcount; G.lev = q;
        hipLaunchKernelGGL(k_curv_general<true>, dim3(256), dim3(256), 0, ctx->stream, G, ctx->d_flags, sk);
      }
      if (all_patch) hipLaunchKernelGGL((k_faces_curv_tab<true, true, true>), gtab, dim3(256), 0, pst, Bt, ctx->d_flags, sk);
      else hipLaunchKernelGGL((k_faces_curv_tab<true, false, true>), gtab, dim3(256), 0, pst, Bt, ctx->d_flags, sk);
      if (pst != ctx->stream) {
        PA_HIP(hipEventRecord(ctx->fix_evs[1], pst));
        PA_HIP(hipStreamWaitEvent(ctx->stream, ctx->fix_evs[1], 0));
      }
    } else {
      const bool sharded = nlev > 0 && phi[0]->lev->nranks > 1;
      const bool with_perim = sharded || npt * 8u <= Ck.w0[Bt.n];
      const unsigned np = with_perim ? npt : 0u;
      const dim3 gc(np + Ck.w0[Bt.n], 1, (unsigned)nslots);
      if (all_patch) hipLaunchKernelGGL((k_faces_fix_chunks<true>), gc, dim3(256), 0, ctx->stream, Bt, Ck, ctx->d_flags, sk, np);
      else hipLaunchKernelGGL((k_faces_fix_chunks<false>), gc, dim3(256), 0, ctx->stream, Bt, Ck, ctx->d_flags, sk, np);
      if (!with_perim) {
        if (all_patch) hipLaunchKernelGGL((k_faces_curv_tab<true, true>), gtab, dim3(256), 0, ctx->stream, Bt, ctx->d_flags, sk);
        else hipLaunchKernelGGL((k_faces_curv_tab<true, false>), gtab, dim3(256), 0, ctx->stream, Bt, ctx->d_flags, sk);
      }
    }
  }
  {
    const int phi_nranks = nlev > 0 ? phi[0]->lev->nranks : 1;
    GenBatch Gb;
    Gb.n = 0;
    Gb.wg0[0] = 0;
    auto flush = [&]() {
      if (!Gb.n) return;
      ProfScope prof(ctx, PA_TAG_GRADCURV_FACES);
      const dim3 gg(Gb.wg0[Gb.n], 1, (unsigned)nslots);
      bool light = !clip, patch = true;
      for (int q = 0; q < Gb.n; ++q) {
        light = light && Gb.a[q].L.nboxes > 0 && phi_nranks == 1;
        patch = patch && (Gb.a[q].use_cp || !Gb.a[q].A.has_crse);
      }
      if (light && patch) hipLaunchKernelGGL((k_curv_general_levels<false, false, true>), gg, dim3(256), 0, ctx->stream, Gb, ctx->d_flags, sk);
      else if (clip) hipLaunchKernelGGL((k_curv_general_levels<true, true, false>), gg, dim3(256), 0, ctx->stream, Gb, ctx->d_flags, sk);
      else hipLaunchKernelGGL((k_curv_general_levels<false, true, false>), gg, dim3(256), 0, ctx->stream, Gb, ctx->d_flags, sk);
      Gb.n = 0;
    };
    for (int l = 0; l < nlev; ++l) {
      const pa_level* L = phi[l]->lev;
      if (L->boxes.empty()) continue;
      if (level_irregular(ctx, L)) return 1;
      if (L->nirr == 0) continue;
      GenLev G = gen_lev(l);
      G.items = (const int4*)L->d_irr; G.n = L->nirr;
      Gb.a[Gb.n] = G;
      Gb.wg0[Gb.n + 1] = Gb.wg0[Gb.n] + (unsigned)((L->nirr + 255) / 256);
      if (++Gb.n == PA_MAXB) flush();
    }
    flush();
  }
  PA_HIP(hipGetLastError());
  return 0;
}
```

peleanalysis_amd/csrc/pa_internal.h:

```cpp
#pragma once
#include <hip/hip_runtime.h>
#include <cstdint>
#include <array>
#include <map>
#include <memory>
#include <string>
#include <utility>
#include <vector>
#include "../../include/peleanalysis_amd.h"

struct DBox { int lo[3]; int hi[3]; };

struct pa_options {
  int filter_exact = 0;
  int allow_unverified_gaussian = 0;
  int retile_max[3] = {0, 0, 0};
  int fused2 = 1;
  int ncg = 1;
  int dist_early = 0;
  int smooth_replicated = 0;
  int smooth_mg = -1;
  int smooth_march = 1;
  int smooth_timing = 0;
  int scratch_poison = 0;
  int force_fallbacks = 0;
};
const pa_options& pa_opt();

struct DLevelView {
  int nboxes;
  const DBox* boxes;
  int domlo[3], domhi[3], is_per[3];
  int g, mlo[3], mn[3];
  const int* owner;
  double dxinv[3];
  int gshift;
  int nsf;
  const int* sfaces;
  const int* sfindex;
  const long long* sfoff;
  const unsigned short* sfcode;
  const long long* cgoff;
  double* cg;
  const long long* cpoff;
  double* cp;
};

enum { PA_SFC_FULL = 1,
       PA_SFC_WALL = 2,
       PA_SFC_HAS_CF = 4,
       PA_SFC_HAS_VALID = 8 };
struct alignas(16) SfChunk {
  int face;
  int box;
  int dir_side;
  int flags;
  int lo[3], hi[3];
  int u0, v0, cw, ch;
  long long sfoff, cgoff, cpoff;
};
#define PA_CODE_FULL 0x555u

struct DMFView {
  double* data;
  const long long* off;
  int ncomp, ng;
  int xform;
  double xa, xb;
};

#define PA_MAXB 4
#define PA_MAXSLOTS 16
template <typename A, int CAP = PA_MAXB>
struct LevBatch {
  int n = 0;
  int ycum[CAP + 1] = {};
  A a[CAP];
  __device__ __forceinline__ int find(unsigned y, unsigned& local) const {
    int l = 0;
    while (l + 1 < n && y >= (unsigned)ycum[l + 1]) ++l;
    local = y - (unsigned)ycum[l];
    return l;
  }
};

struct pa_ctx {
  int device = 0;
  hipStream_t stream = nullptr;
  bool own_stream = false;
  std::string err;
  double* d_red = nullptr;
  size_t red_cap = 0;
  int* d_flags = nullptr;
  void* d_slow = nullptr;
  hipEvent_t fix_evs[2] = {nullptr, nullptr};
  double* d_prog = nullptr;
  void* d_scr = nullptr;
  size_t scr_cap = 0;
  void* h_pin = nullptr;
  size_t h_pin_cap = 0;
  void* d_mcz = nullptr;
  size_t mcz_cap = 0;
  bool mcz_dirty = true;
  std::map<void*, size_t> surf_live;
  std::vector<std::pair<void*, size_t>> surf_cache;
  unsigned profile = 0;
  struct Ev { hipEvent_t a, b; int tag; };
  std::vector<Ev> evs;
  hipStream_t stream2 = nullptr;
  std::vector<hipStream_t> lev_streams;
  std::vector<hipEvent_t> sync_evs;
  std::string sweep_kernel;
  int smooth_iters = -1;
  double smooth_res = 0.0;
  int curv_path = -1;
  pa_comm comm = {nullptr, 0, 1, nullptr, nullptr};
  struct RcclState* rccl = nullptr;
};

struct ProfScope {
  pa_ctx* ctx;
  pa_ctx::Ev e;
  bool on;
  ProfScope(pa_ctx* c, int tag) : ctx(c), on(((c->profile >> tag) & 1u) != 0) {
    if (!on) return;
    e.tag = tag;
    if (hipEventCreate(&e.a) != hipSuccess || hipEventCreate(&e.b) != hipSuccess) { on = false; return; }
    (void)hipEventRecord(e.a, ctx->stream);
  }
  ~ProfScope() {
    if (!on) return;
    (void)hipEventRecord(e.b, ctx->stream);
    ctx->evs.push_back(e);
  }
};
enum { PA_TAG_GRADCURV = 1, PA_TAG_GRADCURV_FACES = 2, PA_TAG_FILL = 3, PA_TAG_BC = 4, PA_TAG_GRAD = 5, PA_TAG_PROGRESS = 6,
       PA_TAG_FILTER = 7, PA_TAG_MC = 8, PA_TAG_XCHG = 9 };

struct WgTab {
  int* d = nullptr;
  unsigned n = 0;
  std::vector<int> h;
  mutable std::map<long long, unsigned char*> gneed;
  ~WgTab() {
    if (d) (void)hipFree(d);
    for (auto& kv : gneed)
      if (kv.second) (void)hipFree(kv.second);
  }
};

struct pa_level {
  pa_ctx* ctx = nullptr;
  std::vector<DBox> boxes;
  int domlo[3], domhi[3], is_per[3];
  double prob_lo[3], prob_hi[3], dx[3], dxinv[3];
  int g = 1, mlo[3], mn[3];
  std::vector<int> owner;
  DBox* d_boxes = nullptr;
  int* d_owner = nullptr;
  std::vector<int> sfaces;
  int* d_sfaces = nullptr;
  int* d_sfindex = nullptr;
  long long* d_sfoff = nullptr;
  unsigned short* d_sfcode = nullptr;
  int maxn[3] = {0, 0, 0};
  long long ncells = 0;
  bool fusable = true;
  bool pure_faces = true;
  long long* d_cpoff = nullptr;
  double* d_cp = nullptr;
  int cp_sets = 0, cg_sets = 0;
  long long cp_total = 0;
  long long* d_cgoff = nullptr;
  double* d_cg = nullptr;
  long long cg_total = 0;
  double* d_ncg = nullptr;
  bool ncg_live = false;
  int ncg_minw = 0;
  std::vector<long long> cgoff;
  int* d_blist = nullptr;
  int nwide = 0, nnarrow = 0;
  int wmax[3] = {0, 0, 0}, nmax[3] = {0, 0, 0};
  int* d_sfboxes = nullptr;
  int nsfboxes = 0;
  void* d_sfwg = nullptr;
  int nsfwg = 0;
  void* d_pfwg = nullptr;
  int npfwg = 0;
  SfChunk* d_sfchunk = nullptr;
  int nsfchunk = 0;
  void* d_ring = nullptr;
  int nring = -1;
  std::vector<unsigned char> xneed;
  void* d_irr = nullptr;
  int nirr = -1;
  int nremote = 0;
  DLevelView view;
  int rank = 0, nranks = 1;
  long long serial = 0;
  std::vector<DBox> gboxes;
  std::vector<int> gowner;
  std::vector<int> gid;
  std::vector<int> glocal;
  bool source_only = false;
  mutable std::map<int, std::unique_ptr<struct XPlan>> fb_plans;
  mutable std::map<long long, std::unique_ptr<struct CpPlan>> cp_plans;
  mutable std::map<int, std::unique_ptr<struct FbLocal>> fb_local;
  mutable std::map<std::pair<long long, int>, std::unique_ptr<struct CsPlan>> cs_plans;
  mutable std::unique_ptr<struct RepPlan> rep_plan;
  mutable std::map<long long, std::unique_ptr<WgTab>> wgtabs;
  mutable std::map<long long, std::unique_ptr<struct RsPlan>> rs_plans;
  mutable std::map<std::pair<long long, int>, std::unique_ptr<struct FpPlan>> fp_plans;
  mutable std::map<std::array<int, 3>, struct pa_mf*> scratch;
  ~pa_level();
};

struct FpPlan {
  int n = 0;
  void* d_items = nullptr;
  ~FpPlan();
};

struct LevelSpec {
  std::vector<DBox> local;
  std::vector<int> gid;
  std::vector<DBox> gboxes;
  std::vector<int> gowner;
  int rank = 0, nranks = 1;
  bool source_only = false;
};
pa_level* pa_level_create_spec(pa_ctx* ctx, const LevelSpec& S, const int32_t domlo[3], const int32_t domhi[3], const int32_t is_per[3],
                               const double prob_lo[3], const double prob_hi[3]);
bool pa_face_is_special(const pa_level* L, const DBox& B, int d, int side);
struct pa_mf* pa_level_scratch(pa_ctx* ctx, const pa_level* L, int ncomp, int ng, int role = 0);
const WgTab* pa_sweep_wgtab(const pa_level* L, int cls, int tw, int mty, int kseg, bool force, int part = 0);
const unsigned char* pa_sweep_gneed(const pa_level* L, const WgTab* T, int tw, int mty, int kseg, long long fine_serial, const std::vector<int>* cpregs);
int pa_host_classify(const pa_level* L, int i, int j, int k);

struct pa_mf {
  const pa_level* lev = nullptr;
  int ncomp = 0, ng = 0;
  double* data = nullptr;
  bool owned = false;
  std::vector<long long> off;
  long long* d_off = nullptr;
  long long total = 0;
  DMFView view;
};

#define PA_HIP(call)                                                                      \
  do {                                                                                    \
    hipError_t e_ = (call);                                                               \
    if (e_ != hipSuccess) {                                                               \
      ctx->err = std::string(#call) + ": " + hipGetErrorString(e_);                       \
      return 1;                                                                           \
    }                                                                                     \
  } while (0)

int pa_fail(pa_ctx* ctx, const std::string& msg);

struct PaBind {
  explicit PaBind(const pa_ctx* c) { if (c) (void)hipSetDevice(c->device); }
};

__host__ __device__ __forceinline__ long long pa_cstride(long long ncells, int ncomp) {
  long long cs = (ncells + 63) / 64 * 64;
  if (ncomp > 1) {
    if (ncells >= 32768) cs += (256 + 2048 - cs % 2048) % 2048;
    else if ((cs % 2048) == 0) cs += 64;
  }
  return cs;
}

__device__ __forceinline__ long long fab_index(const DBox& B, int ng, int ncomp, int c, int i, int j, int k) {
  const long long nx = B.hi[0] - B.lo[0] + 1 + 2 * ng, ny = B.hi[1] - B.lo[1] + 1 + 2 * ng,
                  nz = B.hi[2] - B.lo[2] + 1 + 2 * ng;
  return (long long)c * pa_cstride(nx * ny * nz, ncomp) + ((long long)(k - B.lo[2] + ng) * ny + (j - B.lo[1] + ng)) * nx + (i - B.lo[0] + ng);
}

__device__ __forceinline__ bool wrap_cell(const DLevelView& L, int p[3]) {
#pragma unroll
  for (int d = 0; d < 3; ++d) {
    const int len = L.domhi[d] - L.domlo[d] + 1;
    if (p[d] < L.domlo[d] || p[d] > L.domhi[d]) {
      if (!L.is_per[d]) return false;
      while (p[d] < L.domlo[d]) p[d] += len;
      while (p[d] > L.domhi[d]) p[d] -= len;
    }
  }
  return true;
}

__device__ __forceinline__ int owner_of(const DLevelView& L, const int p[3]) {
  int m[3];
#pragma unroll
  for (int d = 0; d < 3; ++d) {
    const int r = p[d] - L.mlo[d];
    if (r < 0) return -1;
    m[d] = L.gshift >= 0 ? (r >> L.gshift) : (r / L.g);
    if (m[d] >= L.mn[d]) return -1;
  }
  return L.owner[((long long)m[2] * L.mn[1] + m[1]) * L.mn[0] + m[0]];
}

__device__ __forceinline__ int classify(const DLevelView& L, int i, int j, int k, int& box, int p[3]) {
  p[0] = i; p[1] = j; p[2] = k;
  if (!wrap_cell(L, p)) return 2;
  box = owner_of(L, p);
  return (box != -1) ? 0 : 1;
}
__device__ __forceinline__ int classify(const DLevelView& L, int i, int j, int k) {
  int b, p[3];
  return classify(L, i, j, k, b, p);
}

__host__ __device__ __forceinline__ int coarsen_idx(int i, int r) { return r == 2 ? (i >> 1) : ((i < 0) ? -((-i + r - 1) / r) : i / r); }

template <typename F>
__device__ __forceinline__ double sg_sum(const double n[3], F f) {
  return +n[0] * n[1] * n[2] * f(1, 1, 1)
         + n[0] * (1.0 - n[1]) * n[2] * f(1, 0, 1)
         + n[0] * n[1] * (1.0 - n[2]) * f(1, 1, 0)
         + n[0] * (1.0 - n[1]) * (1.0 - n[2]) * f(1, 0, 0)
         + (1.0 - n[0]) * n[1] * n[2] * f(0, 1, 1)
         + (1.0 - n[0]) * (1.0 - n[1]) * n[2] * f(0, 0, 1)
         + (1.0 - n[0]) * n[1] * (1.0 - n[2]) * f(0, 1, 0)
         + (1.0 - n[0]) * (1.0 - n[1]) * (1.0 - n[2]) * f(0, 0, 0);
}

__device__ __forceinline__ void poly_interp_coeff(double xInt, const double* x, int N, double* c) {
  for (int j = 0; j < N; ++j) {
    double num = 1.0, den = 1.0;
    for (int i = 0; i < N; ++i) {
      if (i == j) continue;
      num *= xInt - x[i];
      den *= x[j] - x[i];
    }
    c[j] = num / den;
  }
}

__device__ __forceinline__ double cdiff(double dxinv, double m, double c, double p) {
  const double fl = -(dxinv * (c - m));
// ... 230 lines not shown
```

Before: 69800 Mcells/s.

## Sort face chunks by kind and launch specialized per-kind fix/prep kernels

At level creation, surface chunk records are sorted on the host into straight, mixed and generic groups, and per-kind counts are stored. The prep and fix face kernels are templated on chunk kind so each launch compiles only one code path, with tighter launch bounds for the specialized variants to raise occupancy and cut divergence. Register pressure in the fix chunk is also reduced by loading neighbour data per row and replacing small indexed arrays with scalars. In exchange there are up to three launches instead of one, and a misclassified chunk is flagged through the error counter instead of falling back to the generic path.

```diff
diff --git a/include/peleanalysis_amd.h b/include/peleanalysis_amd.h
--- a/include/peleanalysis_amd.h
+++ b/include/peleanalysis_amd.h
@@ -35,6 +35,7 @@
 int pa_sweep_occupancy(pa_ctx*, int which);
 int pa_last_slow_cells(pa_ctx*);
 int64_t pa_level_irregular_cells(pa_ctx*, const pa_level*);
+int pa_level_chunk_kinds(pa_ctx*, const pa_level*, int32_t kinds[3]);
 int pa_profile_read(pa_ctx*, int tag, int64_t* nlaunch, double* total_ms, int reset);
 
 pa_level* pa_level_create(pa_ctx*, int nboxes, const int32_t* boxes6, const int32_t domlo[3],
diff --git a/peleanalysis_amd/capi.py b/peleanalysis_amd/capi.py
--- a/peleanalysis_amd/capi.py
+++ b/peleanalysis_amd/capi.py
@@ -174,6 +174,7 @@
         "pa_stream_trace": (C.c_int, [vp, C.c_int, C.POINTER(vp), C.c_int, i64, pdbl, C.c_int, dbl, vp, pi32]),
         "pa_last_slow_cells": (C.c_int, [vp]),
         "pa_level_irregular_cells": (i64, [vp, vp]),
+        "pa_level_chunk_kinds": (C.c_int, [vp, vp, pi32]),
         "pa_stream_trace_ranks": (C.c_int, [vp, C.c_int, C.POINTER(vp), C.c_int, i64, pdbl, C.c_int, dbl, vp, pi32, C.c_int]),
         "pa_vtrace_fab": (C.c_int, [vp, C.POINTER(PaFab), i32, vp, i64, vp, i32, C.POINTER(PaFab), i32, C.POINTER(PaFab), i32, pdbl, pdbl, pdbl, dbl,
                                     pi32]),
diff --git a/peleanalysis_amd/csrc/pa_core.hip b/peleanalysis_amd/csrc/pa_core.hip
--- a/peleanalysis_amd/csrc/pa_core.hip
+++ b/peleanalysis_amd/csrc/pa_core.hip
@@ -712,6 +712,24 @@
       pa_level_destroy(L);
       return nullptr;
     }
+    if (L->nsfchunk > 0) {
+      std::vector<SfChunk> ck((size_t)L->nsfchunk), sorted;
+      if (hipMemcpy(ck.data(), L->d_sfchunk, sizeof(SfChunk) * ck.size(), hipMemcpyDeviceToHost) != hipSuccess) {
+        pa_fail(ctx, "pa_level_create: reading the chunk records failed");
+        pa_level_destroy(L);
+        return nullptr;
+      }
+      sorted.reserve(ck.size());
+      for (int kind = 0; kind < 3; ++kind)
+        for (const SfChunk& D : ck)
+          if (sfchunk_kind(D) == kind) { sorted.push_back(D); ++L->nck[kind]; }
+      for (const SfChunk& D : ck) L->nck_cf += (D.flags & (PA_SFC_FULL | PA_SFC_HAS_CF)) ? 1 : 0;
+      if (hipMemcpy(L->d_sfchunk, sorted.data(), sizeof(SfChunk) * sorted.size(), hipMemcpyHostToDevice) != hipSuccess) {
+        pa_fail(ctx, "pa_level_create: device allocation failed");
+        pa_level_destroy(L);
+        return nullptr;
+      }
+    }
   }
   return L;
 }
@@ -739,6 +757,11 @@
   delete L;
 }
 extern "C" int pa_level_nboxes(const pa_level* L) { return L ? (int)L->boxes.size() : 0; }
+extern "C" int pa_level_chunk_kinds(pa_ctx* ctx, const pa_level* L, int32_t kinds[3]) {
+  if (!ctx || !L || !kinds) return pa_fail(ctx, "pa_level_chunk_kinds: null argument");
+  for (int k = 0; k < 3; ++k) kinds[k] = L->nck[k];
+  return 0;
+}
 
 extern "C" int64_t pa_mf_layout(int nboxes, const int32_t* b6, int ncomp, int ng, int64_t* off, int64_t* cstride) {
   int64_t t = 0;
diff --git a/peleanalysis_amd/csrc/pa_fused.hip b/peleanalysis_amd/csrc/pa_fused.hip
--- a/peleanalysis_amd/csrc/pa_fused.hip
+++ b/peleanalysis_amd/csrc/pa_fused.hip
@@ -26,24 +26,25 @@
   const double* cg;
   __device__ __forceinline__ double operator()(int i, int j, int k) const {
     const int p[3] = {i, j, k};
-    int nout = 0, fd[2] = {0, 0}, fs[2] = {0, 0};
+    int nout = 0, fd0 = 0, fd1 = 0, fs0 = 0, fs1 = 0;
     bool near = true;
 #pragma unroll
     for (int d = 0; d < 3; ++d) {
       const int o = p[d] < B.lo[d] ? B.lo[d] - p[d] : (p[d] > B.hi[d] ? p[d] - B.hi[d] : 0);
       if (o) {
-        if (nout < 2) { fd[nout] = d; fs[nout] = p[d] > B.hi[d]; }
+        if (nout == 0) { fd0 = d; fs0 = p[d] > B.hi[d]; }
+        else if (nout == 1) { fd1 = d; fs1 = p[d] > B.hi[d]; }
         ++nout;
         near = near && o == 1;
       }
     }
     int e = -1, d = 0;
-    if (near && nout == 1) { d = fd[0]; e = L->sfindex[b * 6 + d * 2 + fs[0]]; }
+    if (near && nout == 1) { d = fd0; e = L->sfindex[b * 6 + d * 2 + fs0]; }
     if (near && nout == 2) {
-      const int ea = L->sfindex[b * 6 + fd[0] * 2 + fs[0]], ec = L->sfindex[b * 6 + fd[1] * 2 + fs[1]];
+      const int ea = L->sfindex[b * 6 + fd0 * 2 + fs0], ec = L->sfindex[b * 6 + fd1 * 2 + fs1];
       if (ea >= 0 && ec >= 0) return 0.0;
-      if (ea >= 0) { e = ea; d = fd[0]; }
-      if (ec >= 0) { e = ec; d = fd[1]; }
+      if (ea >= 0) { e = ea; d = fd0; }
+      if (ec >= 0) { e = ec; d = fd1; }
     }
     if (e < 0) return (P(i, j, k, pcomp) - pmin) * invd;
     const int t0 = (d == 0) ? 1 : 0, t1 = (d == 2) ? 1 : 2;
@@ -164,9 +165,13 @@
     else if (r < 2 * n0) { a0 = r - n0; a1 = n1 - 1; }
     else { r -= 2 * n0; a0 = (r & 1u) ? n0 - 1 : 0; a1 = 1 + (r >> 1); }
     if (n0 == 1 && (r & 1u) && t >= 2 * (long long)n0) return;
-    q0[fdir] = side ? B.hi[fdir] + 1 : B.lo[fdir] - 1;
-    q0[t0] = B.lo[t0] + (int)a0;
-    q0[t1] = B.lo[t1] + (int)a1;
+    {
+      const int fhi = fdir == 0 ? B.hi[0] : (fdir == 1 ? B.hi[1] : B.hi[2]), flo = fdir == 0 ? B.lo[0] : (fdir == 1 ? B.lo[1] : B.lo[2]);
+      const int f = side ? fhi + 1 : flo - 1;
+      q0[0] = fdir == 0 ? f : B.lo[0] + (int)a0;
+      q0[1] = fdir == 1 ? f : B.lo[1] + (int)(fdir == 0 ? a0 : a1);
+      q0[2] = fdir == 2 ? f : B.lo[2] + (int)a1;
+    }
     if (layer >= B.hi[fdir] - B.lo[fdir] + 1) return;
     if ((L.sfcode[L.sfoff[fy] + a0 + (long long)n0 * a1] & 3u) == 0) return;
   } else {
@@ -674,41 +679,37 @@
     cpatch_geom(B, FD, side, plane, pu0, pv0, pw, ph);
     cf_block_load(L.cp + z * Fx.cp_stride + D.cpoff + (long long)((X1[T1] >> 1) - pv0) * pw + ((X1[T0] >> 1) - pu0), pw, K);
   }
-  double nfd[2][2][3], a0[2][2][3], a1[2][2][3], t01n[2][2], t11n[2][2];
-  if (pre) {
-    const pa_fix_d2* np = (const pa_fix_d2*)(Fx.ncg + 2 * D.cgoff);
-#pragma unroll
-    for (int dv = 0; dv < 2; ++dv)
-#pragma unroll
-      for (int du = 0; du < 2; ++du) {
-        const pa_fix_d2 v0 = np[cgo[dv][du]], v1 = np[Fx.ncgs + cgo[dv][du]], v2 = np[2 * Fx.ncgs + cgo[dv][du]];
-        nfd[dv][du][0] = v0.x; nfd[dv][du][1] = v0.y; nfd[dv][du][2] = v1.x; t01n[dv][du] = v1.y; t11n[dv][du] = v2.x;
-      }
-  } else {
-#pragma unroll
-    for (int dv = 0; dv < 2; ++dv)
-#pragma unroll
-      for (int du = 0; du < 2; ++du) {
-#pragma unroll
-        for (int m = 0; m < 3; ++m) nfd[dv][du][m] = nf[off[dv][du] + m * in];
-#pragma unroll
-        for (int k = 0; k < 3; ++k) {
-          a0[dv][du][k] = n0p[off[dv][du] + (k - 1) * s0];
-          a1[dv][du][k] = n1p[off[dv][du] + (k - 1) * s1];
-        }
-      }
-  }
-  if (cf_here) cf_block_finish(K);
   const bool odd = Fx.A.bc[FD] == PA_BC_REFLECT_ODD;
   constexpr double nc0 = k_cf_coef.nrm[4][0], nc1 = k_cf_coef.nrm[4][1], nc2 = k_cf_coef.nrm[4][2], nc3 = k_cf_coef.nrm[4][3];
   int nbad_here = 0;
 #pragma unroll
-  for (int dv = 0; dv < 2; ++dv)
+  for (int dv = 0; dv < 2; ++dv) {
+    double nfd[2][3], a0[2][3], a1[2][3], t01n[2], t11n[2];
+    if (pre) {
+      const pa_fix_d2* np = (const pa_fix_d2*)(Fx.ncg + 2 * D.cgoff);
+#pragma unroll
+      for (int du = 0; du < 2; ++du) {
+        const pa_fix_d2 v0 = np[cgo[dv][du]], v1 = np[Fx.ncgs + cgo[dv][du]], v2 = np[2 * Fx.ncgs + cgo[dv][du]];
+        nfd[du][0] = v0.x; nfd[du][1] = v0.y; nfd[du][2] = v1.x; t01n[du] = v1.y; t11n[du] = v2.x;
+      }
+    } else {
+#pragma unroll
+      for (int du = 0; du < 2; ++du) {
+#pragma unroll
+        for (int m = 0; m < 3; ++m) nfd[du][m] = nf[off[dv][du] + m * in];
+#pragma unroll
+        for (int k = 0; k < 3; ++k) {
+          a0[du][k] = n0p[off[dv][du] + (k - 1) * s0];
+          a1[du][k] = n1p[off[dv][du] + (k - 1) * s1];
+        }
+      }
+    }
+    if (dv == 0 && cf_here) cf_block_finish(K);
 #pragma unroll
     for (int du = 0; du < 2; ++du) {
       const unsigned cd = live[dv][du] ? code[dv][du] : 2u;
       const int cls = (int)(cd & 3u);
-      const double nfd1 = nfd[dv][du][0], nfd2 = nfd[dv][du][1], nfd3 = nfd[dv][du][2];
+      const double nfd1 = nfd[du][0], nfd2 = nfd[du][1], nfd3 = nfd[du][2];
       double g = odd ? -nfd1 : nfd1;
       bool write = live[dv][du];
       if (cf_here) {
@@ -733,8 +734,8 @@
         else write = false;
       }
       const double f1 = side ? cdiff(L.dxinv[FD], nfd2, nfd1, g) : cdiff(L.dxinv[FD], g, nfd1, nfd2);
-      const double t01 = pre ? t01n[dv][du] : cdiff(L.dxinv[T0], a0[dv][du][0], a0[dv][du][1], a0[dv][du][2]);
-      const double t11 = pre ? t11n[dv][du] : cdiff(L.dxinv[T1], a1[dv][du][0], a1[dv][du][1], a1[dv][du][2]);
+      const double t01 = pre ? t01n[du] : cdiff(L.dxinv[T0], a0[du][0], a0[du][1], a0[du][2]);
+      const double t11 = pre ? t11n[du] : cdiff(L.dxinv[T1], a1[du][0], a1[du][1], a1[du][2]);
       double k1 = 0.0;
       k1 += (FD == 0) ? f1 : t01;
       k1 += (FD == 1) ? f1 : (FD == 0 ? t01 : t11);
@@ -742,25 +743,39 @@
       k1 = k1 * 0.5;
       if (write) ko[off[dv][du]] = k1;
     }
+  }
   if (nbad_here) atomicAdd(nbad, nbad_here);
 }
 
 struct LevChunks { const SfChunk* ck[PA_MAXB]; unsigned w0[PA_MAXB + 1]; };
-template <bool PATCH>
-__global__ __launch_bounds__(256) void k_faces_fix_chunks(LevBatch<FixArgs> Bt, LevChunks Ck, int* nbad, SlotK sk, unsigned nperim) {
-  if (blockIdx.x < nperim) { faces_tab_wg<true, PATCH, false>(Bt, nbad, sk, blockIdx.x); return; }
-  const unsigned wx = blockIdx.x - nperim;
+struct KindChunks { LevChunks k[3]; };
+static void kind_chunks_add(KindChunks& K, int q, const pa_level* L, bool one_kind_ok) {
+  if (q == 0)
+    for (int kind = 0; kind < 3; ++kind) K.k[kind].w0[0] = 0;
+  const int n[3] = {one_kind_ok ? L->nck[0] : 0, one_kind_ok ? L->nck[1] : 0, one_kind_ok ? L->nck[2] : L->nsfchunk};
+  const SfChunk* p = L->d_sfchunk;
+  for (int kind = 0; kind < 3; ++kind) {
+    K.k[kind].ck[q] = p;
+    K.k[kind].w0[q + 1] = K.k[kind].w0[q] + (unsigned)n[kind];
+    if (one_kind_ok) p += n[kind];
+  }
+}
+template <bool PATCH, int KIND, bool PERIM>
+__global__ __launch_bounds__(256, KIND == PA_CK_ANY ? 1 : 4) void k_faces_fix_chunks(LevBatch<FixArgs> Bt, LevChunks Ck, int* nbad, SlotK sk, unsigned nperim) {
+  if (PERIM && blockIdx.x < nperim) { faces_tab_wg<true, PATCH, false>(Bt, nbad, sk, blockIdx.x); return; }
+  const unsigned wx = blockIdx.x - (PERIM ? nperim : 0u);
   int blev = 0;
   while (blev + 1 < Bt.n && wx >= Ck.w0[blev + 1]) ++blev;
   const FixArgs& Fx = Bt.a[blev];
   const SfChunk D = Ck.ck[blev][wx - Ck.w0[blev]];
   const int dir = D.dir_side >> 1;
   const int e0 = D.hi[0] - D.lo[0] + 1, e1 = D.hi[1] - D.lo[1] + 1, e2 = D.hi[2] - D.lo[2] + 1;
-  const int blen = dir == 0 ? e0 : (dir == 1 ? e1 : e2), n0 = dir == 0 ? e1 : e0, n1 = dir == 2 ? e1 : e2;
+  const int blen = dir == 0 ? e0 : (dir == 1 ? e1 : e2);
   const bool cfok = Fx.A.has_crse && Fx.A.ratio == 2 && Fx.use_cp && Fx.L.cp && D.cpoff >= 0;
   const bool straight = blen >= 3 && ((D.flags & PA_SFC_WALL) != 0 || ((D.flags & PA_SFC_FULL) != 0 && cfok));
   const bool mixed = !straight && blen >= 3 && (cfok || !(D.flags & PA_SFC_HAS_CF));
-  if (straight) {
+  if (KIND == PA_CK_STRAIGHT || (KIND == PA_CK_ANY && straight)) {
+    if (!straight) { if (threadIdx.x == 0) atomicAdd(nbad, 1); return; }
     switch (dir) {
       case 0: fix_chunk_uniform<0>(Fx, D, (int)blockIdx.z, nbad); break;
       case 1: fix_chunk_uniform<1>(Fx, D, (int)blockIdx.z, nbad); break;
@@ -768,7 +783,8 @@
     }
     return;
   }
-  if (mixed) {
+  if (KIND == PA_CK_MIXED || (KIND == PA_CK_ANY && mixed)) {
+    if (!mixed) { if (threadIdx.x == 0) atomicAdd(nbad, 1); return; }
     __shared__ double tabs[54];
     cf_tab_to_lds(tabs);
     switch (dir) {
@@ -778,11 +794,14 @@
     }
     return;
   }
-  const int hw = D.cw >> 1, sh = 31 - __builtin_clz((unsigned)hw);
-  const int u = D.u0 + 2 * ((int)threadIdx.x & (hw - 1)), v = D.v0 + 2 * ((int)threadIdx.x >> sh);
-  for (int dv = 0; dv < 2; ++dv)
-    for (int du = 0; du < 2; ++du)
-      if (u + du >= 0 && v + dv >= 0 && u + du < n0 && v + dv < n1) faces_fast_cell<1, PATCH, false>(Bt, nbad, SlowList(), sk, blev, (unsigned)D.face, (long long)(v + dv) * n0 + (u + du));
+  if (KIND == PA_CK_ANY) {
+    const int n0 = dir == 0 ? e1 : e0, n1 = dir == 2 ? e1 : e2;
+    const int hw = D.cw >> 1, sh = 31 - __builtin_clz((unsigned)hw);
+    const int u = D.u0 + 2 * ((int)threadIdx.x & (hw - 1)), v = D.v0 + 2 * ((int)threadIdx.x >> sh);
+    for (int dv = 0; dv < 2; ++dv)
+      for (int du = 0; du < 2; ++du)
+        if (u + du >= 0 && v + dv >= 0 && u + du < n0 && v + dv < n1) faces_fast_cell<1, PATCH, false>(Bt, nbad, SlowList(), sk, blev, (unsigned)D.face, (long long)(v + dv) * n0 + (u + du));
+  }
 }
 
 template <int NL, bool PATCH = false, bool CLIP = false>
@@ -1333,7 +1352,7 @@
   prep_ring_wg<PATCH, DIRECT>(Bt, Rg, nbad, sk, blockIdx.x);
 }
 
-template <bool PATCH, bool PHIONLY = false>
+template <bool PATCH, bool PHIONLY, int KIND>
 __global__ __launch_bounds__(256) void k_prep_faces_chunks(LevBatch<PrepLev> Bt, LevChunks Ck, LevRings Rg, int* nbad, SlotK sk = SlotK()) {
   const unsigned nrw = Rg.w0[Bt.n];
   if (blockIdx.x < nrw) { if (!PHIONLY) prep_ring_wg<PATCH, true>(Bt, Rg, nbad, sk, blockIdx.x); return; }
@@ -1344,20 +1363,22 @@
   const SfChunk D = Ck.ck[blev][wx - Ck.w0[blev]];
   const int dir = D.dir_side >> 1;
   const int e0 = D.hi[0] - D.lo[0] + 1, e1 = D.hi[1] - D.lo[1] + 1, e2 = D.hi[2] - D.lo[2] + 1;
-  const int blen = dir == 0 ? e0 : (dir == 1 ? e1 : e2), n0 = dir == 0 ? e1 : e0, n1 = dir == 2 ? e1 : e2;
+  const int blen = dir == 0 ? e0 : (dir == 1 ? e1 : e2);
   const bool cfok = Pl.A.has_crse && Pl.A.ratio == 2 && Pl.use_cp && Pl.L.cp && D.cpoff >= 0 && blen >= 3;
   const bool straight = (D.flags & PA_SFC_WALL) != 0 || ((D.flags & PA_SFC_FULL) != 0 && cfok);
   const bool mixed = !straight && blen >= 3 && (cfok || !(D.flags & PA_SFC_HAS_CF));
-  if (straight || mixed) {
+  const bool as_straight = KIND == PA_CK_STRAIGHT || (KIND == PA_CK_ANY && straight), as_mixed = !as_straight && (KIND == PA_CK_MIXED || (KIND == PA_CK_ANY && mixed));
+  if (as_straight || as_mixed) {
+    if (as_straight ? !straight : !mixed) { if (threadIdx.x == 0) atomicAdd(nbad, 1); return; }
     __shared__ double tabs[54];
-    if (mixed) cf_tab_to_lds(tabs);
+    if (as_mixed) cf_tab_to_lds(tabs);
     const int z = (int)blockIdx.z;
     PrepArgs A = Pl.A;
     double xa = Pl.MC.xa, xb = Pl.MC.xb;
     if (sk.prog) { A.pmin = xa = sk.prog[2 * z]; A.invd = xb = sk.prog[2 * z + 1]; }
     double* const cgz = PHIONLY ? nullptr : Pl.L.cg + z * Pl.cg_stride;
     const double* const cpz = Pl.L.cp ? Pl.L.cp + z * Pl.cp_stride : nullptr;
-    if (straight) {
+    if (as_straight) {
       switch (dir) {
         case 0: prep_chunk_uniform<0, PHIONLY>(Pl, D, A, xa, xb, Pl.comp + z, cgz, cpz, nbad); break;
         case 1: prep_chunk_uniform<1, PHIONLY>(Pl, D, A, xa, xb, Pl.comp + z, cgz, cpz, nbad); break;
@@ -1372,11 +1393,14 @@
     }
     return;
   }
-  const int hw = D.cw >> 1, sh = 31 - __builtin_clz((unsigned)hw);
-  const int u = D.u0 + 2 * ((int)threadIdx.x & (hw - 1)), v = D.v0 + 2 * ((int)threadIdx.x >> sh);
-  for (int dv = 0; dv < 2; ++dv)
-    for (int du = 0; du < 2; ++du)
-      if (u + du >= 0 && v + dv >= 0 && u + du < n0 && v + dv < n1) prep_faces_cell<PATCH, PHIONLY>(Pl, nbad, sk, (unsigned)D.face, (long long)(v + dv) * n0 + (u + du));
+  if (KIND == PA_CK_ANY) {
+    const int n0 = dir == 0 ? e1 : e0, n1 = dir == 2 ? e1 : e2;
+    const int hw = D.cw >> 1, sh = 31 - __builtin_clz((unsigned)hw);
+    const int u = D.u0 + 2 * ((int)threadIdx.x & (hw - 1)), v = D.v0 + 2 * ((int)threadIdx.x >> sh);
+    for (int dv = 0; dv < 2; ++dv)
+      for (int du = 0; du < 2; ++du)
+        if (u + du >= 0 && v + dv >= 0 && u + du < n0 && v + dv < n1) prep_faces_cell<PATCH, PHIONLY>(Pl, nbad, sk, (unsigned)D.face, (long long)(v + dv) * n0 + (u + du));
+  }
 }
 
 static int level_cg(pa_ctx* ctx, const pa_level* Lc, int nsets = 1) {
@@ -1979,13 +2003,13 @@
     ProfScope prof(ctx, PA_TAG_BC);
     bool all_patch = true;
     for (int q = 0; q < Bf.n; ++q) all_patch = all_patch && (Bf.a[q].use_cp || !Bf.a[q].A.has_crse);
-    LevChunks Ck;
-    Ck.w0[0] = 0;
+    KindChunks Kc;
+    unsigned nchunks = 0;
     for (int q = 0; q < Bf.n; ++q) {
       const pa_level* Lq = batch_lev[q];
       if (!Lq->d_sfchunk || Lq->nsfchunk <= 0) return pa_fail(ctx, "pa_gradcurv_prep_levels: a level without chunk records");
-      Ck.ck[q] = Lq->d_sfchunk;
-      Ck.w0[q + 1] = Ck.w0[q] + (unsigned)Lq->nsfchunk;
+      kind_chunks_add(Kc, q, Lq, all_patch && (Lq->nck_cf == 0 || (Bf.a[q].A.has_crse && Bf.a[q].use_cp && Bf.a[q].L.cp)));
+      nchunks += (unsigned)Lq->nsfchunk;
     }
     LevRings Rg, Rnone;
     Rg.w0[0] = 0;
@@ -1999,17 +2023,27 @@
         Rg.n[q] = (unsigned)Lq->nring;
         Rg.w0[q + 1] = Rg.w0[q] + (unsigned)((Lq->nring + 255) / 256);
       }
-    const bool ring_with_faces = (phase & 1) && (phase & 2) && !(phase & 8) && direct && Rg.w0[Bf.n] * 8u <= Ck.w0[Bf.n];
+    const bool ring_with_faces = (phase & 1) && (phase & 2) && !(phase & 8) && direct && Rg.w0[Bf.n] * 8u <= nchunks;
     if (phase & 1) {
-      const LevRings& Rk = ring_with_faces ? Rg : Rnone;
-      const dim3 gc(Rk.w0[Bf.n] + Ck.w0[Bf.n], 1, (unsigned)nslots);
-      if (phase & 8) {
-        if (all_patch) hipLaunchKernelGGL((k_prep_faces_chunks<true, true>), gc, dim3(256), 0, ctx->stream, Bf, Ck, Rk, ctx->d_flags, sk);
-        else hipLaunchKernelGGL((k_prep_faces_chunks<false, true>), gc, dim3(256), 0, ctx->stream, Bf, Ck, Rk, ctx->d_flags, sk);
-      } else {
-        if (all_patch) hipLaunchKernelGGL((k_prep_faces_chunks<true, false>), gc, dim3(256), 0, ctx->stream, Bf, Ck, Rk, ctx->d_flags, sk);
-        else hipLaunchKernelGGL((k_prep_faces_chunks<false, false>), gc, dim3(256), 0, ctx->stream, Bf, Ck, Rk, ctx->d_flags, sk);
-      }
+      bool ring_pending = ring_with_faces;
+      auto go = [&](auto kind) {
+        constexpr int KIND = decltype(kind)::value;
+        const LevChunks& Ck = Kc.k[KIND];
+        if (Ck.w0[Bf.n] == 0) return;
+        const LevRings& Rk = ring_pending ? Rg : Rnone;
+        ring_pending = false;
+        const dim3 gc(Rk.w0[Bf.n] + Ck.w0[Bf.n], 1, (unsigned)nslots);
+        if (phase & 8) {
+          if (all_patch) hipLaunchKernelGGL((k_prep_faces_chunks<true, true, KIND>), gc, dim3(256), 0, ctx->stream, Bf, Ck, Rk, ctx->d_flags, sk);
+          else if constexpr (KIND == PA_CK_ANY) hipLaunchKernelGGL((k_prep_faces_chunks<false, true, KIND>), gc, dim3(256), 0, ctx->stream, Bf, Ck, Rk, ctx->d_flags, sk);
+        } else {
+          if (all_patch) hipLaunchKernelGGL((k_prep_faces_chunks<true, false, KIND>), gc, dim3(256), 0, ctx->stream, Bf, Ck, Rk, ctx->d_flags, sk);
+          else if constexpr (KIND == PA_CK_ANY) hipLaunchKernelGGL((k_prep_faces_chunks<false, false, KIND>), gc, dim3(256), 0, ctx->stream, Bf, Ck, Rk, ctx->d_flags, sk);
+        }
+      };
+      go(std::integral_constant<int, PA_CK_STRAIGHT>{});
+      go(std::integral_constant<int, PA_CK_MIXED>{});
+      go(std::integral_constant<int, PA_CK_ANY>{});
     }
     if ((phase & 2) && !ring_with_faces && Rg.w0[Bf.n] > 0) {
       const dim3 gr(Rg.w0[Bf.n], 1, (unsigned)nslots);
@@ -2345,14 +2379,14 @@
     unsigned nwgf = 0;
     for (int q = 0; q < Bt.n; ++q) nwgf += (unsigned)Bt.a[q].nwg;
     const dim3 gfast(nwgf, 1, (unsigned)nslots);
-    LevChunks Ck;
-    Ck.w0[0] = 0;
+    KindChunks Kc;
+    unsigned nchunks = 0;
     unsigned npt = 0;
     for (int q = 0; q < Bt.n; ++q) {
       const pa_level* Lq = phi[blev[q]]->lev;
       if (!Lq->d_sfchunk || Lq->nsfchunk <= 0 || !Bt.a[q].pwg || Bt.a[q].npwg <= 0) return pa_fail(ctx, "pa_gradcurv_fix_levels: a level without chunk records / perimeter tables");
-      Ck.ck[q] = Lq->d_sfchunk;
-      Ck.w0[q + 1] = Ck.w0[q] + (unsigned)Lq->nsfchunk;
+      kind_chunks_add(Kc, q, Lq, all_patch && (Lq->nck_cf == 0 || (Bt.a[q].A.has_crse && Bt.a[q].use_cp && Bt.a[q].L.cp)));
+      nchunks += (unsigned)Lq->nsfchunk;
       npt += (unsigned)Bt.a[q].npwg;
     }
     const dim3 gtab(npt, 1, (unsigned)nslots);
@@ -2387,11 +2421,29 @@
       }
     } else {
       const bool sharded = nlev > 0 && phi[0]->lev->nranks > 1;
-      const bool with_perim = sharded || npt * 8u <= Ck.w0[Bt.n];
-      const unsigned np = with_perim ? npt : 0u;
-      const dim3 gc(np + Ck.w0[Bt.n], 1, (unsigned)nslots);
-      if (all_patch) hipLaunchKernelGGL((k_faces_fix_chunks<true>), gc, dim3(256), 0, ctx->stream, Bt, Ck, ctx->d_flags, sk, np);
-      else hipLaunchKernelGGL((k_faces_fix_chunks<false>), gc, dim3(256), 0, ctx->stream, Bt, Ck, ctx->d_flags, sk, np);
+      const bool can_ride = Kc.k[PA_CK_STRAIGHT].w0[Bt.n] > 0 || Kc.k[PA_CK_MIXED].w0[Bt.n] == 0;
+      const bool with_perim = (sharded || npt * 8u <= nchunks) && can_ride;
+      bool perim_pending = with_perim;
+      auto go = [&](auto kind) {
+        constexpr int KIND = decltype(kind)::value;
+        const LevChunks& Ck = Kc.k[KIND];
+        if (Ck.w0[Bt.n] == 0) return;
+        const unsigned np = (perim_pending && KIND != PA_CK_MIXED) ? npt : 0u;
+        if (np) perim_pending = false;
+        const dim3 gc(np + Ck.w0[Bt.n], 1, (unsigned)nslots);
+        if (np) {
+          if constexpr (KIND != PA_CK_MIXED) {
+            if (all_patch) hipLaunchKernelGGL((k_faces_fix_chunks<true, KIND, true>), gc, dim3(256), 0, ctx->stream, Bt, Ck, ctx->d_flags, sk, np);
+            else if constexpr (KIND == PA_CK_ANY) hipLaunchKernelGGL((k_faces_fix_chunks<false, KIND, true>), gc, dim3(256), 0, ctx->stream, Bt, Ck, ctx->d_flags, sk, np);
+          }
+        } else {
+          if (all_patch) hipLaunchKernelGGL((k_faces_fix_chunks<true, KIND, false>), gc, dim3(256), 0, ctx->stream, Bt, Ck, ctx->d_flags, sk, np);
+          else if constexpr (KIND == PA_CK_ANY) hipLaunchKernelGGL((k_faces_fix_chunks<false, KIND, false>), gc, dim3(256), 0, ctx->stream, Bt, Ck, ctx->d_flags, sk, np);
+        }
+      };
+      go(std::integral_constant<int, PA_CK_STRAIGHT>{});
+      go(std::integral_constant<int, PA_CK_MIXED>{});
+      go(std::integral_constant<int, PA_CK_ANY>{});
       if (!with_perim) {
         if (all_patch) hipLaunchKernelGGL((k_faces_curv_tab<true, true>), gtab, dim3(256), 0, ctx->stream, Bt, ctx->d_flags, sk);
         else hipLaunchKernelGGL((k_faces_curv_tab<true, false>), gtab, dim3(256), 0, ctx->stream, Bt, ctx->d_flags, sk);
diff --git a/peleanalysis_amd/csrc/pa_internal.h b/peleanalysis_amd/csrc/pa_internal.h
--- a/peleanalysis_amd/csrc/pa_internal.h
+++ b/peleanalysis_amd/csrc/pa_internal.h
@@ -59,6 +59,15 @@
   int u0, v0, cw, ch;
   long long sfoff, cgoff, cpoff;
 };
+enum { PA_CK_STRAIGHT = 0,
+       PA_CK_MIXED = 1,
+       PA_CK_ANY = 2 };
+static inline int sfchunk_kind(const SfChunk& D) {
+  const int dir = D.dir_side >> 1;
+  if (D.hi[dir] - D.lo[dir] + 1 < 3) return PA_CK_ANY;
+  if (D.flags & (PA_SFC_WALL | PA_SFC_FULL)) return PA_CK_STRAIGHT;
+  return (D.cpoff >= 0 || !(D.flags & PA_SFC_HAS_CF)) ? PA_CK_MIXED : PA_CK_ANY;
+}
 #define PA_CODE_FULL 0x555u
 
 struct DMFView {
@@ -189,6 +198,8 @@
   int npfwg = 0;
   SfChunk* d_sfchunk = nullptr;
   int nsfchunk = 0;
+  int nck[3] = {0, 0, 0};
+  int nck_cf = 0;
   void* d_ring = nullptr;
   int nring = -1;
   std::vector<unsigned char> xneed;
```

Measured after the change: 69790 Mcells/s. Within noise of the previous version (-0.0%).
